# GAMES-UChile/mogptk

Hardware: AMD Instinct MI355X
Metric: log-marginal-likelihood+grad evals/sec, MOSM C=4 N=8192; 1/2/4/8 GPU (higher is better)
Workload: dtype f64

## Files before the change

mogptk_amd/csrc/exact.hip:

```cpp
#include "mogp_model.h"
#include <cstdlib>
#include <limits>

using namespace mogp;

static int wait_stream(hipStream_t st) {
    static const bool spin = !(std::getenv("MOGP_SPIN_WAIT") && std::atoi(std::getenv("MOGP_SPIN_WAIT")) == 0);
    if (!spin) { HIP_TRY(hipStreamSynchronize(st)); return 0; }
    for (;;) {
        const hipError_t e = hipStreamQuery(st);
        if (e == hipSuccess) return 0;
        if (e != hipErrorNotReady) return hip_fail(e, "hipStreamQuery", __FILE__, __LINE__);
    }
}

static hipEvent_t prof_event(mogp_model* m, int idx) {
    if (!m->profiling) return nullptr;
    while ((int)m->ev.size() <= idx) { hipEvent_t e; if (hipEventCreate(&e) != hipSuccess) return nullptr; m->ev.push_back(e); }
    return m->ev[idx];
}

static void kinv_block_ranges(mogp_model* m) {
    std::vector<int> blk;
    tile_blocks(m->sx.off, m->C, blk);
    const int nblk = (int)blk.size() / 2, D = m->D;
    m->blk_cen.assign((size_t)D * nblk, 0.0); m->blk_half.assign((size_t)D * nblk, 0.0);
    for (int b = 0; b < nblk; ++b)
        for (int d = 0; d < D; ++d) {
            const double* x = m->sx.xs.data() + (size_t)d * m->sx.Mpad + blk[2 * b];
            double lo = x[0], hi = x[0];
            for (int i = 1; i < blk[2 * b + 1]; ++i) { lo = std::fmin(lo, x[i]); hi = std::fmax(hi, x[i]); }
            m->blk_cen[(size_t)d * nblk + b] = 0.5 * (lo + hi); m->blk_half[(size_t)d * nblk + b] = 0.5 * (hi - lo);
        }
}

static int kinv_plan(mogp_model* m, bool want) {
    static const bool full = std::getenv("MOGP_FULL_INVERSE") && std::atoi(std::getenv("MOGP_FULL_INVERSE")) != 0;
    m->kinv_sparse = false; m->kinv_fraction = 1.0;
    if (!want || full || m->sh_n > 1 || m->tiles.empty() || m->radial) return 0;
    const int nb = m->nb, D = m->D, T = m->T, W = m->Wt;
    const int64_t ld = m->Npad;
    if (m->blk_cen.empty()) kinv_block_ranges(m);
    const int nblk = (int)(m->blk_cen.size() / std::max(D, 1));
    std::vector<char> need((size_t)nb * nb, 0);
    for (const GTile& t : m->tiles) {
        const double* tab = m->table.data() + (size_t)t.pair * T * W;
        bool read = false;
        for (int k = 0; k < T && !read; ++k) {
            const double* row = tab + (size_t)k * W;
            double emin = 0.0;
            for (int d = 0; d < D; ++d) {
                const double sd = (m->blk_cen[(size_t)d * nblk + t.rb] - m->blk_cen[(size_t)d * nblk + t.cb]) + row[2 + 2 * D + d];
                const double mu = std::fmax(0.0, std::fabs(sd) - m->blk_half[(size_t)d * nblk + t.rb] - m->blk_half[(size_t)d * nblk + t.cb]);
                emin += row[2 + d] * mu * mu;
            }
            read = !(0.5 * emin > 52.0);
        }
        if (!read) continue;
        const int i0 = t.r0 / MOGP_TILE, i1 = (t.r0 + t.nr - 1) / MOGP_TILE, j0 = t.c0 / MOGP_TILE, j1 = (t.c0 + t.nc - 1) / MOGP_TILE;
        for (int i = i0; i <= i1; ++i) for (int j = j0; j <= j1; ++j) if (j <= i) need[(size_t)i * nb + j] = 1;
    }
    for (int i = 0; i < nb; ++i) need[(size_t)i * nb + i] = 1;
    std::vector<GemmTask> acc, lau;
    std::vector<int> prefix(nb + 1, 0);
    for (int i = 0; i < nb; ++i) {
        for (int j = 0; j <= i; ++j) {
            if (!need[(size_t)i * nb + j]) continue;
            GemmTask a;
            a.a_off = (int64_t)i * MOGP_TILE; a.b_off = (int64_t)j * MOGP_TILE; a.c_off = (int64_t)i * MOGP_TILE * ld + (int64_t)j * MOGP_TILE;
            a.kt = 4 * MOGP_TILE / 16; a.pad = i + 1;
            acc.push_back(a);
            GemmTask l;
            l.a_off = (int64_t)i * MOGP_TILE * ld + (int64_t)i * MOGP_TILE; l.b_off = (int64_t)i * MOGP_TILE * ld + (int64_t)j * MOGP_TILE;
            l.c_off = a.c_off; l.kt = (int)((ld - (int64_t)i * MOGP_TILE) / 16); l.pad = 0;
            lau.push_back(l);
        }
        prefix[i + 1] = (int)acc.size();
    }
    const double frac = (double)acc.size() / ((double)nb * (nb + 1) / 2);
    m->kinv_fraction = frac;
    if (frac > 0.85) return 0;
    const bool same = acc.size() == m->kinv_acc_tasks.size() && (acc.empty() || std::memcmp(acc.data(), m->kinv_acc_tasks.data(), acc.size() * sizeof(GemmTask)) == 0);
    if (!same || m->d_kinv_acc.n < acc.size()) {
        int rc;
        if ((rc = m->d_kinv_acc.ensure(std::max<size_t>(acc.size(), 1)))) return rc;
        if ((rc = m->d_kinv_lauum.ensure(std::max<size_t>(lau.size(), 1)))) return rc;
        HIP_TRY(hipMemcpyAsync(m->d_kinv_acc.p, acc.data(), acc.size() * sizeof(GemmTask), hipMemcpyHostToDevice, m->st));
        HIP_TRY(hipMemcpyAsync(m->d_kinv_lauum.p, lau.data(), lau.size() * sizeof(GemmTask), hipMemcpyHostToDevice, m->st));
        HIP_TRY(hipStreamSynchronize(m->st));
        m->kinv_acc_tasks.swap(acc); m->kinv_lauum_tasks.swap(lau);
    }
    m->kinv_prefix.swap(prefix);
    m->kinv_sparse = true;
    return 0;
}

static int pin_ensure(mogp_model* m, size_t n) {
    if (n <= m->h_pin_n) return 0;
    if (m->h_pin) { hipError_t e = hipHostFree(m->h_pin); (void)e; m->h_pin = nullptr; m->h_pin_n = 0; }
    HIP_TRY(hipHostMalloc(reinterpret_cast<void**>(&m->h_pin), n * sizeof(double), hipHostMallocDefault));
    m->h_pin_n = n;
    return 0;
}
struct PinLayout {
    size_t nzz, logdet = 0, zz, info, moments, diagG, pivots, total;
    PinLayout(int nb, int64_t Npad, int C, int T, int Wt) : nzz((size_t)((Npad + 3) / 4)) {
        zz = (size_t)nb; info = zz + nzz; moments = info + 1; diagG = moments + (size_t)(C * (C + 1) / 2) * T * Wt; pivots = diagG + C; total = pivots + 2;
    }
    explicit PinLayout(const mogp_model* m) : PinLayout(m->nb, m->Npad, m->C, m->T, m->Wt) {}
};

namespace mogp {
int begin_call(mogp_model* m, int64_t* info, bool one_gpu) {
    m->mean_w = nullptr;
    if (int rc = use_device(m->ctx)) return rc;
    if (info) *info = 0;
    if (one_gpu) one_gpu_call(m);
    return 0;
}

int exact_begin(mogp_model* m, const double* noise_var, const double* data_var, double jitter, GramArgs& ga, double& jabs) {
    const int C = m->C;
    const int64_t N = m->N, Npad = m->Npad;
    if (m->T <= 0) return fail(MOGP_EINVAL, "mogp_model_set_terms must be called before an evaluation");
    if (!noise_var) return fail(MOGP_EINVAL, "noise_var is null");
    { int r__ = ensure_system(m); if (r__) return r__; }
    m->have_W = m->have_Kinv = false;
    m->gemm_ev_used = 0; m->gemm_launches = 0; m->gemm_flops = 0.0;

    double dsum = 0.0;
    if (!m->point_diag.empty()) {
        for (int c = 0; c < C; ++c)
            for (int k = m->sx.off[c]; k < m->sx.off[c + 1]; ++k) dsum += m->point_diag[k] + noise_var[c];
    } else if (m->radial && m->point_kinds) {
        dsum = table_diag_points(m, m->sx);
        for (int c = 0; c < C; ++c) dsum += (double)(m->sx.off[c + 1] - m->sx.off[c]) * noise_var[c];
    } else
    for (int c = 0; c < C; ++c) dsum += (double)(m->sx.off[c + 1] - m->sx.off[c]) * (table_diag(m, c) + noise_var[c]);
    if (data_var) {
        std::vector<double> dv(Npad, 0.0);
        for (int64_t pos = 0; pos < N; ++pos) { dv[pos] = data_var[m->sx.perm[pos]]; dsum += dv[pos]; }
        { int r__ = m->d_dvar.ensure(Npad); if (r__) return r__; }
        HIP_TRY(hipMemcpyAsync(m->d_dvar.p, dv.data(), Npad * sizeof(double), hipMemcpyHostToDevice, m->st));
    }
    jabs = jitter * dsum / (double)N;
    HIP_TRY(hipMemcpyAsync(m->d_noise.p, noise_var, C * sizeof(double), hipMemcpyHostToDevice, m->st));
    static const unsigned long long big = std::numeric_limits<unsigned long long>::max();
    HIP_TRY(hipMemcpyAsync(m->d_info.p, &big, sizeof(big), hipMemcpyHostToDevice, m->st));
    int rc;
    if ((rc = mark(m, 0))) return rc;
    ga = GramArgs{};
    ga.tiles = m->d_tiles.p; ga.xr = m->d_x.p; ga.xc = m->d_x.p; ga.ldxr = ga.ldxc = Npad; ga.nrows = ga.ncols = N;
    if ((rc = m->ph_xx.prepare(m->sx.off, m->sx.off, C, m->T, Npad, Npad, m->st, ga.ph))) return rc;
    ga.table = m->d_table.p; ga.T = m->T; ga.D = m->D; ga.C = C; ga.W = m->Wt;
    ga.out = m->k.A.p; ga.ldo = Npad; ga.noise = m->d_noise.p; ga.dvar = data_var ? m->d_dvar.p : nullptr;
    ga.jitter_abs = jabs; ga.mirror = 0;
    if (m->radial) { ga.kind = m->d_kind.p; ga.shape = m->d_shape.p; }
    return 0;
}
}

namespace mogp { int chain_fallback(mogp_model* m) {
    if (m->flow_ran) {
        m->no_flow = true; m->flow_ran = false;
        m->flow_timeouts++;
        m->flow_retry_at = m->n_fact + m->flow_backoff;
        m->flow_backoff = std::min(m->flow_backoff * 4, 16384);
        for (hipStream_t q : {m->st, m->st2, m->st3, m->st4, m->ctx->st5, m->st_priv}) if (q) HIP_TRY(hipStreamSynchronize(q));
        static bool said_flow = false;
        if (!said_flow) {
            said_flow = true;
            unsigned code = 0;
            if (m->k.flow_flags.p && m->k.flow_cur && m->k.flow_cur->base_err > 0) { hipError_t e = hipMemcpy(&code, m->k.flow_flags.p + m->k.flow_cur->base_err, sizeof(code), hipMemcpyDeviceToHost); (void)e; }
            fprintf(stderr, "mogp: the dataflow kernel timed out (wait 0x%x; GPU shared with another process?); using the stream schedule for the next %d evaluations (said once)\n", code, (int)(m->flow_retry_at - m->n_fact));
            fprintf(stderr, "mogp: the host enqueued that evaluation in %.0f us (longest so far %.0f us)\n", m->flow_enqueue_us, m->flow_enqueue_us_max);
        }
        if (std::getenv("MOGP_FLOW_DEBUG")) { fprintf(stderr, "mogp: dataflow time-out %d of this model\n", m->flow_timeouts); flow_debug_dump(m); }
        return 0;
    }
    if (m->no_chain) return fail(MOGP_EHIP, "chain kernel: a hand-off timed out although the model is on the launch-per-step chain");
    m->no_chain = true;
    for (hipStream_t q : {m->st, m->st2, m->st3, m->st4, m->ctx->st5, m->st_priv}) if (q) HIP_TRY(hipStreamSynchronize(q));
    static bool said = false;
    if (!said) { said = true; fprintf(stderr, "mogp: the persistent chain kernel timed out (GPU shared with another process?); using the launch-per-step chain\n"); }
    return 0;
} }

template <typename F> static int retry_on_streams(mogp_model* m, int rc, F again) {
    if (rc != MOGP_RETRY_NO_CHAIN) return rc;
    if ((rc = chain_fallback(m))) return rc;
    return again();
}

namespace mogp { int report_not_pd(unsigned long long hinfo, int64_t* info) {
    if (info) *info = (int64_t)hinfo;
    return fail(MOGP_ENOTPD, "linalg.cholesky: The factorization could not be completed because the input is not "
                             "positive-definite (the leading minor of order " + std::to_string(hinfo) + " is not positive-definite).");
} }

static int factorize_finish(mogp_model* m, const GramArgs& ga, double* lml, int64_t* info) {
    const int64_t N = m->N, Npad = m->Npad;
    const PinLayout pl(m);
    const unsigned long long big = std::numeric_limits<unsigned long long>::max();
    unsigned long long hinfo = 0;
    std::memcpy(&hinfo, m->h_pin + pl.info, sizeof(hinfo));
    int rc;
    if (hinfo == MOGP_INFO_CHAIN_TIMEOUT) return MOGP_RETRY_NO_CHAIN;
    static const bool fake = std::getenv("MOGP_FAKE_K") && std::atoi(std::getenv("MOGP_FAKE_K")) > 1;
    if (hinfo != big && !fake) {
        if (info) *info = (int64_t)hinfo;
        int flag = 0;
        HIP_TRY(hipMemsetAsync(m->d_flag.p, 0, sizeof(int), m->st));
        if ((rc = launch_gram(ga, (int)m->tiles.size(), m->st, m->radial ? m->gate_kinds : 0))) return rc;
        if ((rc = launch_nonfinite_scan(m->k.A.p, Npad, N, m->d_flag.p, m->st))) return rc;
        HIP_TRY(hipMemcpyAsync(&flag, m->d_flag.p, sizeof(int), hipMemcpyDeviceToHost, m->st));
        HIP_TRY(hipStreamSynchronize(m->st));
        if (flag & 1) return fail(MOGP_ENONFINITE, "linalg.cholesky: kernel matrix has NaNs!");
        if (flag & 2) return fail(MOGP_ENONFINITE, "linalg.cholesky: kernel matrix has infinities!");
        return report_not_pd(hinfo, info);
    }
    m->pivot_min = m->h_pin[pl.pivots]; m->pivot_max = m->h_pin[pl.pivots + 1];
    double logdet = 0.0, zz = 0.0;
    for (int i = 0; i < m->nb; ++i) logdet += m->h_pin[pl.logdet + i];
    for (size_t i = 0; i < pl.nzz; ++i) zz += m->h_pin[pl.zz + i];
    if (lml) *lml = -0.5 * (double)N * std::log(2.0 * M_PI) - logdet - 0.5 * zz;
    m->have_W = !m->factor_only && !m->accurate_ran;
    return 0;
}

struct FactorPlan {
    enum Schedule { Fused, Phases, FactorOnly } schedule = Phases;
    bool defer = false;
    bool want_inverse = true;
    bool refine = false;
};

static int factorize(mogp_model* m, const double* noise_var, const double* data_var, double jitter, const FactorPlan& plan,
                     double* lml, double* jitter_abs, int64_t* info, GramArgs* ga_out = nullptr) {
    const bool fuse_inverse = plan.schedule == FactorPlan::Fused, factor_only = plan.schedule == FactorPlan::FactorOnly;
    const int64_t N = m->N, Npad = m->Npad;
    GramArgs ga{};
    double jabs = 0.0;
    int rc = exact_begin(m, noise_var, data_var, jitter, ga, jabs);
    if (rc) return rc;
    if (jitter_abs) *jitter_abs = jabs;
    m->n_fact++;
    if (m->no_flow && m->n_fact >= m->flow_retry_at) m->no_flow = false;
    m->factor_only = factor_only;
    ga.ev0 = prof_event(m, 7); ga.ev1 = prof_event(m, 8);
    m->strip.attach(ga);
    static const bool split_on = !(std::getenv("MOGP_GRAM_SPLIT") && std::atoi(std::getenv("MOGP_GRAM_SPLIT")) == 0);
    const bool split = split_on && fuse_inverse && flow_enabled(m, m->k) && !m->tiles_head.empty() && !m->tiles_tail.empty() && m->st2;
    if (split) {
        GramArgs gh = ga, gt = ga;
        gh.tiles = m->d_tiles_head.p; m->strip_head.attach(gh); gh.ev1 = nullptr;
        gt.tiles = m->d_tiles_tail.p; m->strip_tail.attach(gt); gt.ev0 = nullptr; gt.phases_ready = 1;
        if ((rc = launch_gram(gh, (int)m->tiles_head.size(), m->st, m->radial ? m->gate_kinds : 0))) return rc;
        if ((rc = launch_pad_identity(m->k.A.p, Npad, N, Npad, m->st))) return rc;
        if (!m->gram_ev) HIP_TRY(hipEventCreateWithFlags(&m->gram_ev, hipEventDisableTiming));
        HIP_TRY(hipEventRecord(m->gram_ev, m->st));
        HIP_TRY(hipStreamWaitEvent(m->st2, m->gram_ev, 0));
        if ((rc = launch_gram(gt, (int)m->tiles_tail.size(), m->st2, m->radial ? m->gate_kinds : 0))) return rc;
        if (!m->gram_tail_ev) HIP_TRY(hipEventCreateWithFlags(&m->gram_tail_ev, hipEventDisableTiming));
        HIP_TRY(hipEventRecord(m->gram_tail_ev, m->st2));
        m->k.tail_ready = m->gram_tail_ev;
    } else {
        if ((rc = launch_gram(ga, (int)m->tiles.size(), m->st, m->radial ? m->gate_kinds : 0))) return rc;
        if ((rc = launch_pad_identity(m->k.A.p, Npad, N, Npad, m->st))) return rc;
    }
    ga.ev0 = ga.ev1 = nullptr;
    if ((rc = mark(m, 1))) return rc;

    const PinLayout pl(m);
    if ((rc = pin_ensure(m, pl.total))) return rc;
    if ((rc = m->d_pivots.ensure(2))) return rc;
    if (m->accurate && (rc = m->acc_rhs.ensure((size_t)Npad * MOGP_TILE))) return rc;
    m->k.flow_used = false;
    m->flow_ran = false;
    m->k.want_vec = fuse_inverse;
    m->k.vec_y = m->d_y.p; m->k.vec_z = m->d_z.p; m->k.vec_zz = m->d_zz.p; m->k.vec_part = m->d_alpha.p + Npad;
    const bool accurate = m->accurate && plan.schedule == FactorPlan::Phases;
    m->accurate_ran = accurate;
    m->k.keep_L = m->k.refine_panels = plan.refine || accurate;
    if (factor_only && m->rhs_job && flow_enabled(m, m->k)) rc = spd_potri_flow(m, m->k, m->rhs_job);
    else rc = fuse_inverse ? spd_potri_fused(m, m->k) : spd_potrf(m, m->k);
    m->k.keep_L = m->k.refine_panels = false;
    m->k.want_vec = false; m->k.tail_ready = nullptr;
    if (rc) return rc;
    if ((rc = mark(m, 2))) return rc;
    if (accurate) {
        static const bool acc_aside = !(std::getenv("MOGP_ACC_ASIDE") && std::atoi(std::getenv("MOGP_ACC_ASIDE")) == 0);
        hipStream_t ms = (plan.want_inverse && m->st2u && acc_aside) ? m->st2u : m->st;
        if (plan.want_inverse) {
            if (ms != m->st) {
                while ((int)m->k.inv_ev.size() < 4) { hipEvent_t e; HIP_TRY(hipEventCreateWithFlags(&e, hipEventDisableTiming)); m->k.inv_ev.push_back(e); }
                HIP_TRY(hipEventRecord(m->k.inv_ev[0], m->st));
                HIP_TRY(hipStreamWaitEvent(ms, m->k.inv_ev[0], 0));
            }
            if ((rc = m->k.Wm.ensure((size_t)Npad * Npad))) return rc;
            HIP_TRY(hipMemsetAsync(m->k.Wm.p, 0, (size_t)Npad * Npad * sizeof(double), ms));
            if ((rc = launch_add_diag(m->k.Wm.p, Npad, Npad, 1.0, ms))) return rc;
            if ((rc = trsm_lower(m, m->k.A.p, Npad, m->nb, m->k.Wm.p, Npad, Npad, false, ms, true))) return rc;
            GemmArgs g{};
            g.A = m->k.Wm.p; g.lda = Npad; g.a_kmajor = 1; g.B = m->k.Wm.p; g.ldb = Npad; g.b_kmajor = 1;
            g.C = m->k.B.p; g.ldc = Npad; g.alpha = 1.0; g.beta = 0.0; g.mode = GM_LAUUM; g.mt = g.nt = m->nb; g.K = (int)Npad;
            if ((rc = gemm_call(m, g, gemm_flops(g, nullptr), ms))) return rc;
            if (ms != m->st) HIP_TRY(hipEventRecord(m->k.inv_ev[1], ms));
        }
        HIP_TRY(hipMemsetAsync(m->acc_rhs.p, 0, (size_t)Npad * MOGP_TILE * sizeof(double), m->st));
        if ((rc = launch_copy2d(m->acc_rhs.p, MOGP_TILE, m->d_y.p, 1, Npad, 1, 1.0, m->st))) return rc;
        if ((rc = trsm_lower(m, m->k.A.p, Npad, m->nb, m->acc_rhs.p, MOGP_TILE, MOGP_TILE, false))) return rc;
        if ((rc = launch_copy2d(m->d_z.p, 1, m->acc_rhs.p, MOGP_TILE, Npad, 1, 1.0, m->st))) return rc;
        HIP_TRY(hipMemsetAsync(m->d_zz.p, 0, pl.nzz * sizeof(double), m->st));
        if ((rc = launch_gemv_rows(m->d_z.p, Npad, 1, Npad, m->d_z.p, m->d_zz.p, m->st))) return rc;
        if ((rc = trsm_lower(m, m->k.A.p, Npad, m->nb, m->acc_rhs.p, MOGP_TILE, MOGP_TILE, true))) return rc;
        if ((rc = launch_copy2d(m->d_alpha.p, 1, m->acc_rhs.p, MOGP_TILE, Npad, 1, 1.0, m->st))) return rc;
        if (plan.want_inverse && ms != m->st) HIP_TRY(hipStreamWaitEvent(m->st, m->k.inv_ev[1], 0));
    } else if (plan.schedule == FactorPlan::Phases && (rc = spd_trtri(m, m->k))) return rc;
    if ((rc = mark(m, 3))) return rc;

    if (factor_only) {
        HIP_TRY(hipMemsetAsync(m->d_zz.p, 0, pl.nzz * sizeof(double), m->st));
    } else if (!accurate) {
        const double* Wp = fuse_inverse ? m->k.Wm.p : m->k.A.p;
        m->w_in_Wm = fuse_inverse;
        if (fuse_inverse && m->k.flow_used && m->k.vec_done) {
            if ((rc = launch_flow_alpha_sum(m->k, m->d_alpha.p, m->st))) return rc;
        } else {
            if ((rc = launch_trmv_lower(Wp, Npad, Npad, m->d_y.p, m->d_z.p, m->d_zz.p, m->st))) return rc;
            if ((rc = launch_trmv_lower_t(Wp, Npad, Npad, m->d_z.p, m->d_alpha.p, m->st))) return rc;
        }
    }
    if (fuse_inverse && (rc = spd_potri_fused_finish(m, m->k))) return rc;
    if ((rc = mark(m, 4))) return rc;
    {
        static const bool fault = std::getenv("MOGP_FLOW_FAULT") && std::atoi(std::getenv("MOGP_FLOW_FAULT")) != 0;
        static const unsigned long long timed_out = MOGP_INFO_CHAIN_TIMEOUT;
        if (fault && m->k.flow_used) HIP_TRY(hipMemcpyAsync(m->d_info.p, &timed_out, sizeof(timed_out), hipMemcpyHostToDevice, m->st));
    }

    const int nzz = (int)pl.nzz;
    if ((rc = launch_pivot_range(m->k.invd.p, N, m->d_pivots.p, m->st))) return rc;
    HIP_TRY(hipMemcpyAsync(m->h_pin + pl.pivots, m->d_pivots.p, 2 * sizeof(double), hipMemcpyDeviceToHost, m->st));
    HIP_TRY(hipMemcpyAsync(m->h_pin + pl.logdet, m->k.logdet.p, m->nb * sizeof(double), hipMemcpyDeviceToHost, m->st));
    static const int zz_piece = []() { const char* e = std::getenv("MOGP_D2H_CHUNK"); const int v = e ? std::atoi(e) : 2048; return v > 0 ? v : (1 << 30); }();
    for (int o = 0; o < nzz; o += zz_piece)
        HIP_TRY(hipMemcpyAsync(m->h_pin + pl.zz + o, m->d_zz.p + o, std::min(zz_piece, nzz - o) * sizeof(double), hipMemcpyDeviceToHost, m->st));
    HIP_TRY(hipMemcpyAsync(m->h_pin + pl.info, m->d_info.p, sizeof(unsigned long long), hipMemcpyDeviceToHost, m->st));
    if (ga_out) *ga_out = ga;
    if (plan.defer) return 0;
    HIP_TRY(hipStreamSynchronize(m->st));
    return factorize_finish(m, ga, lml, info);
}

namespace mogp { void collect_timing(mogp_model* m, int last_mark) {
    if (!m->profiling) return;
    auto el = [&](int a, int b) { float t = 0.f; if (hipEventElapsedTime(&t, m->ev[a], m->ev[b]) != hipSuccess) t = 0.f; return (double)t; };
    std::fill(m->ms, m->ms + MOGP_ST_COUNT, 0.0);
    m->ms[MOGP_ST_GRAM] = el(0, 1);
    m->ms[MOGP_ST_POTRF] = el(1, 2);
    m->ms[MOGP_ST_TRTRI] = el(2, 3);
    m->ms[MOGP_ST_SOLVE] = el(3, 4);
    if (last_mark >= 6) { m->ms[MOGP_ST_LAUUM] = el(4, 5); m->ms[MOGP_ST_MOMENTS] = el(5, 6); }
    m->ms[MOGP_ST_TOTAL] = el(0, last_mark);
    if ((int)m->ev.size() > 8) m->ms[MOGP_ST_GRAM_KERNEL] = el(7, 8);
    if (last_mark >= 6 && (int)m->ev.size() > 10) m->ms[MOGP_ST_MOMENT_KERNEL] = el(9, 10);
    double gsum = 0.0;
    for (size_t i = 0; i + 1 < m->gemm_ev_used; i += 2) {
        float t = 0.f;
        if (hipEventElapsedTime(&t, m->gemm_ev[i], m->gemm_ev[i + 1]) == hipSuccess) gsum += t;
    }
    m->ms[MOGP_ST_GEMM_KERNEL] = gsum;
}

int moment_pass_device(mogp_model* m, const double* kinv, double ksign) {
    const int C = m->C, D = m->D, W = m->Wt, T = m->T, P = C * (C + 1) / 2;
    const int64_t Npad = m->Npad;
    const int rm = m->sh_n > 1 ? m->sh_n : 0;
    const bool own = m->sh_n > 1 && m->own_n == m->sh_n && m->own_rank == m->sh_rank;
    int rc;
    MomentArgs ma{};
    ma.tiles = own ? m->d_tiles_own.p : m->d_tiles.p; ma.ntiles = (int)(own ? m->tiles_own.size() : m->tiles.size());
    ma.x = m->d_x.p; ma.ldx = Npad; ma.nrows = ma.ncols = m->N;
    if ((rc = m->ph_xx.prepare(m->sx.off, m->sx.off, C, T, Npad, Npad, m->st, ma.ph))) return rc;
    ma.table = m->d_table.p; ma.T = T; ma.D = D; ma.C = C; ma.W = W; ma.kinv = kinv; ma.kinv_sign = ksign; ma.ld = Npad; ma.alpha = m->d_alpha.p;
    ma.row_mod = rm; ma.row_rem = m->sh_rank;
    if (m->radial) { ma.kind = m->d_kind.p; ma.shape = m->d_shape.p; }
    ma.partial = m->d_partial.p;
    ma.phases_ready = 1;
    ma.ev0 = prof_event(m, 9); ma.ev1 = prof_event(m, 10);
    if ((rc = launch_moments(ma, m->st, m->radial ? m->gate_kinds : 0))) return rc;
    if ((rc = launch_moment_reduce(m->d_partial.p, own ? m->d_pair_start_own.p : m->d_pair_start.p, P, T, W, D, m->d_moments.p, m->st))) return rc;
    if ((rc = launch_diagG(kinv, Npad, m->d_alpha.p, m->d_chan_off.p, C, m->d_diagG.p, m->st, ksign, rm, m->sh_rank))) return rc;
    if ((rc = mean_grad_enqueue(m, m->d_alpha.p, -1.0))) return rc;
    return mark(m, 6);
}

int moment_pass(mogp_model* m, const double* kinv, double ksign, double* moments, double* diagG) {
    const int C = m->C, W = m->Wt, T = m->T, P = C * (C + 1) / 2;
    int rc;
    if ((rc = moment_pass_device(m, kinv, ksign))) return rc;
    HIP_TRY(hipMemcpyAsync(moments, m->d_moments.p, (size_t)P * T * W * sizeof(double), hipMemcpyDeviceToHost, m->st));
    HIP_TRY(hipMemcpyAsync(diagG, m->d_diagG.p, C * sizeof(double), hipMemcpyDeviceToHost, m->st));
    HIP_TRY(hipStreamSynchronize(m->st));
    return 0;
}

int test_side(mogp_model* m, int64_t S, const double* Xs, const double* kss_diag, int64_t extra_rows, hipStream_t st, TestSide& ts, GramArgs& ga) {
    const int C = m->C, D = m->D;
    const int64_t Npad = m->Npad;
    SortedX& ss = ts.ss;
    int rc;
    if ((rc = sort_inputs(Xs, S, D, C, MOGP_TILE, ss))) return rc;
    const int64_t Spad = ts.Spad = ss.Mpad, Srow = Spad + extra_rows;
    std::vector<GTile> pt;
    build_rect_tiles(ss.off, m->sx.off, C, pt);
    ts.ntiles = (int)pt.size();
    if ((rc = m->d_xs.ensure((size_t)D * Spad))) return rc;
    if ((rc = m->d_Ksf.ensure((size_t)Srow * Npad))) return rc;
    if ((rc = m->d_mu.ensure(Spad))) return rc;
    if ((rc = m->d_kdiag.ensure(Spad))) return rc;
    if ((rc = m->d_ptiles.ensure(std::max<size_t>(pt.size(), 1)))) return rc;
    std::vector<double> kd(Spad, 0.0);
    const bool per_point = m->Wt > 2 + 3 * D || (m->radial && m->point_kinds);
    for (int c = 0; c < C; ++c)
        for (int pos = ss.off[c]; pos < ss.off[c + 1]; ++pos) kd[pos] = per_point ? kss_diag[ss.perm[pos]] : kss_diag[c];
    HIP_TRY(hipMemcpyAsync(m->d_xs.p, ss.xs.data(), (size_t)D * Spad * sizeof(double), hipMemcpyHostToDevice, st));
    HIP_TRY(hipMemcpyAsync(m->d_kdiag.p, kd.data(), Spad * sizeof(double), hipMemcpyHostToDevice, st));
    HIP_TRY(hipMemcpyAsync(m->d_ptiles.p, pt.data(), pt.size() * sizeof(GTile), hipMemcpyHostToDevice, st));
    HIP_TRY(hipMemsetAsync(m->d_Ksf.p, 0, (size_t)Srow * Npad * sizeof(double), st));
    ga = GramArgs{};
    ga.tiles = m->d_ptiles.p; ga.xr = m->d_xs.p; ga.ldxr = Spad; ga.xc = m->d_x.p; ga.ldxc = Npad; ga.nrows = S; ga.ncols = m->N;
    if ((rc = m->ph_sx.prepare(ss.off, m->sx.off, C, m->T, Spad, Npad, st, ga.ph))) return rc;
    ga.table = m->d_table.p; ga.T = m->T; ga.D = D; ga.C = C; ga.W = m->Wt; ga.out = m->d_Ksf.p; ga.ldo = Npad;
    ga.noise = nullptr; ga.dvar = nullptr; ga.jitter_abs = 0.0; ga.mirror = 0;
    if (m->radial) { ga.kind = m->d_kind.p; ga.shape = m->d_shape.p; }
    return 0;
}
}

static const std::string& grad_path_env() {
    static const std::string grad_path = []() { const char* e = std::getenv("MOGP_GRAD_PATH"); return std::string(e ? e : ""); }();
    return grad_path;
}

static int enqueue_inverse(mogp_model* m, const double* noise_var, const double* data_var, double jitter, bool inverse, bool banded,
                           double* lml, double* jitter_abs, int64_t* info, GramArgs& ga) {
    const std::string& grad_path = grad_path_env();
    int rc;
    if ((rc = ensure_system(m))) return rc;
    if ((rc = kinv_plan(m, inverse && banded && !m->accurate))) return rc;
    const int fused_max = flow_enabled(m, m->k) ? 112 : 80;
    const bool fused = inverse && !m->accurate && (grad_path == "fused" || (grad_path != "phases" && m->nb <= fused_max));
    FactorPlan plan;
    plan.schedule = fused ? FactorPlan::Fused : FactorPlan::Phases; plan.defer = inverse; plan.want_inverse = inverse;
    if ((rc = factorize(m, noise_var, data_var, jitter, plan, lml, jitter_abs, info, &ga))) return rc;
    if (!inverse) return 0;
    if (!fused && !m->accurate_ran && (rc = spd_lauum(m, m->k))) return rc;
    return mark(m, 5);
}

extern "C" {

int mogp_exact_eval(mogp_model* m, const double* noise_var, const double* data_var, double jitter, int flags,
                    double* lml, double* moments, double* diagG, double* trG, double* jitter_abs, int64_t* info) {
    if (!m) return fail(MOGP_EINVAL, "mogp_exact_eval: model is null");
    int rc;
    if ((rc = begin_call(m, info, true))) return rc;
    const std::string& grad_path = grad_path_env();
    const bool sweep = grad_path == "sweep" && (flags & MOGP_EVAL_GRAD);
    const bool grad = (flags & MOGP_EVAL_GRAD) != 0;
    GramArgs ga{};
    auto again = [&]() { return mogp_exact_eval(m, noise_var, data_var, jitter, flags, lml, moments, diagG, trG, jitter_abs, info); };
    if (grad && (!moments || !diagG || !trG)) return fail(MOGP_EINVAL, "mogp_exact_eval: gradient outputs are null");
    if (sweep) {
        if ((rc = ensure_system(m))) return rc;
        if ((rc = kinv_plan(m, false))) return rc;
        m->pivot_min = m->pivot_max = 0.0;
        if ((rc = eval_sweep(m, noise_var, data_var, jitter, lml, jitter_abs, info))) return retry_on_streams(m, rc, again);
    }
    else if ((rc = enqueue_inverse(m, noise_var, data_var, jitter, grad, true, lml, jitter_abs, info, ga))) return retry_on_streams(m, rc, again);
    if (!grad) { collect_timing(m, 4); return MOGP_OK; }

    const int C = m->C, W = m->Wt, T = m->T, P = C * (C + 1) / 2;

    const double* kinv = sweep ? m->k.A.p : m->k.B.p;
    const double ksign = sweep ? -1.0 : 1.0;
    if (sweep && (rc = mark(m, 5))) return rc;
    if (sweep) {
        if ((rc = moment_pass(m, kinv, ksign, moments, diagG))) return rc;
    } else {
        if ((rc = moment_pass_device(m, kinv, ksign))) return rc;
        const PinLayout pl(m);
        HIP_TRY(hipMemcpyAsync(m->h_pin + pl.moments, m->d_moments.p, (size_t)P * T * W * sizeof(double), hipMemcpyDeviceToHost, m->st));
        HIP_TRY(hipMemcpyAsync(m->h_pin + pl.diagG, m->d_diagG.p, C * sizeof(double), hipMemcpyDeviceToHost, m->st));
        if ((rc = wait_stream(m->st))) return rc;
        if ((rc = factorize_finish(m, ga, lml, info))) return retry_on_streams(m, rc, again);
        std::memcpy(moments, m->h_pin + pl.moments, (size_t)P * T * W * sizeof(double));
        std::memcpy(diagG, m->h_pin + pl.diagG, C * sizeof(double));
    }
    double tr = 0.0;
    for (int c = 0; c < C; ++c) tr += diagG[c];
    *trG = tr;
    m->have_Kinv = true;
    m->kinv_in_A = sweep;
    mean_grad_collect(m);
    collect_timing(m, 6);
    return MOGP_OK;
}

int mogp_exact_loo(mogp_model* m, const double* noise_var, const double* data_var, double jitter, int flags,
                   double* loo, double* mu, double* var, double* moments, double* diagG, double* trG, double* jitter_abs, int64_t* info) {
    if (!m) return fail(MOGP_EINVAL, "mogp_exact_loo: model is null");
    if (!loo || !mu || !var) return fail(MOGP_EINVAL, "mogp_exact_loo: loo, mu or var is null");
    const bool grad = (flags & MOGP_EVAL_GRAD) != 0;
    if (grad && (!moments || !diagG || !trG)) return fail(MOGP_EINVAL, "mogp_exact_loo: gradient outputs are null");
    int rc;
    if ((rc = begin_call(m, info, true))) return rc;
    auto again = [&]() { return mogp_exact_loo(m, noise_var, data_var, jitter, flags, loo, mu, var, moments, diagG, trG, jitter_abs, info); };
    const int C = m->C, W = m->Wt, T = m->T, P = C * (C + 1) / 2;
    const int64_t N = m->N, Npad = m->Npad;
    if ((rc = ensure_system(m))) return rc;
    if ((rc = loo_workspace(m, grad))) return rc;
    const PinLayout pl(m);
    const size_t pin_loo = pl.total, pin_mu = pin_loo + 1, pin_var = pin_mu + (size_t)Npad;
    if ((rc = pin_ensure(m, pin_var + (size_t)Npad))) return rc;
    GramArgs ga{};
    if ((rc = enqueue_inverse(m, noise_var, data_var, jitter, true, false, nullptr, jitter_abs, info, ga))) return retry_on_streams(m, rc, again);
    double* v = m->loo.vec.p;
    if ((rc = loo_points(m, m->k.B.p))) return rc;
    if (grad) {
        m->have_W = false;
        if ((rc = loo_adjoint(m, m->k.B.p, m->k.A.p))) return rc;
        if ((rc = loo_moment_pass(m))) return rc;
        HIP_TRY(hipMemcpyAsync(m->h_pin + pl.moments, m->d_moments.p, (size_t)P * T * W * sizeof(double), hipMemcpyDeviceToHost, m->st));
        HIP_TRY(hipMemcpyAsync(m->h_pin + pl.diagG, m->d_diagG.p, C * sizeof(double), hipMemcpyDeviceToHost, m->st));
    }
    HIP_TRY(hipMemcpyAsync(m->h_pin + pin_loo, v + LOO_SUM * Npad, sizeof(double), hipMemcpyDeviceToHost, m->st));
    HIP_TRY(hipMemcpyAsync(m->h_pin + pin_mu, v + LOO_MU * Npad, N * sizeof(double), hipMemcpyDeviceToHost, m->st));
    HIP_TRY(hipMemcpyAsync(m->h_pin + pin_var, v + LOO_VAR * Npad, N * sizeof(double), hipMemcpyDeviceToHost, m->st));
    if ((rc = wait_stream(m->st))) return rc;
    if ((rc = factorize_finish(m, ga, nullptr, info))) return retry_on_streams(m, rc, again);
    if (grad) m->have_W = false;
    *loo = m->h_pin[pin_loo];
    scatter_by_perm(m->sx, m->h_pin + pin_mu, mu);
    scatter_by_perm(m->sx, m->h_pin + pin_var, var);
    m->have_Kinv = true;
    m->kinv_in_A = false;
    if (!grad) { collect_timing(m, 5); return MOGP_OK; }
    std::memcpy(moments, m->h_pin + pl.moments, (size_t)P * T * W * sizeof(double));
    std::memcpy(diagG, m->h_pin + pl.diagG, C * sizeof(double));
    double tr = 0.0;
    for (int c = 0; c < C; ++c) tr += diagG[c];
    *trG = tr;
    mean_grad_collect(m);
    collect_timing(m, 6);
    return MOGP_OK;
}

int mogp_exact_cv(mogp_model* m, const double* noise_var, const double* data_var, double jitter, int flags, const int32_t* fold, int64_t nfolds,
                  double* cv, double* mu, double* var, double* moments, double* diagG, double* trG, double* jitter_abs, int64_t* info) {
    if (!m) return fail(MOGP_EINVAL, "mogp_exact_cv: model is null");
    if (!fold || !cv || !mu || !var) return fail(MOGP_EINVAL, "mogp_exact_cv: fold, cv, mu or var is null");
    const bool grad = (flags & MOGP_EVAL_GRAD) != 0;
    if (grad && (!moments || !diagG || !trG)) return fail(MOGP_EINVAL, "mogp_exact_cv: gradient outputs are null");
    int rc;
    if ((rc = begin_call(m, info, true))) return rc;
    auto again = [&]() { return mogp_exact_cv(m, noise_var, data_var, jitter, flags, fold, nfolds, cv, mu, var, moments, diagG, trG, jitter_abs, info); };
    const int C = m->C, W = m->Wt, T = m->T, P = C * (C + 1) / 2;
    const int64_t N = m->N, Npad = m->Npad;
    if ((rc = ensure_system(m))) return rc;
    if ((rc = cv_workspace(m, fold, nfolds, grad))) return rc;
    const PinLayout pl(m);
    const size_t pin_cv = pl.total, pin_mu = pin_cv + 1, pin_var = pin_mu + (size_t)Npad, pin_info = pin_var + (size_t)Npad;
    if ((rc = pin_ensure(m, pin_info + 1))) return rc;
    GramArgs ga{};
    if ((rc = enqueue_inverse(m, noise_var, data_var, jitter, true, false, nullptr, jitter_abs, info, ga))) return retry_on_streams(m, rc, again);
    double* v = m->loo.vec.p;
    if ((rc = cv_points(m, m->k.B.p, grad))) return rc;
    if (grad) {
        m->have_W = false;
        if ((rc = cv_adjoint(m, m->k.B.p, m->k.A.p))) return rc;
        if ((rc = loo_moment_pass(m))) return rc;
        HIP_TRY(hipMemcpyAsync(m->h_pin + pl.moments, m->d_moments.p, (size_t)P * T * W * sizeof(double), hipMemcpyDeviceToHost, m->st));
        HIP_TRY(hipMemcpyAsync(m->h_pin + pl.diagG, m->d_diagG.p, C * sizeof(double), hipMemcpyDeviceToHost, m->st));
    }
    HIP_TRY(hipMemcpyAsync(m->h_pin + pin_cv, v + LOO_SUM * Npad, sizeof(double), hipMemcpyDeviceToHost, m->st));
    HIP_TRY(hipMemcpyAsync(m->h_pin + pin_mu, v + LOO_MU * Npad, N * sizeof(double), hipMemcpyDeviceToHost, m->st));
    HIP_TRY(hipMemcpyAsync(m->h_pin + pin_var, v + LOO_VAR * Npad, N * sizeof(double), hipMemcpyDeviceToHost, m->st));
    HIP_TRY(hipMemcpyAsync(m->h_pin + pin_info, m->d_info.p, sizeof(unsigned long long), hipMemcpyDeviceToHost, m->st));
    if ((rc = wait_stream(m->st))) return rc;
    if ((rc = factorize_finish(m, ga, nullptr, info))) return retry_on_streams(m, rc, again);
    if (grad) m->have_W = false;
    unsigned long long finfo = 0;
    std::memcpy(&finfo, m->h_pin + pin_info, sizeof(finfo));
    if (finfo != std::numeric_limits<unsigned long long>::max()) {
        if (info) *info = (int64_t)(finfo - 1) / 256;
        return fail(MOGP_ENOTPD, "mogp_exact_cv: the block of Kj^-1 over fold " + std::to_string((finfo - 1) / 256) + " is not positive definite (pivot " +
                                 std::to_string((finfo - 1) % 256 + 1) + " of its factorisation): Kj is too ill-conditioned for this fold");
    }
    *cv = m->h_pin[pin_cv];
    for (int64_t pos = 0; pos < N; ++pos)
        if (m->cv.label[pos] < 0) m->h_pin[pin_mu + pos] = m->h_pin[pin_var + pos] = std::numeric_limits<double>::quiet_NaN();
    scatter_by_perm(m->sx, m->h_pin + pin_mu, mu);
    scatter_by_perm(m->sx, m->h_pin + pin_var, var);
    m->have_Kinv = true;
    m->kinv_in_A = false;
    if (!grad) { collect_timing(m, 5); return MOGP_OK; }
    std::memcpy(moments, m->h_pin + pl.moments, (size_t)P * T * W * sizeof(double));
    std::memcpy(diagG, m->h_pin + pl.diagG, C * sizeof(double));
    double tr = 0.0;
    for (int c = 0; c < C; ++c) tr += diagG[c];
    *trG = tr;
    mean_grad_collect(m);
    collect_timing(m, 6);
    return MOGP_OK;
}

int mogp_model_loo_bytes(mogp_model* m, int64_t* bytes) {
    if (!m || !bytes) return fail(MOGP_EINVAL, "mogp_model_loo_bytes: bad argument");
    *bytes = (int64_t)((m->loo.G.n + m->loo.vec.n) * sizeof(double) + cv_bytes(m));
    return MOGP_OK;
}

static int predict_core(mogp_model* m, const double* noise_var, const double* data_var, double jitter,
                        const double* kss_diag, int64_t S, const double* Xs, int full,
                        double* mu, double* var, int64_t* info, const double* mean_w) {
    int rc;
    if ((rc = begin_call(m, info, true))) return rc;
    const int C = m->C, nb = m->nb;
    const int64_t Npad = m->Npad;
    hipStream_t sv = m->st3 ? m->st3 : m->st;
    for (auto& e : m->pred_ev) if (!e) HIP_TRY(hipEventCreateWithFlags(&e, hipEventDisableTiming));
    HIP_TRY(hipEventRecord(m->pred_ev[0], m->st));
    HIP_TRY(hipStreamWaitEvent(sv, m->pred_ev[0], 0));
    TestSide ts; GramArgs ga{};
    if ((rc = test_side(m, S, Xs, kss_diag, MOGP_TILE, sv, ts, ga))) return rc;
    const SortedX& ss = ts.ss;
// ... 137 lines not shown
```

mogptk_amd/csrc/flow.hip:

```cpp
#include "mogp_model.h"
#include <unistd.h>
#include <chrono>
#include <set>

#include <cstdio>
#include <cstdlib>

namespace mogp {

typedef double d4_t __attribute__((ext_vector_type(4)));
typedef double d2_t __attribute__((ext_vector_type(2)));

#define FL_BK 16
#define FL_ROWK 18
#define FL_WTM 4
#define FL_WTN 2
#define FL_NWJ 4
#define FL_NWI 2
#define FL_NT 512
#define FL_COLK (MOGP_TILE + 16)
#define FL_OPER (MOGP_TILE * FL_ROWK)
#define FL_LDS_DOUBLES (2 * 2 * FL_OPER)
#define FL_LDS_BYTES (FL_LDS_DOUBLES * 8 + 16 + 3 * 64 * 4 + 16)
static_assert(MOGP_TILE * FL_ROWK == 16 * FL_COLK, "one LDS operand slot serves both layouts");
// ... 659 lines not shown
}
int launch_flow_alpha_sum(const Spd& w, double* alpha, hipStream_t st) {
    const FlowPlan& p = w.flow_cur ? *w.flow_cur : w.flow;
    hipLaunchKernelGGL(k_alpha_sum, dim3((unsigned)((w.Npad + 255) / 256)), dim3(256), 0, st, w.vec_part, w.Npad, p.nouter, p.ob, alpha);
    HIP_TRY(hipGetLastError());
    return 0;
}

bool flow_enabled(const mogp_model* m, const Spd& w) {
    const char* eo = std::getenv("MOGP_FLOW");
    const char* en = std::getenv("MOGP_FLOW_MIN");
    const int on = eo ? std::atoi(eo) : 1, nmin = en ? std::atoi(en) : 8;
    if (!on || (m->no_flow && m->n_fact < m->flow_retry_at) || !chain_enabled(m) || !m->ctx->st_priv) return false;
    if (m->kinv_sparse && &w == &m->k) return false;
    return w.nb >= nmin && w.nb <= 0xfff0;
}

int spd_potri_flow(mogp_model* m, Spd& w, const FlowRhs* rhs) {
    const int nb = w.nb, ob = 4;
    const int64_t ld = w.Npad;
    int rc;
    const auto host_t0 = std::chrono::steady_clock::now();
    hipStream_t crit = m->st, priv = m->st_priv, bulk = m->st2;
    if (w.Wm.n < (size_t)ld * ld) {
        if ((rc = w.Wm.ensure((size_t)ld * ld))) return rc;
        HIP_TRY(hipMemsetAsync(w.Wm.p, 0, (size_t)ld * ld * sizeof(double), crit));
    }
    if ((rc = w.Lm.ensure((size_t)ld * ld))) return rc;
    if (!rhs && (rc = w.Wt.ensure((size_t)ld * ld))) return rc;
    const bool replay = m->replay_flow && !rhs && &w == &m->k;
    FlowPlan& plan = rhs ? w.flow_rhs : replay ? w.flow_replay : w.flow;
    DevBuf<FlowTask>& d_tasks = rhs ? w.flow_tasks_rhs : replay ? w.flow_tasks_replay : w.flow_tasks;
    DevBuf<int>& d_qmeta = rhs ? w.flow_qmeta_rhs : replay ? w.flow_qmeta_replay : w.flow_qmeta;
    const int rhs_nt = rhs ? rhs->nt : 0;
    if (plan.nb != nb || plan.ob != ob || plan.rhs_nt != rhs_nt) {
        flow_build(nb, ob, plan, rhs_nt, replay);
        if ((rc = d_tasks.ensure(plan.tasks.size()))) return rc;
        if ((rc = d_qmeta.ensure(2 * FLOW_MAXQ))) return rc;
        int qm[2 * FLOW_MAXQ] = {0};
        for (int q = 0; q < plan.nq; ++q) { qm[2 * q] = plan.qbase[q]; qm[2 * q + 1] = plan.qsize[q]; }
        HIP_TRY(hipStreamSynchronize(crit));
        HIP_TRY(dev_upload(d_tasks.p, plan.tasks.data(), plan.tasks.size() * sizeof(FlowTask)));
        HIP_TRY(dev_upload(d_qmeta.p, qm, sizeof(qm)));
    }
    if ((rc = w.flow_flags.ensure((size_t)plan.nflags))) return rc;
    if (!w.flow_diag.p) {
        if ((rc = w.flow_diag.ensure(FLOW_DIAG_WORDS))) return rc;
        HIP_TRY(hipMemsetAsync(w.flow_diag.p, 0, FLOW_DIAG_WORDS * sizeof(unsigned), crit));
    }
    w.flow_cur = &plan;
    const FlowPlan& p = plan;
    const int nouter = p.nouter;
    if ((rc = w.chain_flags.ensure((size_t)(nouter + 1) * MOGP_CHAIN_FLAGS))) return rc;
    HIP_TRY(hipMemsetAsync(w.chain_flags.p, 0, (size_t)(nouter + 1) * MOGP_CHAIN_FLAGS * sizeof(unsigned), crit));
    HIP_TRY(hipMemsetAsync(w.flow_flags.p, 0, (size_t)p.nflags * sizeof(unsigned), crit));
    if (replay) {
        std::vector<unsigned> preset((size_t)p.nflags, 0u);
        for (const FlowPlan::Chain& c : p.chain) preset[c.done_idx] = c.expect;
        HIP_TRY(hipMemcpyAsync(w.flow_flags.p, preset.data(), preset.size() * sizeof(unsigned), hipMemcpyHostToDevice, crit));
        HIP_TRY(hipStreamSynchronize(crit));
    }
    if (!rhs && w.want_vec && w.vec_zz) HIP_TRY(hipMemsetAsync(w.vec_zz, 0, (size_t)((ld + 3) / 4) * sizeof(double), crit));
    static const bool want_trace = std::getenv("MOGP_FLOW_TRACE") && std::atoi(std::getenv("MOGP_FLOW_TRACE")) != 0;
    if (want_trace) {
        if ((rc = w.flow_trace.ensure(FLOW_TRACE_W * p.tasks.size() + 4 * (size_t)nouter))) return rc;
        HIP_TRY(hipMemsetAsync(w.flow_trace.p, 0, w.flow_trace.n * sizeof(unsigned long long), crit));
    }
    while ((int)w.inv_ev.size() < 4) {
        hipEvent_t e;
        HIP_TRY(hipEventCreateWithFlags(&e, hipEventDisableTiming));
        w.inv_ev.push_back(e);
    }
    hipEvent_t start = w.inv_ev[0], e_flow = w.inv_ev[1], e_chain = w.inv_ev[2];
    HIP_TRY(hipEventRecord(start, crit));
    HIP_TRY(hipStreamWaitEvent(bulk, start, 0));
    HIP_TRY(hipStreamWaitEvent(priv, start, 0));

    static std::atomic<unsigned long long> attr_done{0ull};
    static std::atomic<unsigned long long> attr_done_dbg{0ull};
    { int r__ = set_max_dynamic_lds(reinterpret_cast<const void*>(k_flow<false>), FL_LDS_BYTES, attr_done); if (r__) return r__; }
    { int r__ = set_max_dynamic_lds(reinterpret_cast<const void*>(k_flow<true>), FL_LDS_BYTES, attr_done_dbg); if (r__) return r__; }
    static const int wg_per_cu = std::getenv("MOGP_FLOW_WGS") ? std::max(1, std::atoi(std::getenv("MOGP_FLOW_WGS"))) : 2;
    int cus = (m->ctx->ncu > 0 ? m->ctx->ncu : 256) - m->ctx->ncu_reserved;
    { static const int drop = std::getenv("MOGP_FLOW_DROP_CUS") ? std::atoi(std::getenv("MOGP_FLOW_DROP_CUS")) : 16;
      if (drop > 0 && drop < cus) cus -= drop; }
    FlowArgs g{};
    g.bA = w.A.p; g.bL = w.Lm.p; g.bWt = rhs ? rhs->T : w.Wt.p; g.bWm = w.Wm.p; g.bB = rhs ? rhs->X : w.B.p; g.ld = ld;
    g.tasks = d_tasks.p; g.qmeta = d_qmeta.p; g.flags = w.flow_flags.p;
    g.nq = p.nq; g.ncas = FLOW_NCAS; g.base_heads = p.base_heads; g.base_err = p.base_err; g.info = m->d_info.p;
    g.trace = want_trace ? w.flow_trace.p : nullptr;
    g.diag = w.flow_diag.p;
    static const bool want_post = std::getenv("MOGP_FLOW_DEBUG") && std::atoi(std::getenv("MOGP_FLOW_DEBUG")) != 0;
    if (want_post) {
        const size_t nwg = (size_t)wg_per_cu * ((size_t)cus + (size_t)m->ctx->ncu_reserved);
        if ((rc = w.flow_post.ensure(nwg * FLOW_POST_W))) return rc;
        HIP_TRY(hipMemsetAsync(w.flow_post.p, 0, w.flow_post.n * sizeof(unsigned), bulk));
        g.post = w.flow_post.p;
        if ((rc = w.flow_done.ensure(p.tasks.size()))) return rc;
        HIP_TRY(hipMemsetAsync(w.flow_done.p, 0, p.tasks.size(), bulk));
        g.done = w.flow_done.p;
    }
    g.npad = ld;
    { const char* e = std::getenv("MOGP_FLOW_REFILL"); g.refill = e ? std::atoi(e) : 0; }
    { const char* e = std::getenv("MOGP_FLOW_CLAIM1"); g.claim_one = e ? std::atoi(e) : 0; }
    { const char* e = std::getenv("MOGP_FLOW_NHI"); g.nhi = e ? std::atoi(e) : 0; }
    { const char* e = std::getenv("MOGP_FLOW_NAP"); g.nap_max = e ? (unsigned)std::max(0, std::atoi(e)) : 4u; }
    { const char* e = std::getenv("MOGP_FLOW_NAP_CALM"); g.nap_calm = e ? (unsigned)std::max(0, std::atoi(e)) : 0u; if (g.nap_calm < g.nap_max) g.nap_calm = g.nap_max; }
    w.vec_done = false;
    if (!rhs && w.want_vec && w.vec_y && w.vec_z && w.vec_zz && w.vec_part) {
        g.vy = w.vec_y; g.vz = w.vec_z; g.vzz = w.vec_zz; g.vpart = w.vec_part;
        w.vec_done = true;
    }
    hipEvent_t pe0 = nullptr, pe1 = nullptr;
    if (m->profiling) {
        if (m->gemm_ev_used + 2 > m->gemm_ev.size())
            for (int i = 0; i < 64; ++i) { hipEvent_t e; HIP_TRY(hipEventCreate(&e)); m->gemm_ev.push_back(e); }
        pe0 = m->gemm_ev[m->gemm_ev_used++]; pe1 = m->gemm_ev[m->gemm_ev_used++];
        HIP_TRY(hipEventRecord(pe0, bulk));
    }
    if (rhs && rhs->ready) HIP_TRY(hipStreamWaitEvent(bulk, rhs->ready, 0));
    const bool dbg_kernel = g.post != nullptr || g.trace != nullptr;
    static_assert(sizeof(FlowArgs) <= 512, "Spd::flow_args slots");
    if ((rc = w.flow_args.ensure(1024))) return rc;
    if (w.flow_args_h.size() != 2048) w.flow_args_h.assign(2048, (char)0xff);
    auto upload = [&](size_t slot, const FlowArgs& a, hipStream_t st) -> int {
        char* held = w.flow_args_h.data() + slot;
        char* fresh_ = w.flow_args_h.data() + 1024 + slot;
        std::memset(fresh_, 0, 512);
        std::memcpy(fresh_, &a, sizeof(a));
        if (std::memcmp(held, fresh_, 512) == 0) return 0;
        HIP_TRY(hipStreamSynchronize(st));
        HIP_TRY(dev_upload(w.flow_args.p + slot, fresh_, 512));
        std::memcpy(held, fresh_, 512);
        return 0;
    };
    if ((rc = upload(0, g, bulk))) return rc;
    const FlowArgs* d_g = reinterpret_cast<const FlowArgs*>(w.flow_args.p);
    FlowHot hot{};
    hot.bA = g.bA; hot.bL = g.bL; hot.bWt = g.bWt; hot.bWm = g.bWm; hot.bB = g.bB; hot.ld = g.ld; hot.tasks = g.tasks; hot.qmeta = g.qmeta; hot.flags = g.flags;
    hot.nq = g.nq; hot.ncas = g.ncas; hot.base_heads = g.base_heads; hot.base_err = g.base_err; hot.nap_max = g.nap_max; hot.nap_calm = g.nap_calm;
    if (dbg_kernel) hipLaunchKernelGGL(k_flow<true>, dim3(wg_per_cu * cus), dim3(FL_NT), FL_LDS_BYTES, bulk, d_g, hot);
    else hipLaunchKernelGGL(k_flow<false>, dim3(wg_per_cu * cus), dim3(FL_NT), FL_LDS_BYTES, bulk, d_g, hot);
    HIP_TRY(hipGetLastError());
    if (pe1) HIP_TRY(hipEventRecord(pe1, bulk));
    HIP_TRY(hipEventRecord(e_flow, bulk));
    m->gemm_launches += 1;
    m->gemm_flops += p.flops;

    unsigned* ferr = w.flow_flags.p + p.base_err;
    for (int kb = 0; kb < nouter && !replay; ++kb) {
        const int k0 = kb * ob, k1 = std::min(k0 + ob, nb), nk = k1 - k0, na = std::min(ob, nb - k1);
        const FlowPlan::Chain& pc = p.chain[kb];
        ChainFlow cf{};
        cf.done_flag = w.flow_flags.p + pc.done_idx; cf.write_through = 1;
        cf.trace = want_trace ? w.flow_trace.p + FLOW_TRACE_W * p.tasks.size() + 4 * (size_t)kb : nullptr;
        cf.diag = w.flow_diag.p;
        if ((rc = launch_chain(w.A.p, ld, k0, nk, w.invd.p, w.logdet.p, m->d_info.p, 0, w.Wm.p + (int64_t)k0 * MOGP_TILE * (ld + 1), ld,
                               w.chain_flags.p + (size_t)kb * MOGP_CHAIN_FLAGS, ferr, priv, &cf))) return rc;
        if (na <= 0) continue;
        GemmArgs t1{};
        t1.A = w.A.p + (int64_t)k1 * MOGP_TILE * ld + (int64_t)k0 * MOGP_TILE; t1.lda = ld; t1.a_kmajor = 0;
        t1.B = w.Wm.p + (int64_t)k0 * MOGP_TILE * (ld + 1); t1.ldb = ld; t1.b_kmajor = 0;
        t1.C = w.Lm.p + (int64_t)k1 * MOGP_TILE * ld + (int64_t)k0 * MOGP_TILE; t1.ldc = ld; t1.alpha = 1.0; t1.beta = 0.0;
        t1.mode = GM_KHI_J; t1.small = 1; t1.mt = 2 * na; t1.nt = nk; t1.K = nk * MOGP_TILE;
        t1.fl_flags = w.flow_flags.p; t1.fl_nwait = pc.t1_nwait;
        for (int k = 0; k < pc.t1_nwait; ++k) { t1.fl_widx[k] = pc.t1_widx[k]; t1.fl_wval[k] = pc.t1_wval[k]; }
        static const unsigned hook_spins = std::getenv("MOGP_FLOW_HOOK_SPINS") ? (unsigned)std::atoll(std::getenv("MOGP_FLOW_HOOK_SPINS")) : 0u;
        t1.fl_spins = hook_spins; t1.fl_diag = w.flow_diag.p;
        t1.fl_wt = 1; t1.fl_sig = 1; t1.fl_sig_base = pc.t1_sig_base; t1.fl_sig_shift = 1; t1.fl_err = ferr; t1.sk_info = m->d_info.p;
        if ((rc = launch_gemm(t1, priv))) return rc;
        if (kb == 0 && w.tail_ready) HIP_TRY(hipStreamWaitEvent(priv, w.tail_ready, 0));
        GemmArgs t2{};
        t2.A = t1.C; t2.lda = ld; t2.a_kmajor = 0; t2.B = t1.C; t2.ldb = ld; t2.b_kmajor = 0;
        t2.C = w.A.p + (int64_t)k1 * MOGP_TILE * (ld + 1); t2.ldc = ld; t2.alpha = -1.0; t2.beta = 1.0;
        t2.mode = GM_RECT_LOWER; t2.small = 2; t2.mt = 2 * na; t2.nt = 2 * na; t2.K = nk * MOGP_TILE;
        t2.fl_flags = w.flow_flags.p; t2.fl_nwait = pc.t2_wval ? 1 : 0; t2.fl_widx[0] = pc.t2_widx; t2.fl_wval[0] = pc.t2_wval;
        t2.fl_err = ferr; t2.sk_info = m->d_info.p; t2.fl_spins = hook_spins; t2.fl_diag = w.flow_diag.p;
        if ((rc = launch_gemm(t2, priv))) return rc;
        m->gemm_flops += gemm_flops(t1, nullptr) + gemm_flops(t2, nullptr);
    }
    static const bool tail_on = !(std::getenv("MOGP_FLOW_TAIL") && std::atoi(std::getenv("MOGP_FLOW_TAIL")) == 0);
    if (tail_on && m->ctx->ncu_reserved > 0 && !replay) {
        if (rhs && rhs->ready) HIP_TRY(hipStreamWaitEvent(priv, rhs->ready, 0));
        g.post_base = wg_per_cu * cus;
        if ((rc = upload(512, g, priv))) return rc;
        const FlowArgs* d_g2 = reinterpret_cast<const FlowArgs*>(w.flow_args.p + 512);
        if (dbg_kernel) hipLaunchKernelGGL(k_flow<true>, dim3(wg_per_cu * m->ctx->ncu_reserved), dim3(FL_NT), FL_LDS_BYTES, priv, d_g2, hot);
        else hipLaunchKernelGGL(k_flow<false>, dim3(wg_per_cu * m->ctx->ncu_reserved), dim3(FL_NT), FL_LDS_BYTES, priv, d_g2, hot);
        HIP_TRY(hipGetLastError());
    }
    HIP_TRY(hipEventRecord(e_chain, priv));
    HIP_TRY(hipStreamWaitEvent(crit, e_flow, 0));
    HIP_TRY(hipStreamWaitEvent(crit, e_chain, 0));
    w.fused_last_inv = nullptr; w.fused_last_wt = nullptr;
    w.flow_used = true;
    m->flow_ran = true;
    m->flow_enqueue_us = std::chrono::duration<double, std::micro>(std::chrono::steady_clock::now() - host_t0).count();
    m->flow_enqueue_us_max = std::max(m->flow_enqueue_us_max, m->flow_enqueue_us);
    { const char* e = std::getenv("MOGP_FLOW_DEBUG");
      if (e && std::atoi(e) == 2 && &w == &m->k) { usleep(60000); fprintf(stderr, "mogp: dataflow state 60 ms after the evaluation was enqueued\n"); flow_debug_dump(m); } }
    return 0;
}

}

namespace mogp { void flow_debug_dump(mogp_model* m) {
    if (!m->k.flow_flags.p || !m->k.flow_cur) return;
    const FlowPlan& p = *m->k.flow_cur;
    std::vector<unsigned> fl((size_t)p.nflags);
    hipError_t e = hipMemcpy(fl.data(), m->k.flow_flags.p, fl.size() * sizeof(unsigned), hipMemcpyDeviceToHost); (void)e;
    std::vector<unsigned long long> tr;
// ... 212 lines not shown
```

mogptk_amd/csrc/gram.hip:

```cpp
#include "mogp_internal.h"

#include <algorithm>
#include <vector>
#include <cstdlib>

#ifdef MOGP_GRAM_DEBUG
#define GRAM_DBG(a, bit) ((a).dbg & (bit))
#else
#define GRAM_DBG(a, bit) 0
#endif

namespace mogp {

typedef double d2_t __attribute__((ext_vector_type(2)));

__device__ __forceinline__ double frac_turn(double p) { return p - rint(p); }

#define GT_SKIP (-1)
#define GT_GENERAL 0
#define GT_SKIP_EXPONENT 50.0
#define GT_DEGREE(zmax) ((zmax) <= 1.19e-3 ? 4 : (zmax) <= 4.93e-3 ? 5 : (zmax) <= 0.0139 ? 6 : (zmax) <= 0.0308 ? 7 : (zmax) <= 0.0578 ? 8 : (zmax) <= 0.0968 ? 9 : \
                         (zmax) <= 0.149 ? 10 : (zmax) <= 0.2147 ? 11 : (zmax) <= 0.294 ? 12 : 14)
#define GT_DEGREE_CASES(X) X(4) X(5) X(6) X(7) X(8) X(9) X(10) X(11) X(12) X(14)

__device__ __forceinline__ double fast_exp(double x) {
    const double n = rint(x * 1.44269504088896338700e+00);
    double r = fma(-n, 6.93147180369123816490e-01, x);
    r = fma(-n, 1.90821492927058770002e-10, r);
    double p = 1.6059043836821613e-10;
    p = fma(p, r, 2.08767569878681e-09);
    p = fma(p, r, 2.505210838544172e-08);
    p = fma(p, r, 2.755731922398589e-07);
    p = fma(p, r, 2.7557319223985893e-06);
    p = fma(p, r, 2.48015873015873e-05);
    p = fma(p, r, 1.984126984126984e-04);
    p = fma(p, r, 1.388888888888889e-03);
    p = fma(p, r, 8.333333333333333e-03);
    p = fma(p, r, 4.1666666666666664e-02);
    p = fma(p, r, 1.6666666666666666e-01);
    p = fma(p, r, 0.5);
    p = fma(p, r, 1.0);
    p = fma(p, r, 1.0);
    return ldexp(p, (int)n);
}

template <int N>
__device__ __forceinline__ double exp_taylor(double z) {
    constexpr double c[15] = {1.0, 1.0, 0.5, 1.6666666666666666e-01, 4.1666666666666664e-02, 8.333333333333333e-03,
                              1.388888888888889e-03, 1.984126984126984e-04, 2.48015873015873e-05, 2.7557319223985893e-06,
                              2.755731922398589e-07, 2.505210838544172e-08, 2.08767569878681e-09, 1.6059043836821613e-10,
                              1.1470745597729725e-11};
    double p = c[N];
#pragma unroll
    for (int k = N - 1; k >= 0; --k) p = fma(p, z, c[k]);
    return p;
}

struct PhaseArgs {
    const double* x; int64_t ld; const int* off; const double* table; int T, D, C, W, role; double* cs; double* sn;
};
__global__ __launch_bounds__(256) void k_phase_table(PhaseArgs a) {
    const int64_t pt = (int64_t)blockIdx.x * 256 + threadIdx.x;
    if (pt >= a.off[a.C]) return;
    const int o = blockIdx.y, t = blockIdx.z, D = a.D, W = a.W;
    int c = 0;
    while (pt >= a.off[c + 1]) ++c;
    const int pair = a.role == 0 ? c * a.C + o : o * a.C + c;
    const double* row = a.table + ((size_t)pair * a.T + t) * W;
    double ph = a.role == 0 ? row[1] : 0.0;
    for (int d = 0; d < D; ++d) {
        const double m = row[2 + D + d], xv = a.x[(size_t)d * a.ld + pt];
        ph = a.role == 0 ? fma(m, xv + row[2 + 2 * D + d], ph) : fma(m, xv, ph);
    }
    double sn, cs;
    sincospi(2.0 * frac_turn(ph), &sn, &cs);
    const size_t idx = ((size_t)o * a.T + t) * a.ld + pt;
    a.cs[idx] = cs;
    a.sn[idx] = sn;
}

struct CentreArgs { const double* x; int64_t ld; const int* off; int C, D; double* cen; double* half; };
__global__ __launch_bounds__(64) void k_block_centres(CentreArgs a) {
    int b = blockIdx.x, c = 0;
    for (; c < a.C; ++c) {
        const int nb = (a.off[c + 1] - a.off[c] + MOGP_GT - 1) / MOGP_GT;
        if (b < nb) break;
        b -= nb;
    }
    if (c >= a.C) return;
    const int start = a.off[c] + b * MOGP_GT, n = min(MOGP_GT, a.off[c + 1] - start), lane = threadIdx.x;
    for (int d = 0; d < a.D; ++d) {
        const double v = a.x[(size_t)d * a.ld + start + (lane < n ? lane : 0)];
        double lo = v, hi = v;
#pragma unroll
        for (int off = 32; off > 0; off >>= 1) { lo = fmin(lo, __shfl_xor(lo, off, 64)); hi = fmax(hi, __shfl_xor(hi, off, 64)); }
        if (lane == 0) { a.cen[(size_t)d * a.ld + start] = 0.5 * (lo + hi); a.half[(size_t)d * a.ld + start] = 0.5 * (hi - lo); }
    }
}

size_t phase_ws_doubles(int C, int T, int64_t ldr, int64_t ldc) { return (size_t)2 * (C * T + MOGP_MAXD) * (size_t)(ldr + ldc); }

struct PhaseView {
    const double *rcs, *rsn, *ccs, *csn, *rcen, *rhalf, *ccen, *chalf;
};
__host__ __device__ static inline PhaseView phase_view(double* ws, int C, int T, int D, int64_t ldr, int64_t ldc) {
    PhaseView v;
    double* p = ws;
    v.rcs = p; p += (size_t)C * T * ldr; v.rsn = p; p += (size_t)C * T * ldr;
    v.ccs = p; p += (size_t)C * T * ldc; v.csn = p; p += (size_t)C * T * ldc;
    v.rcen = p; p += (size_t)D * ldr; v.rhalf = p; p += (size_t)D * ldr;
    v.ccen = p; p += (size_t)D * ldc; v.chalf = p;
    return v;
}

static int launch_phase_tables(const PhaseRef& ph, const double* xr, int64_t ldxr, int64_t nr, const double* xc, int64_t ldxc, int64_t nc,
                               const double* table, int T, int D, int C, int W, hipStream_t s) {
    if (!ph.ws || !ph.offr || !ph.offc) { set_error("Gram / moment launch without a phase workspace"); return -1; }
    const PhaseView v = phase_view(ph.ws, C, T, D, ldxr, ldxc);
    PhaseArgs a;
    a.table = table; a.T = T; a.D = D; a.C = C; a.W = W;
    a.x = xr; a.ld = ldxr; a.off = ph.offr; a.role = 0; a.cs = const_cast<double*>(v.rcs); a.sn = const_cast<double*>(v.rsn);
    if (nr > 0) hipLaunchKernelGGL(k_phase_table, dim3((unsigned)((nr + 255) / 256), C, T), dim3(256), 0, s, a);
    a.x = xc; a.ld = ldxc; a.off = ph.offc; a.role = 1; a.cs = const_cast<double*>(v.ccs); a.sn = const_cast<double*>(v.csn);
    if (nc > 0) hipLaunchKernelGGL(k_phase_table, dim3((unsigned)((nc + 255) / 256), C, T), dim3(256), 0, s, a);
    CentreArgs c;
    c.C = C; c.D = D;
    c.x = xr; c.ld = ldxr; c.off = ph.offr; c.cen = const_cast<double*>(v.rcen); c.half = const_cast<double*>(v.rhalf);
    if (nr > 0) hipLaunchKernelGGL(k_block_centres, dim3((unsigned)((nr + MOGP_GT - 1) / MOGP_GT + C)), dim3(64), 0, s, c);
    c.x = xc; c.ld = ldxc; c.off = ph.offc; c.cen = const_cast<double*>(v.ccen); c.half = const_cast<double*>(v.chalf);
    if (nc > 0) hipLaunchKernelGGL(k_block_centres, dim3((unsigned)((nc + MOGP_GT - 1) / MOGP_GT + C)), dim3(64), 0, s, c);
    HIP_TRY(hipGetLastError());
    return 0;
}

template <int DM>
struct TileLds {
    double cu[MOGP_TC][MOGP_GT], su[MOGP_TC][MOGP_GT], cw[MOGP_TC][MOGP_GT], sw[MOGP_TC][MOGP_GT];
    double V[MOGP_TC][DM], s[MOGP_TC][DM], M[MOGP_TC][DM], A[MOGP_TC];
    double Kp[MOGP_TC][DM];
    double L[MOGP_TC][DM], e[MOGP_TC][DM];
    int deg[MOGP_TC];
};
template <int DM>
struct TileCtx { double cr[DM], cc[DM], hr[DM], hc[DM]; };

template <int DM>
__device__ __forceinline__ void tile_centres(TileCtx<DM>& X, const GTile& tl, int D, const PhaseView& v, int64_t ldxr, int64_t ldxc) {
    for (int d = 0; d < D; ++d) {
        X.cr[d] = v.rcen[(size_t)d * ldxr + tl.r0]; X.hr[d] = v.rhalf[(size_t)d * ldxr + tl.r0];
        X.cc[d] = v.ccen[(size_t)d * ldxc + tl.c0]; X.hc[d] = v.chalf[(size_t)d * ldxc + tl.c0];
    }
}

template <int DM>
__device__ __forceinline__ void tile_context(TileCtx<DM>& X, double (&p)[4][DM], double (&q)[4][DM], const GTile& tl, int D,
                                             const PhaseView& v, const double* __restrict__ xr, int64_t ldxr,
                                             const double* __restrict__ xc, int64_t ldxc, int rg, int cg) {
    tile_centres<DM>(X, tl, D, v, ldxr, ldxc);
#pragma unroll
    for (int m = 0; m < 4; ++m)
        for (int d = 0; d < D; ++d) {
            p[m][d] = xr[(size_t)d * ldxr + tl.r0 + min(rg * 4 + m, tl.nr - 1)] - X.cr[d];
            q[m][d] = xc[(size_t)d * ldxc + tl.c0 + min(cg * 4 + m, tl.nc - 1)] - X.cc[d];
        }
}

constexpr int STAGE_ITEMS = MOGP_TC * MOGP_GT * 2 / 256;
template <int DM>
struct StageItem { double x[DM], cs, sn; };

template <int DM>
__device__ __forceinline__ void stage_item_load(StageItem<DM>& I, int which, int t, int pnt, const GTile& tl, int D, int C, int T, int t0,
                                                const PhaseView& v, const double* __restrict__ xr, int64_t ldxr,
                                                const double* __restrict__ xc, int64_t ldxc) {
    const int i = tl.pair / C, j = tl.pair - i * C;
    if (which == 0) {
        const int64_t g = tl.r0 + min(pnt, tl.nr - 1);
        const size_t k = ((size_t)j * T + t0 + t) * ldxr + g;
        I.cs = v.rcs[k]; I.sn = v.rsn[k];
        for (int d = 0; d < D; ++d) I.x[d] = xr[(size_t)d * ldxr + g];
    } else {
        const int64_t g = tl.c0 + min(pnt, tl.nc - 1);
        const size_t k = ((size_t)i * T + t0 + t) * ldxc + g;
// ... 1682 lines not shown
```

mogptk_amd/csrc/loo.hip:

```cpp
#include "mogp_model.h"

using namespace mogp;

#define RC(x) do { int r__ = (x); if (r__) return r__; } while (0)

namespace {

__global__ __launch_bounds__(256) void k_loo_points(const double* __restrict__ kinv, int64_t ld, const double* __restrict__ alpha,
                                                    const double* __restrict__ y, int64_t N, int64_t Npad, double* __restrict__ vec) {
    const int64_t i = (int64_t)blockIdx.x * 256 + threadIdx.x;
    if (i >= Npad) return;
    double mu = 0.0, var = 0.0, a = 0.0, b = 0.0, sa = 0.0, term = 0.0;
    if (i < N) {
        const double kap = kinv[i * ld + i], al = alpha[i];
        var = 1.0 / kap;
        b = al * var;
        mu = y[i] - b;
        a = 0.5 * var + 0.5 * b * b;
        sa = sqrt(a);
        term = 0.5 * log(kap) - 0.5 * al * b - 0.91893853320467274178;
    }
    vec[LOO_MU * Npad + i] = mu; vec[LOO_VAR * Npad + i] = var; vec[LOO_A * Npad + i] = a; vec[LOO_B * Npad + i] = b;
    vec[LOO_SA * Npad + i] = sa; vec[LOO_TERM * Npad + i] = term;
}
// ... 43 lines not shown
    return 0;
}

int loo_points(mogp_model* m, double* kinv) {
    const int64_t N = m->N, Npad = m->Npad;
    double* v = m->loo.vec.p;
    RC(launch_symmetrize(kinv, Npad, Npad, m->st));
    const double* y = m->mean_on ? m->d_y0.p : m->d_y.p;
    hipLaunchKernelGGL(k_loo_points, dim3((unsigned)((Npad + 255) / 256)), dim3(256), 0, m->st, kinv, Npad, m->d_alpha.p, y, N, Npad, v);
    hipLaunchKernelGGL(k_loo_sum, dim3(1), dim3(256), 0, m->st, v + LOO_TERM * Npad, N, v + LOO_SUM * Npad);
    HIP_TRY(hipGetLastError());
    return 0;
}

int loo_adjoint(mogp_model* m, const double* kinv, double* scratch) {
    const int64_t N = m->N, Npad = m->Npad;
    double* v = m->loo.vec.p;
    double* rho = v + LOO_RHO * Npad;
    RC(launch_gemv_rows(kinv, Npad, Npad, Npad, v + LOO_B * Npad, rho, m->st));
    RC(launch_scale_cols(kinv, scratch, Npad, Npad, Npad, v + LOO_SA * Npad, m->st));
    GemmArgs g = make_gemm(scratch, Npad, 0, scratch, Npad, 0, m->loo.G.p, Npad, -1.0, GM_LOWER, m->nb, m->nb, Npad);
    RC(gemm_call(m, g, gemm_flops(g, nullptr)));
    hipLaunchKernelGGL(k_loo_rank2, dim3((unsigned)((N + 255) / 256), (unsigned)N), dim3(256), 0, m->st, m->loo.G.p, Npad, N, m->d_alpha.p, rho);
    HIP_TRY(hipGetLastError());
    return 0;
}

int launch_loo_sum(const double* term, int64_t n, double* out, hipStream_t st) {
    hipLaunchKernelGGL(k_loo_sum, dim3(1), dim3(256), 0, st, term, n, out);
    HIP_TRY(hipGetLastError());
    return 0;
}

int launch_loo_rank2(double* G, int64_t ld, int64_t n, const double* alpha, const double* rho, hipStream_t st) {
    hipLaunchKernelGGL(k_loo_rank2, dim3((unsigned)((n + 255) / 256), (unsigned)n), dim3(256), 0, st, G, ld, n, alpha, rho);
    HIP_TRY(hipGetLastError());
    return 0;
}

int loo_moment_pass(mogp_model* m) {
    const int C = m->C, D = m->D, W = m->Wt, T = m->T, P = C * (C + 1) / 2;
    const int64_t Npad = m->Npad;
    MomentArgs ma{};
    ma.tiles = m->d_tiles.p; ma.ntiles = (int)m->tiles.size();
    ma.x = m->d_x.p; ma.ldx = Npad; ma.nrows = ma.ncols = m->N;
    RC(m->ph_xx.prepare(m->sx.off, m->sx.off, C, T, Npad, Npad, m->st, ma.ph));
    ma.table = m->d_table.p; ma.T = T; ma.D = D; ma.C = C; ma.W = W;
    ma.G = m->loo.G.p; ma.ldg = Npad; ma.sym = 1; ma.ldgz = Npad;
    if (m->radial) { ma.kind = m->d_kind.p; ma.shape = m->d_shape.p; }
    ma.partial = m->d_partial.p;
    ma.phases_ready = 1;
    RC(launch_moments(ma, m->st, m->radial ? m->gate_kinds : 0));
    RC(launch_moment_reduce(m->d_partial.p, m->d_pair_start.p, P, T, W, D, m->d_moments.p, m->st, 1));
    hipLaunchKernelGGL(k_loo_diag, dim3(C), dim3(256), 0, m->st, m->loo.G.p, Npad, m->d_chan_off.p, m->d_diagG.p);
    HIP_TRY(hipGetLastError());
    RC(mean_grad_enqueue(m, m->loo.vec.p + LOO_RHO * Npad, -1.0));
    return mark(m, 6);
}

}
```

mogptk_amd/csrc/mogp_api.hip:

```cpp
#include "mogp_model.h"

#include <algorithm>
#include <cmath>
#include <cstring>
#include <cstdlib>

namespace mogp {

static thread_local std::string g_err;
void set_error(const std::string& msg) { g_err = msg; }
int hip_fail(hipError_t e, const char* what, const char* file, int line) {
    g_err = std::string("HIP error '") + hipGetErrorString(e) + "' in " + what + " (" + file + ":" + std::to_string(line) + ")";
    return MOGP_EHIP;
}
int launch_potrf_trtri_tile(double* A, int64_t ld, int t, double* invd, double* logdet, unsigned long long* info, hipStream_t s,
                            long long info_base = 0, int store_L = 0);

int fail(int code, const std::string& msg) { g_err = msg; return code; }

int sort_inputs(const double* X, int64_t M, int D, int C, int64_t pad_to, SortedX& o) {
    o.M = M;
    o.Mpad = round_up(std::max<int64_t>(M, 1), pad_to);
    o.perm.resize(M);
    o.off.assign(C + 1, 0);
// ... 529 lines not shown
                        v = r[0] * h * h;
                    }
                    prod *= v;
                    if (t == m->T - 1 || !(kd[t] & MOGP_KIND_TIMES)) { s += prod; prod = 1.0; }
                }
            }
        }
        return s;
    }
    if (W == 2 + 3 * D) {
        for (int c = 0; c < C; ++c) s += (double)(pts.off[c + 1] - pts.off[c]) * table_diag(m, c);
        return s;
    }
    for (int c = 0; c < C; ++c) {
        const double* tab = m->table.data() + (size_t)(c * C + c) * m->T * W;
        for (int pos = pts.off[c]; pos < pts.off[c + 1]; ++pos)
            for (int t = 0; t < m->T; ++t) {
                const double* r = tab + (size_t)t * W;
                double arg = 0.0, ph = r[1], env = 0.0;
                for (int d = 0; d < D; ++d) {
                    arg += r[2 + d] * r[2 + 2 * D + d] * r[2 + 2 * D + d];
                    ph += r[2 + D + d] * r[2 + 2 * D + d];
                    const double a = pts.xs[(size_t)d * pts.Mpad + pos] - r[2 + 4 * D + d];
                    env += r[2 + 3 * D + d] * a * a;
                }
                s += r[0] * std::exp(-0.5 * (arg + env)) * std::cos(2.0 * M_PI * ph);
            }
    }
    return s;
}
}

namespace mogp { void one_gpu_call(mogp_model* m) { m->sh_n = 1; m->sh_rank = 0; m->sh_owned = false; } }

namespace mogp { int ensure_system(mogp_model* m) {
    int rc;
    if (m->tiles.empty()) {
        build_sym_tiles(m->sx.off, m->C, m->tiles, m->pair_start);
        if ((rc = m->d_tiles.ensure(m->tiles.size()))) return rc;
        if ((rc = m->d_pair_start.ensure(m->pair_start.size()))) return rc;
        HIP_TRY(dev_upload(m->d_tiles.p, m->tiles.data(), m->tiles.size() * sizeof(GTile)));
        if ((rc = m->strip.build(m->tiles))) return rc;
        for (const GTile& t : m->tiles) (t.c0 < 4 * MOGP_TILE ? m->tiles_head : m->tiles_tail).push_back(t);
        if (!m->tiles_head.empty() && !m->tiles_tail.empty()) {
            if ((rc = m->d_tiles_head.ensure(m->tiles_head.size()))) return rc;
            if ((rc = m->d_tiles_tail.ensure(m->tiles_tail.size()))) return rc;
            HIP_TRY(dev_upload(m->d_tiles_head.p, m->tiles_head.data(), m->tiles_head.size() * sizeof(GTile)));
            HIP_TRY(dev_upload(m->d_tiles_tail.p, m->tiles_tail.data(), m->tiles_tail.size() * sizeof(GTile)));
            if ((rc = m->strip_head.build(m->tiles_head))) return rc;
            if ((rc = m->strip_tail.build(m->tiles_tail))) return rc;
        }
        HIP_TRY(dev_upload(m->d_pair_start.p, m->pair_start.data(), m->pair_start.size() * sizeof(int)));
    }
    if ((rc = m->d_partial.ensure(m->tiles.size() * (size_t)std::max(m->T, 1) * (size_t)std::max(m->Wt, 1)))) return rc;
    if (m->k.Npad == m->Npad) return (m->k.owned_rows && !m->sh_owned) ? spd_make_whole(m->k) : 0;
    return spd_alloc(m->k, m->Npad, m->sh_owned ? m->ctx->device : -1);
} }

extern "C" {

static int ctx_streams(mogp_ctx* ctx) {
    if (ctx->streams_ready) return 0;
    int lo_prio = 0;
    {
        int lo = 0, hi = 0;
        HIP_TRY(hipDeviceGetStreamPriorityRange(&lo, &hi));
        lo_prio = lo;
        HIP_TRY(hipStreamCreateWithPriority(&ctx->st, hipStreamNonBlocking, hi));
        const char* er = std::getenv("MOGP_RESERVE_CUS");
        const int reserve = er ? std::atoi(er) : 2;
        hipDeviceProp_t prop;
        HIP_TRY(hipGetDeviceProperties(&prop, ctx->device));
        const int ncu = prop.multiProcessorCount;
        const bool masked = reserve > 0 && 16 * reserve < ncu;
        ctx->ncu = ncu; ctx->ncu_reserved = masked ? 8 * reserve : 0;
        ctx->chain_ok = !masked || 8 * reserve >= 13;
        if (masked) {
            std::vector<uint32_t> bulk((ncu + 31) / 32, 0u), priv((ncu + 31) / 32, 0u);
            for (int i = 0; i < ncu; ++i) (i < 8 * reserve ? priv : bulk)[i / 32] |= 1u << (i % 32);
            HIP_TRY(hipExtStreamCreateWithCUMask(&ctx->st_priv, (uint32_t)priv.size(), priv.data()));
            HIP_TRY(hipExtStreamCreateWithCUMask(&ctx->st2, (uint32_t)bulk.size(), bulk.data()));
            HIP_TRY(hipExtStreamCreateWithCUMask(&ctx->st3, (uint32_t)bulk.size(), bulk.data()));
            HIP_TRY(hipExtStreamCreateWithCUMask(&ctx->st4, (uint32_t)bulk.size(), bulk.data()));
        } else {
            HIP_TRY(hipStreamCreateWithPriority(&ctx->st2, hipStreamNonBlocking, (lo + hi) / 2));
            HIP_TRY(hipStreamCreateWithPriority(&ctx->st3, hipStreamNonBlocking, lo));
            HIP_TRY(hipStreamCreateWithPriority(&ctx->st4, hipStreamNonBlocking, lo));
        }
    }
    {
        hipDeviceProp_t prop;
        HIP_TRY(hipGetDeviceProperties(&prop, ctx->device));
        std::vector<uint32_t> all((prop.multiProcessorCount + 31) / 32, 0u);
        for (int i = 0; i < prop.multiProcessorCount; ++i) all[i / 32] |= 1u << (i % 32);
        if (ctx->st_priv) HIP_TRY(hipExtStreamCreateWithCUMask(&ctx->st2u, (uint32_t)all.size(), all.data()));
        else HIP_TRY(hipStreamCreateWithPriority(&ctx->st2u, hipStreamNonBlocking, lo_prio));
    }
    ctx->streams_ready = true;
    return 0;
}

int mogp_model_create(mogp_ctx* ctx, int64_t N, int D, int C, const double* X, const double* y, mogp_model** out) {
    if (!ctx || !X || !y || !out) return fail(MOGP_EINVAL, "mogp_model_create: null argument");
    *out = nullptr;
    if (N <= 0 || D <= 0 || D > MOGP_MAXD || C <= 0) return fail(MOGP_EINVAL, "mogp_model_create: need N > 0, 0 < D <= 8, C > 0");
    int rc;
    if ((rc = use_device(ctx))) return rc;
    mogp_model* m = new mogp_model();
    m->ctx = ctx; m->N = N; m->D = D; m->C = C;
    if ((rc = sort_inputs(X, N, D, C, MOGP_TILE, m->sx))) { delete m; return rc; }
    m->Npad = m->sx.Mpad;
    m->nb = (int)(m->Npad / MOGP_TILE);
    const int64_t Npad = m->Npad;
    const int nchunks = (int)((Npad + 511) / 512);
#define TRY_RC(x) do { int r__ = (x); if (r__) { mogp_model_destroy(m); return r__; } } while (0)
#define TRY_HIP(x) do { hipError_t e__ = (x); if (e__ != hipSuccess) { int r__ = hip_fail(e__, #x, __FILE__, __LINE__); mogp_model_destroy(m); return r__; } } while (0)
    TRY_RC(ctx_streams(ctx));
    m->st = ctx->st; m->st2 = ctx->st2; m->st2u = ctx->st2u; m->st3 = ctx->st3; m->st4 = ctx->st4; m->st_priv = ctx->st_priv;
    TRY_RC(m->d_x.ensure((size_t)D * Npad));
    TRY_RC(m->d_y.ensure(Npad));
    TRY_RC(m->d_noise.ensure(C));
    TRY_RC(m->d_z.ensure(Npad));
    TRY_RC(m->d_alpha.ensure((size_t)(1 + nchunks) * Npad));
    TRY_RC(m->d_zz.ensure((Npad + 3) / 4));
    TRY_RC(m->d_diagG.ensure(C));
    TRY_RC(m->d_info.ensure(2));
    TRY_RC(m->d_flag.ensure(1));
    TRY_RC(m->d_chan_off.ensure(C + 1));
    TRY_HIP(dev_upload(m->d_x.p, m->sx.xs.data(), (size_t)D * Npad * sizeof(double)));
    TRY_HIP(dev_upload(m->d_chan_off.p, m->sx.off.data(), (C + 1) * sizeof(int)));
    TRY_RC(mogp_model_set_y(m, y));
#undef TRY_RC
#undef TRY_HIP
    *out = m;
    return MOGP_OK;
}

int mogp_model_destroy(mogp_model* m) {
    if (!m) return MOGP_OK;
    if (m->ctx) { hipError_t e = hipSetDevice(m->ctx->device); (void)e; }
    if (m->st) { hipError_t e = hipStreamSynchronize(m->st); (void)e; }
    for (auto e : m->ev) { hipError_t r = hipEventDestroy(e); (void)r; }
    for (auto e : m->gemm_ev) { hipError_t r = hipEventDestroy(e); (void)r; }
    for (auto& e : m->pred_ev) if (e) { hipError_t r = hipEventDestroy(e); (void)r; e = nullptr; }
    for (hipStream_t q : {m->st2, m->st2u, m->st3, m->st4, m->ctx->st5, m->st_priv}) if (q) { hipError_t e = hipStreamSynchronize(q); (void)e; }
    m->k.release(); m->ws.release(); m->ws_tail.release();
    for (int b = 0; b < 2; ++b) { m->swU[b].release(); m->swUr[b].release(); m->swXr[b].release(); }
    for (auto e : m->sw_ev) { hipError_t r = hipEventDestroy(e); (void)r; }
    for (auto e : m->sh_prof) { hipError_t r = hipEventDestroy(e); (void)r; }
    m->d_symv.release(); m->sh_send.release(); m->sh_recv.release(); m->sh_send1.release(); m->sh_recv1.release(); m->sh_fact.release();
    for (auto e : m->sh_ev) { hipError_t r = hipEventDestroy(e); (void)r; }
    if (m->tw) { m->tw->release(); delete m->tw; m->tw = nullptr; }
    m->oa.release();
    m->loo.release();
    m->cv.release();
    m->d_x.release(); m->d_y.release(); m->d_table.release(); m->d_kind.release(); m->d_shape.release();
    m->d_noise.release(); m->d_dvar.release(); m->d_z.release(); m->d_alpha.release(); m->d_zz.release();
    m->d_partial.release(); m->d_moments.release(); m->d_diagG.release(); m->d_tiles.release(); m->d_pair_start.release(); m->strip.release(); m->strip_own.release();
    m->d_tiles_head.release(); m->d_tiles_tail.release(); m->strip_head.release(); m->strip_tail.release();
    if (m->gram_ev) { hipError_t r = hipEventDestroy(m->gram_ev); (void)r; m->gram_ev = nullptr; }
    if (m->gram_tail_ev) { hipError_t r = hipEventDestroy(m->gram_tail_ev); (void)r; m->gram_tail_ev = nullptr; }
    m->d_chan_off.release(); m->d_flag.release(); m->d_info.release(); m->d_pivots.release(); m->acc_rhs.release();
    m->d_xs.release(); m->d_Ksf.release(); m->d_Vt.release(); m->d_mu.release(); m->d_var.release(); m->d_kdiag.release();
    m->d_Kss.release(); m->d_ptiles.release(); m->d_pred_tasks.release();
    m->ph_xx.release(); m->ph_sx.release(); m->ph_ss.release();
    if (m->h_pin) { hipError_t e = hipHostFree(m->h_pin); (void)e; m->h_pin = nullptr; }
    mean_release(m);

    delete m;
    return MOGP_OK;
}

int mogp_model_set_y(mogp_model* m, const double* y) {
    if (!m || !y) return fail(MOGP_EINVAL, "mogp_model_set_y: null argument");
    int rc;
    if ((rc = use_device(m->ctx))) return rc;
    std::vector<double> ys(m->Npad, 0.0);
    for (int64_t pos = 0; pos < m->N; ++pos) ys[pos] = y[m->sx.perm[pos]];
    if (m->mean_on) {
        HIP_TRY(dev_upload(m->d_y0.p, ys.data(), m->Npad * sizeof(double)));
        m->hy0 = ys;
        m->mean_g_valid = m->mean_g_pending = false;
        return mean_apply(m);
    }
    HIP_TRY(dev_upload(m->d_y.p, ys.data(), m->Npad * sizeof(double)));
    m->hy = ys;
    return MOGP_OK;
}

int mogp_model_set_terms_ex(mogp_model* m, int T, int width, const double* table) {
    if (!m || !table || T <= 0) return fail(MOGP_EINVAL, "mogp_model_set_terms: bad argument");
    if (width != 2 + 3 * m->D && width != 2 + 5 * m->D) return fail(MOGP_EINVAL, "mogp_model_set_terms: the row width must be 2 + 3 D or 2 + 5 D");
    int rc;
    if ((rc = use_device(m->ctx))) return rc;
    const int W = width;
    const size_t n = (size_t)m->C * m->C * T * W;
    for (size_t i = 0; i < n; ++i)
        if (!std::isfinite(table[i])) return fail(MOGP_ENONFINITE, "spectral term table has non-finite entries (kernel parameters diverged)");
    if (T != m->T) { m->radial = m->point_kinds = false; m->gate_kinds = 0; }
    m->T = T;
    m->Wt = W;
    if (m->tw) m->tw->pred_valid = false;
    m->table.assign(table, table + n);
    if ((rc = m->d_table.ensure(n))) return rc;
    if ((rc = m->d_moments.ensure((size_t)(m->C * (m->C + 1) / 2) * T * W))) return rc;
    HIP_TRY(hipMemcpyAsync(m->d_table.p, m->table.data(), n * sizeof(double), hipMemcpyHostToDevice, m->st));
    return MOGP_OK;
}

int mogp_model_set_terms(mogp_model* m, int T, const double* table) {
    if (!m) return fail(MOGP_EINVAL, "mogp_model_set_terms: bad argument");
    return mogp_model_set_terms_ex(m, T, 2 + 3 * m->D, table);
}

int mogp_model_set_kinds(mogp_model* m, int T, const int* kind, const double* shape) {
    if (!m) return fail(MOGP_EINVAL, "mogp_model_set_kinds: model is null");
    if (T != m->T || T <= 0) return fail(MOGP_EINVAL, "mogp_model_set_kinds: T must be that of the last mogp_model_set_terms");
    const size_t n = (size_t)m->C * m->C * T;
    bool any = false;
    if (const char* bad = check_kinds(kind, shape, m->C, m->D, T, &any)) return fail(MOGP_EINVAL, std::string("mogp_model_set_kinds: ") + bad);
    m->radial = false; m->point_kinds = false; m->gate_kinds = 0;
    if (!any) return MOGP_OK;
    if (m->Wt != 2 + 3 * m->D) return fail(MOGP_EINVAL, "mogp_model_set_kinds: radial profiles do not combine with enveloped term rows");
    m->hkind.assign(kind, kind + n);
    m->hshape.assign(shape, shape + n);
    for (size_t i = 0; i < n; ++i) {
        const int k = kind[i] & MOGP_KIND_MASK;
        m->point_kinds |= k == MOGP_KIND_DOT || k == MOGP_KIND_GATE || k == MOGP_KIND_WDOT;
    }
    m->gate_kinds = extra_rows(kind, n);
    int rc;
    if ((rc = use_device(m->ctx))) return rc;
    if ((rc = m->d_kind.ensure(n))) return rc;
    if ((rc = m->d_shape.ensure(n))) return rc;
    HIP_TRY(hipMemcpyAsync(m->d_kind.p, kind, n * sizeof(int), hipMemcpyHostToDevice, m->st));
    HIP_TRY(hipMemcpyAsync(m->d_shape.p, shape, n * sizeof(double), hipMemcpyHostToDevice, m->st));
    m->radial = true;
    return MOGP_OK;
}

int mogp_model_set_point_diag(mogp_model* m, const double* kdiag) {
    if (!m) return fail(MOGP_EINVAL, "mogp_model_set_point_diag: model is null");
    m->point_diag.clear();
    if (kdiag) {
        m->point_diag.resize(m->N);
        for (int64_t pos = 0; pos < m->N; ++pos) m->point_diag[pos] = kdiag[m->sx.perm[pos]];
    }
    return MOGP_OK;
}

int mogp_gram(mogp_ctx* ctx, int C, int D, int T, const double* table, int64_t M1, const double* X1,
              int64_t M2, const double* X2, double* K_out) {
    return mogp_gram_ex(ctx, C, D, T, 2 + 3 * D, table, M1, X1, M2, X2, K_out);
}

int mogp_gram_ex(mogp_ctx* ctx, int C, int D, int T, int width, const double* table, int64_t M1, const double* X1,
                 int64_t M2, const double* X2, double* K_out) {
    return mogp_gram_kinds(ctx, C, D, T, width, table, nullptr, nullptr, M1, X1, M2, X2, K_out);
// ... 222 lines not shown
```

mogptk_amd/csrc/mogp_internal.h:

```cpp
#pragma once
#include <hip/hip_runtime.h>
#include <stdint.h>
#include <atomic>
#include <string>
#include <vector>

#define MOGP_TILE 128
#define MOGP_GT 64
#define MOGP_TC 8
#define MOGP_MAXD 8

#define MOGP_KIND_GAUSS 0
#define MOGP_KIND_RQ 1
#define MOGP_KIND_MATERN12 2
#define MOGP_KIND_MATERN32 3
#define MOGP_KIND_MATERN52 4
#ifndef MOGP_KIND_PERIODIC
#define MOGP_KIND_PERIODIC 5
#endif
#ifndef MOGP_KIND_SINC
#define MOGP_KIND_SINC 6
#define MOGP_KIND_DOT 7
#define MOGP_DOT_DEGREE_MAX 8
#endif
#ifndef MOGP_KIND_GATE
#define MOGP_KIND_GATE 8
#endif
#ifndef MOGP_KIND_WDOT
#define MOGP_KIND_WDOT 9
#define MOGP_KIND_WHITE 10
#endif
#ifndef MOGP_KIND_TIMES
#define MOGP_KIND_TIMES (1 << 8)
#endif
#define MOGP_KIND_MASK 0xff
#define MOGP_GROUP_MAX 4

namespace mogp {
const char* check_kinds(const int* kind, const double* shape, int C, int D, int T, bool* any);
}

namespace mogp {

void set_error(const std::string& msg);
int hip_fail(hipError_t e, const char* what, const char* file, int line);
#define HIP_TRY(x)                                                        \
    do {                                                                  \
        hipError_t e__ = (x);                                             \
        if (e__ != hipSuccess) return mogp::hip_fail(e__, #x, __FILE__, __LINE__); \
    } while (0)

inline int set_max_dynamic_lds(const void* fn, int bytes, std::atomic<unsigned long long>& done) {
    int dev = 0;
    HIP_TRY(hipGetDevice(&dev));
    const unsigned long long bit = 1ull << (dev & 63);
    if (done.load(std::memory_order_acquire) & bit) return 0;
    HIP_TRY(hipFuncSetAttribute(fn, hipFuncAttributeMaxDynamicSharedMemorySize, bytes));
    done.fetch_or(bit, std::memory_order_release);
    return 0;
}

struct GTile {
    int r0, c0;
    int nr, nc;
    int pair;
    int flags;
    int rb, cb;
};
struct GSeg { int r0, c0, n, pair; int diag, pad[3]; };
enum { GT_MIRROR = 1,
       GT_DIAG = 2 };

struct PhaseRef {
    const int* offr = nullptr;
    const int* offc = nullptr;
    double* ws = nullptr;
};
size_t phase_ws_doubles(int C, int T, int64_t ldr, int64_t ldc);

struct GramArgs {
    const GTile* tiles;
    const double* xr;
    const double* xc;
    int64_t ldxr, ldxc;
    int64_t nrows, ncols;
    PhaseRef ph;
    const double* table;
    int T, D, C;
    int W;
    double* out;
    int64_t ldo;
    double* out2;
    const double* noise;
    const double* dvar;
    double jitter_abs;
    int mirror;
    hipEvent_t ev0, ev1;
    const GSeg* segs; int nsegs;
    const GTile* rest; int nrest;
    int dbg;
    int tab_lds;
    int phases_ready;
    const int* kind;
    const double* shape;
};

struct MomentArgs {
    const GTile* tiles;
    int ntiles;
    const double* x;
    int64_t ldx;
    const double* xc;
    int64_t ldxc;
    int64_t nrows, ncols;
    PhaseRef ph;
    const double* table;
    int T, D, C;
    int W;
    const double* kinv;
    int64_t ld;
    const double* alpha;
    double kinv_sign;
    int row_mod, row_rem;
    const double* G;
    int64_t ldg;
    const double* ru;
    const double* rw;
    double rcoef;
    int sym;
// ... 145 lines not shown
```

mogptk_amd/csrc/mogp_model.h:

```cpp
#pragma once
#include "../../include/mogp_hip.h"
#include "mogp_internal.h"

#include <algorithm>
#include <cmath>
#include <cstring>
#include <string>
#include <map>
#include <vector>

namespace mogp {

inline int dev_fill_zero(void* p, size_t bytes) {
    HIP_TRY(hipMemset(p, 0, bytes));
    HIP_TRY(hipStreamSynchronize(nullptr));
    return 0;
}

inline hipError_t dev_upload(void* dst, const void* src, size_t bytes) {
    hipError_t e = hipMemcpy(dst, src, bytes, hipMemcpyHostToDevice);
    return e != hipSuccess ? e : hipStreamSynchronize(nullptr);
}

template <typename T>
struct DevBuf {
    T* p = nullptr;
    size_t n = 0;
    bool borrowed = false;
    int ensure(size_t count) {
        if (count <= n) return 0;
        if (borrowed) { set_error("DevBuf: a borrowed range cannot grow"); return -1; }
        if (p) { hipError_t e = hipFree(p); (void)e; p = nullptr; n = 0; }
        HIP_TRY(hipMalloc(reinterpret_cast<void**>(&p), count * sizeof(T)));
        n = count;
        return 0;
    }
    void release() { if (p && !borrowed) { hipError_t e = hipFree(p); (void)e; } p = nullptr; n = 0; borrowed = false; }
};

struct RowBacked {
    static constexpr size_t GRAN = (size_t)2 << 20;
    char* base = nullptr;
    size_t bytes = 0, gran = GRAN;
    int device = 0;
    std::vector<hipMemGenericAllocationHandle_t> handle;
    std::vector<char> have;
    size_t nbacked = 0;
    int reserve(size_t nbytes, int dev) {
        release();
        bytes = (nbytes + gran - 1) / gran * gran;
        void* q = nullptr;
        HIP_TRY(hipMemAddressReserve(&q, bytes, gran, nullptr, 0));
        base = static_cast<char*>(q); device = dev;
        have.assign(bytes / gran, 0);
        handle.resize(bytes / gran);
        return 0;
    }
    int back(size_t off, size_t len) {
        if (len == 0) return 0;
        if (!base || off + len > bytes) { set_error("RowBacked::back: outside the reserved range"); return -1; }
        const size_t g_lo = off / gran, g_hi = (off + len - 1) / gran;
        hipMemAllocationProp prop{};
        prop.type = hipMemAllocationTypePinned; prop.location.type = hipMemLocationTypeDevice; prop.location.id = device;
        hipMemAccessDesc acc{};
        acc.location.type = hipMemLocationTypeDevice; acc.location.id = device; acc.flags = hipMemAccessFlagsProtReadWrite;
        for (size_t g = g_lo; g <= g_hi;) {
            if (have[g]) { ++g; continue; }
            size_t e = g;
            for (; e <= g_hi && !have[e]; ++e) {
                HIP_TRY(hipMemCreate(&handle[e], gran, &prop, 0));
                hipError_t me = hipMemMap(base + e * gran, gran, 0, handle[e], 0);
                if (me == hipSuccess) me = hipMemSetAccess(base + e * gran, gran, &acc, 1);
                if (me != hipSuccess) { hipError_t x = hipMemUnmap(base + e * gran, gran); x = hipMemRelease(handle[e]); (void)x; HIP_TRY(me); }
                have[e] = 1; ++nbacked;
            }
            { int z__ = dev_fill_zero(base + g * gran, (e - g) * gran); if (z__) return z__; }
            g = e;
        }
        return 0;
    }
    size_t backed_bytes() const { return nbacked * gran; }
    void release() {
        for (size_t g = 0; g < have.size(); ++g)
            if (have[g]) {
                hipError_t e = hipMemUnmap(base + g * gran, gran); (void)e;
                e = hipMemRelease(handle[g]); (void)e;
            }
        have.clear(); handle.clear(); nbacked = 0;
        if (base) { hipError_t e = hipMemAddressFree(base, bytes); (void)e; }
        base = nullptr; bytes = 0;
    }
};

struct PhaseWs {
    DevBuf<double> ws;
    DevBuf<int> offr, offc;
    std::vector<int> hr, hc;
    int prepare(const std::vector<int>& r, const std::vector<int>& c, int C, int T, int64_t ldr, int64_t ldc, hipStream_t s, PhaseRef& out) {
        int rc;
        if ((rc = ws.ensure(phase_ws_doubles(C, T, ldr, ldc)))) return rc;
        if (hr != r) {
            if ((rc = offr.ensure(r.size()))) return rc;
            hr = r;
            HIP_TRY(hipMemcpyAsync(offr.p, hr.data(), hr.size() * sizeof(int), hipMemcpyHostToDevice, s));
        }
        if (hc != c) {
            if ((rc = offc.ensure(c.size()))) return rc;
            hc = c;
            HIP_TRY(hipMemcpyAsync(offc.p, hc.data(), hc.size() * sizeof(int), hipMemcpyHostToDevice, s));
        }
        out.offr = offr.p; out.offc = offc.p; out.ws = ws.p;
        return 0;
    }
    void release() { ws.release(); offr.release(); offc.release(); hr.clear(); hc.clear(); }
};

struct SortedX {
    int64_t M = 0, Mpad = 0;
    std::vector<int64_t> perm;
    std::vector<int> off;
    std::vector<double> xs;
    bool identity = true;
};


int fail(int code, const std::string& msg);
static inline int64_t round_up(int64_t v, int64_t m) { return (v + m - 1) / m * m; }
int sort_inputs(const double* X, int64_t M, int D, int C, int64_t pad_to, SortedX& o);
void build_sym_tiles(const std::vector<int>& off, int C, std::vector<GTile>& tiles, std::vector<int>& pair_start);
void build_rect_tiles(const std::vector<int>& offr, const std::vector<int>& offc, int C, std::vector<GTile>& tiles,
                      std::vector<int>* pair_start = nullptr);

}

using namespace mogp;

enum { MOGP_COMM_NONE = 0, MOGP_COMM_RCCL = 1, MOGP_COMM_EXTERNAL = 2 };
struct mogp_comm {
    int kind = MOGP_COMM_NONE, rank = 0, n = 1;
    void* nccl = nullptr;
    mogp_allgather_cb allgather = nullptr;
    mogp_allreduce_cb allreduce = nullptr;
    void* user = nullptr;
};

struct mogp_ctx {
    int device = 0;
    mogp_comm comm;
    std::string name;
    hipStream_t st = nullptr, st2 = nullptr, st3 = nullptr, st4 = nullptr, st5 = nullptr, st_priv = nullptr, st2u = nullptr;
    bool streams_ready = false;
    bool chain_ok = true;
    struct SkWs { DevBuf<double> ws; DevBuf<unsigned> flags; unsigned epoch = 0; };
    std::map<hipStream_t, SkWs> sk;
    int ncu = 0, ncu_reserved = 0;
};

struct TrtriLevel {
    std::vector<GemmTask> h1, h2;
    DevBuf<GemmTask> d1, d2;
    double flops1 = 0, flops2 = 0;
};

#define MOGP_CHAIN_BOUND_TILES 160
#define MOGP_NPANEL 4
struct Spd {
    int64_t Npad = 0;
    int nb = 0;
    bool keep_L = false;
    bool refine_panels = false;
    DevBuf<double> pscr;
    DevBuf<double> A, B, invd, logdet;
    RowBacked Arows;
    bool owned_rows = false;
    DevBuf<double> Wm;
    std::vector<TrtriLevel> levels;
    std::vector<hipEvent_t> sync_ev;
    std::vector<hipEvent_t> row_ev;
    bool want_row_ev = false;
    std::vector<hipEvent_t> inv_ev;
    hipEvent_t fused_last_inv = nullptr, fused_last_wt = nullptr;
    DevBuf<double> Wd;
    DevBuf<double> Pb[MOGP_NPANEL];
    DevBuf<unsigned> chain_flags;
    DevBuf<double> Lm, Wt;
    FlowPlan flow;
    DevBuf<FlowTask> flow_tasks;
    DevBuf<int> flow_qmeta;
    FlowPlan flow_replay;
    DevBuf<FlowTask> flow_tasks_replay;
    DevBuf<int> flow_qmeta_replay;
    FlowPlan flow_rhs;
    DevBuf<FlowTask> flow_tasks_rhs;
    DevBuf<int> flow_qmeta_rhs;
    const FlowPlan* flow_cur = nullptr;
    DevBuf<unsigned> flow_flags;
    DevBuf<char> flow_args;
    std::vector<char> flow_args_h;
    DevBuf<unsigned char> flow_done;
    DevBuf<unsigned> flow_post;
    DevBuf<unsigned> flow_diag;
    DevBuf<unsigned long long> flow_trace;
    hipEvent_t tail_ready = nullptr;
    bool flow_used = false;
    bool want_vec = false, vec_done = false;
    const double* vec_y = nullptr; double* vec_z = nullptr; double* vec_zz = nullptr; double* vec_part = nullptr;
    void release() {
        for (auto& lv : levels) { lv.d1.release(); lv.d2.release(); }
        for (auto e : sync_ev) { hipError_t r = hipEventDestroy(e); (void)r; }
        for (auto e : row_ev) { hipError_t r = hipEventDestroy(e); (void)r; }
        row_ev.clear();
        for (auto e : inv_ev) { hipError_t r = hipEventDestroy(e); (void)r; }
        inv_ev.clear(); Wm.release(); Wd.release(); chain_flags.release(); for (auto& b : Pb) b.release();
        Lm.release(); Wt.release(); flow_tasks.release(); flow_qmeta.release(); flow_flags.release(); flow_args.release(); flow_args_h.clear(); flow_diag.release(); flow_post.release(); flow_done.release(); flow_trace.release(); flow = FlowPlan();
        flow_tasks_rhs.release(); flow_qmeta_rhs.release(); flow_rhs = FlowPlan(); flow_cur = nullptr;
        flow_tasks_replay.release(); flow_qmeta_replay.release(); flow_replay = FlowPlan();
        levels.clear(); sync_ev.clear();
        A.release(); B.release(); invd.release(); logdet.release(); pscr.release();
        Arows.release(); owned_rows = false;
    }
};

struct StripTiles {
    std::vector<mogp::GSeg> segs;
    std::vector<mogp::GTile> rest;
    mogp::DevBuf<mogp::GSeg> d_segs;
    mogp::DevBuf<mogp::GTile> d_rest;
    int build(const std::vector<mogp::GTile>& tiles);
    void attach(mogp::GramArgs& ga) const { ga.segs = d_segs.p; ga.nsegs = (int)segs.size(); ga.rest = d_rest.p; ga.nrest = (int)rest.size(); }
    void release() { d_segs.release(); d_rest.release(); }
};

struct TitsiasWork {
    int64_t Mpad = 0;
    Spd a, q;
    DevBuf<double> zx, B, v, GB, Qs, E, R, T1, GA, Hm;
    DevBuf<double> vec, scratch, gz, partial_uu, partial_uf, mom_uu, mom_uf, zero_noise;
    DevBuf<GTile> tiles_uu, tiles_uf;
    DevBuf<int> ps_uu, ps_uf;
    StripTiles strip_uf;
    std::vector<int> tile_key;
    size_t n_tuu = 0, n_tuf = 0;
    DevBuf<double> Kus, Aus, Bus;
    DevBuf<double> zero_col;
    DevBuf<double> kslices;
    DevBuf<double> red;
    const double* Wq = nullptr;
    SortedX pred_ss;
    bool pred_valid = false;
    hipEvent_t side_ev[2] = {nullptr, nullptr};
    hipEvent_t prod_ev[2] = {nullptr, nullptr};
    DevBuf<int> blk_z, blk_x;
    std::vector<int> hblk_z, hblk_x;
    DevBuf<double> gzp;
    SortedX sv_sz; bool sv_dense = false, sv_valid = false;
    DevBuf<double> kd_point;
    DevBuf<double> nvec;
    PhaseWs ph_zz, ph_zx, ph_zs;
    void release() {
        ph_zz.release(); ph_zx.release(); ph_zs.release();
        a.release(); q.release();
        zx.release(); B.release(); v.release(); GB.release(); Qs.release(); E.release(); R.release(); T1.release(); GA.release(); Hm.release();
        vec.release(); scratch.release(); gz.release(); partial_uu.release(); partial_uf.release(); mom_uu.release(); mom_uf.release();
        zero_noise.release(); tiles_uu.release(); tiles_uf.release(); ps_uu.release(); ps_uf.release(); strip_uf.release(); tile_key.clear();
        Kus.release(); Aus.release(); Bus.release(); zero_col.release(); kslices.release(); nvec.release(); kd_point.release(); red.release();
        blk_z.release(); blk_x.release(); gzp.release(); hblk_z.clear(); hblk_x.clear();
        for (auto& e : side_ev) if (e) { hipError_t r = hipEventDestroy(e); (void)r; e = nullptr; }
        for (auto& e : prod_ev) if (e) { hipError_t r = hipEventDestroy(e); (void)r; e = nullptr; }
    }
};

struct OaWork {
    mogp::DevBuf<double> K, Sc, Y, vec;
    bool valid = false;
    void release() { K.release(); Sc.release(); Y.release(); vec.release(); valid = false; }
};

struct LooWork {
    mogp::DevBuf<double> G, vec;
    void release() { G.release(); vec.release(); }
};

struct CvWork {
    mogp::DevBuf<int> off, idx;
    mogp::DevBuf<long long> foff;
    mogp::DevBuf<double> fac;
    std::vector<int> label;
    int64_t nfolds = 0;
    int mmax = 0;
    size_t fac_doubles = 0;
    hipEvent_t ev[4] = {nullptr, nullptr, nullptr, nullptr};
    bool timed = false;
    void release() {
        off.release(); idx.release(); foff.release(); fac.release(); label.clear(); nfolds = 0; mmax = 0; fac_doubles = 0;
        for (auto& e : ev) if (e) { hipError_t r = hipEventDestroy(e); (void)r; e = nullptr; }
        timed = false;
    }
};

struct FlowRhs { double* T; double* X; int nt; hipEvent_t ready; };
struct mogp_model {
    mogp_ctx* ctx = nullptr;
    int64_t N = 0, Npad = 0;
    int nb = 0, D = 0, C = 0, T = 0;
    int Wt = 0;
    std::vector<double> point_diag;
    SortedX sx;
    std::vector<GTile> tiles;
    std::vector<int> pair_start;
    std::vector<double> table;
    int gate_kinds = 0;
    bool radial = false;
    mogp::DevBuf<int> d_kind;
    std::vector<int> hkind;
    mogp::DevBuf<double> d_shape;
    std::vector<double> hshape;
    bool point_kinds = false;
    hipStream_t st = nullptr;
    hipStream_t st2 = nullptr;
    hipStream_t st2u = nullptr;
    hipStream_t st3 = nullptr;
    hipStream_t st4 = nullptr;
    hipStream_t st_priv = nullptr;
    Spd k;
    Spd ws, ws_tail;
    DevBuf<double> swU[2], swUr[2];
    DevBuf<double> swXr[2];
    std::vector<hipEvent_t> sw_ev;
    int sh_rank = 0, sh_n = 1;
    bool sh_owned = false;
    int backed_rank = -1, backed_n = 0;
    std::vector<GTile> tiles_own;
    std::vector<int> pair_start_own;
    DevBuf<GTile> d_tiles_own;
    bool factor_only = false;
    hipEvent_t pred_ev[2] = {nullptr, nullptr};
    StripTiles strip, strip_own;
    std::vector<GTile> tiles_head, tiles_tail;
    DevBuf<GTile> d_tiles_head, d_tiles_tail;
    StripTiles strip_head, strip_tail;
    hipEvent_t gram_ev = nullptr, gram_tail_ev = nullptr;
    DevBuf<int> d_pair_start_own;
    int own_rank = -1, own_n = 0;
    DevBuf<double> sh_send, sh_recv;
    DevBuf<double> sh_send1, sh_recv1;
    DevBuf<double> sh_fact;
    bool sh_factor_once = false;
    bool sh_split = false;
    std::vector<hipEvent_t> sh_ev;
    std::vector<hipEvent_t> sh_prof;
    double sh_ms[6] = {0, 0, 0, 0, 0, 0};
    int sh_prof_blocks = 0;
    double sh_jabs = 0.0;
    bool sh_dvar = false;

    std::vector<double> hy;
    DevBuf<double> d_symv;
    DevBuf<double> d_x, d_y, d_table, d_noise, d_dvar, d_z, d_alpha, d_zz, d_partial, d_moments, d_diagG;
    DevBuf<GTile> d_tiles;
    std::vector<GemmTask> kinv_acc_tasks, kinv_lauum_tasks;
    std::vector<int> kinv_prefix;
    DevBuf<GemmTask> d_kinv_acc, d_kinv_lauum;
    std::vector<double> blk_cen, blk_half;
    bool kinv_sparse = false;
    double kinv_fraction = 1.0;
    DevBuf<int> d_pair_start, d_chan_off, d_flag;
    DevBuf<double> d_pivots;
    bool accurate = false, accurate_ran = false;
    DevBuf<double> acc_rhs;
    double pivot_min = 0.0, pivot_max = 0.0;
    DevBuf<unsigned long long> d_info;

    DevBuf<double> d_xs, d_Ksf, d_Vt, d_mu, d_var, d_kdiag, d_Kss;
    DevBuf<GTile> d_ptiles;
    DevBuf<GemmTask> d_pred_tasks;
    PhaseWs ph_xx, ph_sx, ph_ss;

    double* h_pin = nullptr;
    size_t h_pin_n = 0;

    bool profiling = false;
    std::vector<hipEvent_t> ev;
    std::vector<hipEvent_t> gemm_ev;
    size_t gemm_ev_used = 0;
    double ms[MOGP_ST_COUNT] = {0};
    int64_t gemm_launches = 0;
    double gemm_flops = 0.0;
    bool have_W = false, have_Kinv = false, kinv_in_A = false, w_in_Wm = false;
    bool flow_ran = false;
    const FlowRhs* rhs_job = nullptr;
    bool replay_flow = false;
    bool no_flow = false;
    long long n_fact = 0, flow_retry_at = 0;
    int flow_backoff = 64, flow_timeouts = 0;
    double flow_enqueue_us = 0.0, flow_enqueue_us_max = 0.0;
    bool no_chain = false;
    TitsiasWork* tw = nullptr;
    OaWork oa;
    LooWork loo;
    CvWork cv;

    bool mean_on = false, mean_g_valid = false, mean_g_pending = false;
    std::vector<double> mean_coef, mean_g, hy0;
    DevBuf<double> d_y0, d_mean_coef, d_mean_part, d_mean_g;
    double* h_mean_pin = nullptr;
    hipEvent_t mean_ev = nullptr;
    const double* mean_w = nullptr;
    double mean_w_scale = 0.0;
};


namespace mogp {
int use_device(mogp_ctx* c);
int gemm_call(mogp_model* m, const GemmArgs& g, double flops, hipStream_t st = nullptr);
int mark(mogp_model* m, int idx);
double table_diag(const mogp_model* m, int c);
double table_diag_points(const mogp_model* m, const SortedX& pts);
int mean_apply(mogp_model* m);
int mean_grad_enqueue(mogp_model* m, const double* w, double scale);
void mean_grad_collect(mogp_model* m);
void mean_release(mogp_model* m);
int spd_alloc(Spd& w, int64_t Npad, int owned_rows_device = -1);
int spd_make_whole(Spd& w);
inline GemmArgs make_gemm(const double* A, int64_t lda, int akm, const double* B, int64_t ldb, int bkm, double* C, int64_t ldc,
                          double alpha, int mode, int mt, int nt, int64_t K) {
    GemmArgs g{};
    g.A = A; g.lda = lda; g.a_kmajor = akm; g.B = B; g.ldb = ldb; g.b_kmajor = bkm; g.C = C; g.ldc = ldc;
    g.alpha = alpha; g.beta = 0.0; g.mode = mode; g.mt = mt; g.nt = nt; g.K = (int)K;
    return g;
}
int side_fork(mogp_model* m, TitsiasWork& t, hipStream_t* side);
int side_join(mogp_model* m, TitsiasWork& t, hipStream_t side);
int gz_prepare(mogp_model* m, TitsiasWork& t, const std::vector<int>& offz, int D);
void gz_attach(const TitsiasWork& t, MomentArgs& ma, bool zx);
int spd_check_info(mogp_model* m, const char* which, int64_t* info);
int spd_info_verdict(mogp_model* m, const char* which, unsigned long long hinfo, int64_t* info);
int sparse_timeout_check(mogp_model* m);
bool chain_enabled(const mogp_model* m);
int chain_fallback(mogp_model* m);
int spd_invert(mogp_model* m, Spd& w, const char* which, int64_t* info, const double** W, bool defer_check = false);
int mm_lower_splitk(mogp_model* m, TitsiasWork& t, const double* A, const double* B, double* out, int mt, int64_t Mpad, int64_t ldk, int64_t K,
                    double alpha = 1.0);
int launch_scale_cols(const double* in, double* out, int64_t ld, int64_t rows, int64_t n, const double* s, hipStream_t st);
int sparse_workspace(mogp_model* m, TitsiasWork& t, int64_t Mpad);
int sparse_tiles(mogp_model* m, TitsiasWork& t, const SortedX& sz, bool want_uf);
int sparse_kuu(mogp_model* m, int64_t M, const double* Z, double jitter, bool want_uf, SortedX& sz, double* jit, const char* need_grouped = nullptr);
int sparse_kuf(mogp_model* m, TitsiasWork& t, const SortedX& sz, hipStream_t stream, bool use_strips, double* out2);
int refined_apply(mogp_model* m, TitsiasWork& t, const double* P, const double* Q, const double* rhs, double* out);
int allreduce_vec_scalars(mogp_model* m, TitsiasWork& t, double* vec, int64_t n, double* hs, int k);
int adjoint_GA(mogp_model* m, TitsiasWork& t, double scale, hipStream_t stream);
int solve_with_rider(mogp_model* m, TitsiasWork& t, double* panel, const double* r, double* beta);
struct MomentSpec { const double* G; int64_t ldg; const double* ru; const double* rw; double rcoef; bool dz; };
int sparse_moments(mogp_model* m, TitsiasWork& t, const SortedX& sz, const MomentSpec* uf, const MomentSpec& uu, bool sharded, hipStream_t side);
int sparse_predict_panels(mogp_model* m, TitsiasWork& t, const SortedX& sz, int64_t S, const double* Xs, SortedX& ss);
int sparse_point_stats(mogp_model* m, TitsiasWork& t, const SortedX& pts, const double* a, const double* b, const double* mu_panel,
                       const double* mu_vec, double mu_div, const double* kdiag, double* mu, double* var);
int sparse_predict_finish(mogp_model* m, TitsiasWork& t, const SortedX& ss, const double* mu_panel, const double* mu_vec, double mu_div,
                          const double* kss_diag, double* mu, double* var);
#define MOGP_RETRY_NO_CHAIN 0x7e7e
extern int g_outer;
int begin_call(mogp_model* m, int64_t* info, bool one_gpu);
int exact_begin(mogp_model* m, const double* noise_var, const double* data_var, double jitter, GramArgs& ga, double& jabs);
int report_not_pd(unsigned long long hinfo, int64_t* info);
struct TestSide { SortedX ss; int64_t Spad = 0; int ntiles = 0; };
int test_side(mogp_model* m, int64_t S, const double* Xs, const double* kss_diag, int64_t extra_rows, hipStream_t st, TestSide& ts, GramArgs& ga);
inline void scatter_by_perm(const SortedX& ss, const double* sorted, double* out) { for (int64_t pos = 0; pos < ss.M; ++pos) out[ss.perm[pos]] = sorted[pos]; }
int moment_pass_device(mogp_model* m, const double* kinv, double ksign);
int moment_pass(mogp_model* m, const double* kinv, double ksign, double* moments, double* diagG);
void collect_timing(mogp_model* m, int last_mark);
enum { LOO_MU = 0, LOO_VAR, LOO_A, LOO_B, LOO_SA, LOO_TERM, LOO_RHO, LOO_SUM, LOO_COUNT };
int loo_workspace(mogp_model* m, bool grad);
int loo_points(mogp_model* m, double* kinv);
int loo_adjoint(mogp_model* m, const double* kinv, double* scratch);
int loo_moment_pass(mogp_model* m);
int launch_loo_sum(const double* term, int64_t n, double* out, hipStream_t st);
int launch_loo_rank2(double* G, int64_t ld, int64_t n, const double* alpha, const double* rho, hipStream_t st);
int cv_workspace(mogp_model* m, const int32_t* fold, int64_t nfolds, bool grad);
int cv_points(mogp_model* m, double* kinv, bool grad);
int cv_adjoint(mogp_model* m, const double* kinv, double* scratch);
size_t cv_bytes(const mogp_model* m);
int eval_sweep(mogp_model* m, const double* noise_var, const double* data_var, double jitter, double* lml, double* jitter_abs, int64_t* info);
void one_gpu_call(mogp_model* m);
int ensure_system(mogp_model* m);
int spd_potrf(mogp_model* m, Spd& w, long long info_base = 0);
int spd_potri_fused(mogp_model* m, Spd& w);
bool flow_enabled(const mogp_model* m, const Spd& w);
int launch_flow_alpha_sum(const Spd& w, double* alpha, hipStream_t st);
int spd_potri_flow(mogp_model* m, Spd& w, const FlowRhs* rhs = nullptr);
void flow_debug_dump(mogp_model* m);
int spd_potri_fused_finish(mogp_model* m, Spd& w);
int spd_trtri(mogp_model* m, Spd& w);
int spd_lauum(mogp_model* m, Spd& w);
int spd_sweep(mogp_model* m, Spd& w);
int sweep_prepare(mogp_model* m, Spd& w);
int sweep_nblocks(const Spd& w);
int sweep_block(mogp_model* m, Spd& w, int kb, hipEvent_t* prof = nullptr, hipEvent_t panel_ready = nullptr, hipEvent_t* stall = nullptr);
int sweep_finish(mogp_model* m, Spd& w);
int trsm_lower(mogp_model* m, const double* L, int64_t ldl, int nb, double* B, int64_t ldb, int64_t ncols, bool trans, hipStream_t st = nullptr, bool tri = false,
               const hipEvent_t* row_ready = nullptr);
int launch_transpose(double* dst, const double* src, int64_t ld, int64_t n, hipStream_t s);
int launch_sym_lower_avg(double* A, int64_t ld, int64_t n, double scale, hipStream_t s);
int comm_allgather(mogp_ctx* ctx, const double* send, double* recv, int64_t count, hipStream_t st);
int comm_allreduce(mogp_ctx* ctx, double* buf, int64_t count, hipStream_t st);
int shard_pack(mogp_model* m, Spd& w, int kb, double** send, double** recv, int64_t* count);
int shard_unpack(mogp_model* m, Spd& w, int kb);
int shard_pack_part(mogp_model* m, Spd& w, int kb, int part, DevBuf<double>& sendb, DevBuf<double>& recvb, int64_t* count, hipStream_t st);
int shard_unpack_part(mogp_model* m, Spd& w, int kb, int part, DevBuf<double>& recvb, hipStream_t st);
int shard_factor_bcast(mogp_model* m, Spd& w, Spd& s, int k0, int nk, bool mine, hipStream_t st);
}
```

mogptk_amd/csrc/oa.hip:

```cpp
#include "mogp_model.h"

#include <cmath>
#include <cstring>
#include <limits>

using namespace mogp;

#define RC(x) do { int r__ = (x); if (r__) return r__; } while (0)

namespace {

__global__ void k_oa_scale(const double* __restrict__ K, double* __restrict__ A, int64_t ld, const double* __restrict__ lam) {
    const int64_t i = blockIdx.x;
    const int64_t jend = (i / MOGP_TILE + 1) * MOGP_TILE;
    const double li = lam[i];
    for (int64_t j = threadIdx.x; j < jend; j += blockDim.x) {
        const int64_t lo = j <= i ? i * ld + j : j * ld + i;
        A[i * ld + j] = li * lam[j] * K[lo] + (i == j ? 1.0 : 0.0);
    }
}

__global__ void k_oa_rowstats(const double* __restrict__ Binv, int64_t ld, int64_t n, const double* __restrict__ d,
                              double* __restrict__ s_out, double* __restrict__ r_out) {
    const int64_t i = blockIdx.x;
// ... 10 lines not shown
        __syncthreads();
    }
    if (threadIdx.x == 0) { s_out[i] = rs[0]; r_out[i] = rr[0]; }
}

__global__ void k_oa_adjoint(double* __restrict__ Y, const double* __restrict__ Binv, int64_t ld, int64_t n, const double* __restrict__ lam,
                             const double* __restrict__ nu, const double* __restrict__ e) {
    const int64_t j = (int64_t)blockIdx.x * blockDim.x + threadIdx.x;
    if (j >= n) return;
    const int64_t i = blockIdx.y;
    Y[i * ld + j] = lam[i] * lam[j] * (Y[i * ld + j] - 0.5 * Binv[i * ld + j]) + 0.5 * (e[i] * nu[j] + nu[i] * e[j] - nu[i] * nu[j]);
}


enum { V_NU = 0, V_LAM, V_MU, V_B, V_E, V_F, V_D, V_W, V_S, V_R, V_EN, V_GNU, V_COUNT };

int upload_sorted(mogp_model* m, const double* src, double* dst, double pad) {
    std::vector<double> h(m->Npad, pad);
    for (int64_t pos = 0; pos < m->N; ++pos) h[pos] = src[m->sx.perm[pos]];
    HIP_TRY(dev_upload(dst, h.data(), m->Npad * sizeof(double)));
    return 0;
}

}

extern "C" {

int mogp_oa_forward(mogp_model* m, const double* q_nu, const double* q_lambda, double* mu, double* var, double* kl, int64_t* info) {
    if (m) m->mean_w = nullptr;
    if (!m || !q_nu || !q_lambda || !mu || !var || !kl) return fail(MOGP_EINVAL, "mogp_oa_forward: bad argument");
    RC(use_device(m->ctx));
    if (info) *info = 0;
    const int C = m->C, D = m->D;
    const int64_t N = m->N, Npad = m->Npad;
    if (m->T <= 0) return fail(MOGP_EINVAL, "mogp_model_set_terms must be called before an evaluation");
    if (m->Wt != 2 + 3 * D) return fail(MOGP_EINVAL, "the Opper-Archambeau path does not take terms with an envelope (MOHSM): exact inference only");
    for (int64_t i = 0; i < N; ++i)
        if (!(q_lambda[i] > 0.0)) return fail(MOGP_EINVAL, "mogp_oa_forward: q_lambda must be positive");
    OaWork& o = m->oa;
    o.valid = false;
    one_gpu_call(m);
    RC(ensure_system(m));
    m->have_W = m->have_Kinv = false;
    m->kinv_sparse = false;
    m->gemm_ev_used = 0; m->gemm_launches = 0; m->gemm_flops = 0.0;
    RC(o.K.ensure((size_t)Npad * Npad));
    RC(o.vec.ensure((size_t)V_COUNT * Npad));
    const int nchunks = (int)((Npad + 511) / 512);
    RC(m->d_symv.ensure((size_t)(4 + nchunks) * Npad));
    double* nu = o.vec.p + V_NU * Npad;
    double* lam = o.vec.p + V_LAM * Npad;
    RC(upload_sorted(m, q_nu, nu, 0.0));
    RC(upload_sorted(m, q_lambda, lam, 0.0));
    const unsigned long long big = std::numeric_limits<unsigned long long>::max();
    HIP_TRY(hipMemcpyAsync(m->d_info.p, &big, sizeof(big), hipMemcpyHostToDevice, m->st));

    GramArgs ga{};
    ga.tiles = m->d_tiles.p; ga.xr = m->d_x.p; ga.xc = m->d_x.p; ga.ldxr = ga.ldxc = Npad; ga.nrows = ga.ncols = N;
    RC(m->ph_xx.prepare(m->sx.off, m->sx.off, C, m->T, Npad, Npad, m->st, ga.ph));
    ga.table = m->d_table.p; ga.T = m->T; ga.D = D; ga.C = C; ga.W = m->Wt;
    ga.out = o.K.p; ga.ldo = Npad; ga.noise = nullptr; ga.dvar = nullptr; ga.jitter_abs = 0.0; ga.mirror = 0;
    m->strip.attach(ga);
    RC(launch_gram(ga, (int)m->tiles.size(), m->st));
    RC(launch_pad_identity(o.K.p, Npad, N, Npad, m->st));
    double* dmu = o.vec.p + V_MU * Npad;
    RC(launch_symv_lower(o.K.p, Npad, Npad, nu, dmu, m->d_symv.p, 1.0, m->st, 0, 0));
    std::vector<double> hmu(Npad), hb(Npad), hl(m->nb);
    HIP_TRY(hipMemcpyAsync(hmu.data(), dmu, Npad * sizeof(double), hipMemcpyDeviceToHost, m->st));
    hipLaunchKernelGGL(k_oa_scale, dim3((unsigned)Npad), dim3(256), 0, m->st, o.K.p, m->k.A.p, Npad, lam);
    HIP_TRY(hipGetLastError());
    if (m->nb <= (flow_enabled(m, m->k) ? 112 : 80)) {
        RC(spd_potri_fused(m, m->k));
        RC(spd_potri_fused_finish(m, m->k));
    } else {
        RC(spd_potrf(m, m->k)); RC(spd_trtri(m, m->k)); RC(spd_lauum(m, m->k));
    }
    RC(launch_symmetrize(m->k.B.p, Npad, Npad, m->st));
    double* db = o.vec.p + V_B * Npad;
    RC(launch_get_diag(m->k.B.p, Npad, Npad, db, m->st));
    unsigned long long hinfo = 0;
    HIP_TRY(hipMemcpyAsync(hb.data(), db, Npad * sizeof(double), hipMemcpyDeviceToHost, m->st));
    HIP_TRY(hipMemcpyAsync(hl.data(), m->k.logdet.p, m->nb * sizeof(double), hipMemcpyDeviceToHost, m->st));
    HIP_TRY(hipMemcpyAsync(&hinfo, m->d_info.p, sizeof(hinfo), hipMemcpyDeviceToHost, m->st));
    HIP_TRY(hipStreamSynchronize(m->st));
    if (hinfo == MOGP_INFO_CHAIN_TIMEOUT) {
        RC(chain_fallback(m));
        return mogp_oa_forward(m, q_nu, q_lambda, mu, var, kl, info);
    }
    if (hinfo != big) {
        if (info) *info = (int64_t)hinfo;
        return fail(MOGP_ENOTPD, "linalg.cholesky: The factorization could not be completed because the input is not "
                                 "positive-definite (the leading minor of order " + std::to_string(hinfo) + " is not positive-definite).");
    }
    double logdet = 0.0, tr = 0.0, maha = 0.0;
    for (double v : hl) logdet += v;
    for (int64_t pos = 0; pos < N; ++pos) {
        const int64_t dst = m->sx.perm[pos];
        mu[dst] = hmu[pos];
        var[dst] = (1.0 - hb[pos]) / (q_lambda[dst] * q_lambda[dst]);
        tr += hb[pos];
        maha += q_nu[dst] * hmu[pos];
    }
    *kl = maha + 2.0 * logdet + tr - (double)N;
    o.valid = true;
    return MOGP_OK;
}
// ... 70 lines not shown
```

mogptk_amd/csrc/shard.hip:

```cpp
#include "mogp_model.h"
#include <cstdlib>
#include <limits>

using namespace mogp;

static int sweep_eval_begin(mogp_model* m, const double* noise_var, const double* data_var, double jitter) {
    const int64_t N = m->N, Npad = m->Npad;
    GramArgs ga{};
    int rc = exact_begin(m, noise_var, data_var, jitter, ga, m->sh_jabs);
    if (rc) return rc;
    m->sh_dvar = data_var != nullptr;
    if (m->radial) return fail(MOGP_EINVAL, "the sweep / sharded evaluation does not take radial kinds (mogp_model_set_kinds)");
    const bool own = m->sh_n > 1 && m->own_n == m->sh_n && m->own_rank == m->sh_rank;
    if (own) ga.tiles = m->d_tiles_own.p;
    (own ? m->strip_own : m->strip).attach(ga);
    if ((rc = launch_gram(ga, (int)(own ? m->tiles_own.size() : m->tiles.size()), m->st))) return rc;
    if (!(m->sh_owned && m->sh_n > 1 && (m->nb - 1) % m->sh_n != m->sh_rank))
        if ((rc = launch_pad_identity(m->k.A.p, Npad, N, Npad, m->st))) return rc;
    return mark(m, 1);
}

static int sweep_eval_alpha(mogp_model* m) {
    const int64_t Npad = m->Npad;
    int rc;
// ... 153 lines not shown
    { const char* e = std::getenv("MOGP_SHARD_FACTOR_ONCE"); m->sh_factor_once = c.n > 1 && e && std::atoi(e) != 0; }
    const int PEV = 10;
    if (m->profiling) {
        while ((int)m->sh_prof.size() < PEV * nblocks) { hipEvent_t e; HIP_TRY(hipEventCreate(&e)); m->sh_prof.push_back(e); }
        m->sh_prof_blocks = nblocks;
    }
    while ((int)m->sh_ev.size() < 2 * nblocks) { hipEvent_t e; HIP_TRY(hipEventCreateWithFlags(&e, hipEventDisableTiming)); m->sh_ev.push_back(e); }
    hipStream_t qc = m->st3;
    for (int kb = 0; kb < nblocks; ++kb) {
        int64_t count = 0;
        hipEvent_t* pe = m->profiling ? m->sh_prof.data() + PEV * kb : nullptr;
        if (pe) HIP_TRY(hipEventRecord(pe[0], m->st));
        if (!m->sh_split) {
            double *send = nullptr, *recv = nullptr;
            if ((rc = shard_pack(m, m->k, kb, &send, &recv, &count))) return rc;
            if ((rc = comm_allgather(m->ctx, send, recv, count, m->st))) return rc;
            if ((rc = shard_unpack(m, m->k, kb))) return rc;
            if (pe) HIP_TRY(hipEventRecord(pe[1], m->st));
            if ((rc = sweep_block(m, m->k, kb, pe ? pe + 2 : nullptr))) return rc;
            continue;
        }
        hipEvent_t packed = m->sh_ev[2 * kb], rest_in = m->sh_ev[2 * kb + 1];
        int64_t count2 = 0;
        if ((rc = shard_pack_part(m, m->k, kb, 1, m->sh_send1, m->sh_recv1, &count, m->st))) return rc;
        if ((rc = shard_pack_part(m, m->k, kb, 2, m->sh_send, m->sh_recv, &count2, m->st))) return rc;
        HIP_TRY(hipEventRecord(packed, m->st));
        if ((rc = comm_allgather(m->ctx, m->sh_send1.p, m->sh_recv1.p, count, m->st))) return rc;
        if ((rc = shard_unpack_part(m, m->k, kb, 1, m->sh_recv1, m->st))) return rc;
        if (pe) HIP_TRY(hipEventRecord(pe[1], m->st));
        HIP_TRY(hipStreamWaitEvent(qc, packed, 0));
        if (pe) HIP_TRY(hipEventRecord(pe[6], qc));
        if ((rc = comm_allgather(m->ctx, m->sh_send.p, m->sh_recv.p, count2, qc))) return rc;
        if ((rc = shard_unpack_part(m, m->k, kb, 2, m->sh_recv, qc))) return rc;
        if (pe) HIP_TRY(hipEventRecord(pe[7], qc));
        HIP_TRY(hipEventRecord(rest_in, qc));
        if ((rc = sweep_block(m, m->k, kb, pe ? pe + 2 : nullptr, rest_in, pe ? pe + 8 : nullptr))) return rc;
    }
    if ((rc = sweep_finish(m, m->k))) return rc;
    if ((rc = sweep_eval_alpha(m))) return rc;
    return comm_allreduce(m->ctx, m->d_alpha.p, m->Npad, m->st);
}

int mogp_exact_eval_sharded(mogp_model* m, const double* noise_var, const double* data_var, double jitter,
                            double* lml, double* moments, double* diagG, double* trG, double* jitter_abs, int64_t* info) {
    if (!m || !lml || !moments || !diagG || !trG) return fail(MOGP_EINVAL, "mogp_exact_eval_sharded: bad argument");
    int rc;
    if ((rc = begin_call(m, info, false))) return rc;
    const int C = m->C, W = m->Wt, T = m->T, P = C * (C + 1) / 2;
    m->pivot_min = m->pivot_max = 0.0;
    if ((rc = sharded_inverse(m, noise_var, data_var, jitter, jitter_abs))) return rc;
    if ((rc = mark(m, 5))) return rc;
    if ((rc = moment_pass_device(m, m->k.A.p, -1.0))) return rc;
    if ((rc = comm_allreduce(m->ctx, m->d_moments.p, (int64_t)P * T * W, m->st))) return rc;
    if ((rc = comm_allreduce(m->ctx, m->d_diagG.p, C, m->st))) return rc;
    HIP_TRY(hipMemcpyAsync(moments, m->d_moments.p, (size_t)P * T * W * sizeof(double), hipMemcpyDeviceToHost, m->st));
    HIP_TRY(hipMemcpyAsync(diagG, m->d_diagG.p, C * sizeof(double), hipMemcpyDeviceToHost, m->st));
    if ((rc = sweep_eval_scalars(m, lml, info))) return sharded_rc(m, rc);
    if (m->sh_prof_blocks > 0) {
        for (hipStream_t q : {m->st2, m->st2u}) if (q) HIP_TRY(hipStreamSynchronize(q));
        if (m->st3) HIP_TRY(hipStreamSynchronize(m->st3));
        double acc6[6] = {0, 0, 0, 0, 0, 0};
        for (int kb = 0; kb < m->sh_prof_blocks; ++kb) {
            hipEvent_t* pe = m->sh_prof.data() + 10 * kb;
            const int a_[6] = {0, 1, 2, 4, 6, 8}, b_[6] = {1, 2, 3, 5, 7, 9};
            for (int i = 0; i < 6; ++i) {
                if (i >= 4 && !m->sh_split) continue;
                float t = 0.f;
                if (hipEventElapsedTime(&t, pe[a_[i]], pe[b_[i]]) == hipSuccess) acc6[i] += t;
            }
        }
        for (int i = 0; i < 6; ++i) m->sh_ms[i] = acc6[i];
    }
    double tr = 0.0;
    for (int c = 0; c < C; ++c) tr += diagG[c];
    *trG = tr;
    m->have_Kinv = true; m->kinv_in_A = true;
    collect_timing(m, 6);
    return MOGP_OK;
}

__global__ __launch_bounds__(256) void k_owned_quadform(const double* __restrict__ Ksf, int64_t ldk, const double* __restrict__ T, int64_t ldt, int64_t S,
                                                        int nown, int P, int rank, double* __restrict__ part) {
    const int lane = threadIdx.x & 63, wave = threadIdx.x >> 6;
    const int64_t s = (int64_t)blockIdx.x * 4 + wave;
    if (s >= S) return;
    double acc = 0.0;
    for (int j = 0; j < nown; ++j) {
        const double* kr = Ksf + s * ldk + (int64_t)(rank + j * P) * MOGP_TILE;
        const double* tr = T + s * ldt + (int64_t)j * MOGP_TILE;
        acc = fma(kr[lane], tr[lane], acc);
        acc = fma(kr[lane + 64], tr[lane + 64], acc);
    }
#pragma unroll
    for (int off = 32; off > 0; off >>= 1) acc += __shfl_down(acc, off, 64);
    if (lane == 0) part[s] = acc;
}
__global__ void k_var_finish(const double* __restrict__ kdiag, const double* __restrict__ part, int64_t S, double* __restrict__ var) {
    const int64_t i = (int64_t)blockIdx.x * blockDim.x + threadIdx.x;
    if (i < S) var[i] = kdiag[i] + part[i];
}

int mogp_exact_predict_sharded(mogp_model* m, const double* noise_var, const double* data_var, double jitter,
                               const double* kss_diag, int64_t S, const double* Xs, double* mu, double* var, int64_t* info) {
    if (!m || !Xs || !mu || !var || !kss_diag || S <= 0) return fail(MOGP_EINVAL, "mogp_exact_predict_sharded: bad argument");
    int rc;
    if ((rc = begin_call(m, info, false))) return rc;
    mogp_comm& cm = m->ctx->comm;
    const int P = cm.n, rank = cm.rank, nb = m->nb;
    const int64_t Npad = m->Npad;
// ... 72 lines not shown
```

mogptk_amd/csrc/sparse.hip:

```cpp
#include "mogp_model.h"

#include <cmath>
#include <cstdlib>
#include <cstring>
#include <limits>

using namespace mogp;

#define RC(x) do { int r__ = (x); if (r__) return r__; } while (0)

namespace {

__global__ void k_scale_cols(const double* __restrict__ in, double* __restrict__ out, int64_t ld, int64_t n, const double* __restrict__ s) {
    const int64_t j = (int64_t)blockIdx.x * blockDim.x + threadIdx.x;
    if (j >= n) return;
    const int64_t r = blockIdx.y;
    out[r * ld + j] = in[r * ld + j] * s[j];
}

}

namespace mogp {

int launch_scale_cols(const double* in, double* out, int64_t ld, int64_t rows, int64_t n, const double* s, hipStream_t st) {
// ... 127 lines not shown
        t.Mpad = Mpad;
        RC(spd_alloc(t.a, Mpad)); RC(spd_alloc(t.q, Mpad));
        RC(t.zx.ensure((size_t)D * Mpad));
        RC(t.B.ensure((size_t)Mpad * Npad)); RC(t.v.ensure((size_t)Mpad * Npad));
        RC(t.Qs.ensure((size_t)Mpad * Mpad));
        RC(t.vec.ensure((size_t)8 * Mpad + 4 * Npad));
        RC(t.scratch.ensure((size_t)(Mpad / 256 + 2) * std::max(Npad, Mpad) + (size_t)(Mpad / 512 + 2) * Mpad));
        RC(t.zero_noise.ensure(C));
        RC(dev_fill_zero(t.zero_noise.p, C * sizeof(double)));
        RC(dev_fill_zero(t.B.p, (size_t)Mpad * Npad * sizeof(double)));
        RC(dev_fill_zero(t.v.p, (size_t)Mpad * Npad * sizeof(double)));
    }
    return 0;
}

int sparse_tiles(mogp_model* m, TitsiasWork& t, const SortedX& sz, bool want_uf) {
    std::vector<int> key(sz.off);
    key.insert(key.end(), m->sx.off.begin(), m->sx.off.end());
    key.push_back(1);
    if (key == t.tile_key) return 0;
    if (!want_uf) { key.back() = 0; if (key == t.tile_key) return 0; }
    t.tile_key.clear();
    std::vector<GTile> tuu, tuf;
    std::vector<int> psuu, psuf;
    build_sym_tiles(sz.off, m->C, tuu, psuu);
    if (want_uf) build_rect_tiles(sz.off, m->sx.off, m->C, tuf, &psuf);
    HIP_TRY(hipStreamSynchronize(m->st));
    RC(t.tiles_uu.ensure(tuu.size())); RC(t.ps_uu.ensure(psuu.size()));
    HIP_TRY(dev_upload(t.tiles_uu.p, tuu.data(), tuu.size() * sizeof(GTile)));
    HIP_TRY(dev_upload(t.ps_uu.p, psuu.data(), psuu.size() * sizeof(int)));
    if (want_uf) {
        RC(t.tiles_uf.ensure(tuf.size())); RC(t.ps_uf.ensure(psuf.size()));
        HIP_TRY(dev_upload(t.tiles_uf.p, tuf.data(), tuf.size() * sizeof(GTile)));
        HIP_TRY(dev_upload(t.ps_uf.p, psuf.data(), psuf.size() * sizeof(int)));
        RC(t.strip_uf.build(tuf));
    }
    t.n_tuu = tuu.size(); t.n_tuf = tuf.size();
    t.tile_key = key;
    return 0;
}

int sparse_kuu(mogp_model* m, int64_t M, const double* Z, double jitter, bool want_uf, SortedX& sz, double* jit, const char* need_grouped) {
    const int C = m->C, D = m->D, W = m->Wt;
    if (m->T <= 0) return fail(MOGP_EINVAL, "mogp_model_set_terms must be called before an evaluation");
    RC(sort_inputs(Z, M, D, C, MOGP_TILE, sz));
    if (need_grouped && !sz.identity) return fail(MOGP_EINVAL, need_grouped);
    const int64_t Mpad = sz.Mpad;
    if (!m->tw) m->tw = new TitsiasWork();
    TitsiasWork& t = *m->tw;
    RC(sparse_workspace(m, t, Mpad));
    m->gemm_ev_used = 0; m->gemm_launches = 0; m->gemm_flops = 0.0;
    HIP_TRY(hipMemcpyAsync(t.zx.p, sz.xs.data(), (size_t)D * Mpad * sizeof(double), hipMemcpyHostToDevice, m->st));
    RC(sparse_tiles(m, t, sz, want_uf));
    const unsigned long long big = std::numeric_limits<unsigned long long>::max();
    HIP_TRY(hipMemcpyAsync(m->d_info.p, &big, sizeof(big), hipMemcpyHostToDevice, m->st));

    *jit = jitter * table_diag_points(m, sz) / (double)M;

    GramArgs ga{};
    ga.tiles = t.tiles_uu.p; ga.xr = t.zx.p; ga.xc = t.zx.p; ga.ldxr = ga.ldxc = Mpad; ga.nrows = ga.ncols = M;
    RC(t.ph_zz.prepare(sz.off, sz.off, C, m->T, Mpad, Mpad, m->st, ga.ph));
    ga.table = m->d_table.p; ga.T = m->T; ga.D = D; ga.C = C; ga.W = W; ga.out = t.a.A.p; ga.ldo = Mpad;
    ga.noise = t.zero_noise.p; ga.dvar = nullptr; ga.jitter_abs = *jit; ga.mirror = 0;
    RC(launch_gram(ga, (int)t.n_tuu, m->st));
    RC(launch_pad_identity(t.a.A.p, Mpad, M, Mpad, m->st));
    t.a.keep_L = true;
    t.a.refine_panels = !(std::getenv("MOGP_REFINE_PANELS") && std::atoi(std::getenv("MOGP_REFINE_PANELS")) == 0);
    return 0;
}

int sparse_kuf(mogp_model* m, TitsiasWork& t, const SortedX& sz, hipStream_t stream, bool use_strips, double* out2) {
    const int64_t Mpad = t.Mpad, Npad = m->Npad;
    GramArgs ga{};
    ga.tiles = t.tiles_uf.p; ga.xr = t.zx.p; ga.ldxr = Mpad; ga.xc = m->d_x.p; ga.ldxc = Npad; ga.nrows = sz.M; ga.ncols = m->N;
    RC(t.ph_zx.prepare(sz.off, m->sx.off, m->C, m->T, Mpad, Npad, stream, ga.ph));
    ga.table = m->d_table.p; ga.T = m->T; ga.D = m->D; ga.C = m->C; ga.W = m->Wt; ga.out = t.B.p; ga.ldo = Npad; ga.mirror = 0;
    ga.out2 = out2;
    if (use_strips) t.strip_uf.attach(ga);
    return launch_gram(ga, (int)t.n_tuf, stream);
}

int refined_apply(mogp_model* m, TitsiasWork& t, const double* P, const double* Q, const double* rhs, double* out) {
    const int64_t Mpad = t.Mpad;
    double* tmp = t.vec.p + 5 * Mpad;
    double* res = t.vec.p + 6 * Mpad;
    RC(launch_gemv_rows(P, Mpad, Mpad, Mpad, rhs, out, m->st));
    RC(launch_gemv_rows(Q, Mpad, Mpad, Mpad, out, tmp, m->st));
    RC(launch_axpby(Mpad, 1.0, rhs, -1.0, tmp, res, m->st));
    RC(launch_gemv_rows(P, Mpad, Mpad, Mpad, res, tmp, m->st));
    RC(launch_axpby(Mpad, 1.0, out, 1.0, tmp, out, m->st));
    return 0;
}

int allreduce_vec_scalars(mogp_model* m, TitsiasWork& t, double* vec, int64_t n, double* hs, int k) {
    RC(t.red.ensure((size_t)n + k));
    if (n) HIP_TRY(hipMemcpyAsync(t.red.p, vec, n * sizeof(double), hipMemcpyDeviceToDevice, m->st));
    HIP_TRY(hipMemcpyAsync(t.red.p + n, hs, k * sizeof(double), hipMemcpyHostToDevice, m->st));
    HIP_TRY(hipStreamSynchronize(m->st));
    RC(comm_allreduce(m->ctx, t.red.p, n + k, m->st));
    if (n) HIP_TRY(hipMemcpyAsync(vec, t.red.p, n * sizeof(double), hipMemcpyDeviceToDevice, m->st));
    HIP_TRY(hipMemcpyAsync(hs, t.red.p + n, k * sizeof(double), hipMemcpyDeviceToHost, m->st));
    HIP_TRY(hipStreamSynchronize(m->st));
    return 0;
}

int adjoint_GA(mogp_model* m, TitsiasWork& t, double scale, hipStream_t stream) {
// ... 122 lines not shown
```

Measured before the change: 96.84.

## Pre-arm next evaluation's flag resets and move tail readbacks to side stream

Several latency-trimming changes land together. The flow/chain flag and zz memsets for the next gradient evaluation are enqueued on the bulk stream at the end of the current one ("arming"). Pivot, logdet, zz and info readbacks move to a side stream gated on inversion events. The tail Gram launch is deferred into a callback run by the factorization. Moments and diagG are merged into one buffer so a single D2H copy suffices, the phase-centre workspace is reused across calls, and the kinv sparsity plan skips tiles already marked. This cuts per-call launch and synchronization overhead, but adds cross-call state whose invalidation must be handled correctly in every path.

```diff
diff --git a/mogptk_amd/csrc/exact.hip b/mogptk_amd/csrc/exact.hip
--- a/mogptk_amd/csrc/exact.hip
+++ b/mogptk_amd/csrc/exact.hip
@@ -44,6 +44,10 @@
     const int nblk = (int)(m->blk_cen.size() / std::max(D, 1));
     std::vector<char> need((size_t)nb * nb, 0);
     for (const GTile& t : m->tiles) {
+        const int i0 = t.r0 / MOGP_TILE, i1 = (t.r0 + t.nr - 1) / MOGP_TILE, j0 = t.c0 / MOGP_TILE, j1 = (t.c0 + t.nc - 1) / MOGP_TILE;
+        bool marked = true;
+        for (int i = i0; i <= i1 && marked; ++i) for (int j = j0; j <= j1; ++j) if (j <= i && !need[(size_t)i * nb + j]) { marked = false; break; }
+        if (marked) continue;
         const double* tab = m->table.data() + (size_t)t.pair * T * W;
         bool read = false;
         for (int k = 0; k < T && !read; ++k) {
@@ -57,10 +61,13 @@
             read = !(0.5 * emin > 52.0);
         }
         if (!read) continue;
-        const int i0 = t.r0 / MOGP_TILE, i1 = (t.r0 + t.nr - 1) / MOGP_TILE, j0 = t.c0 / MOGP_TILE, j1 = (t.c0 + t.nc - 1) / MOGP_TILE;
         for (int i = i0; i <= i1; ++i) for (int j = j0; j <= j1; ++j) if (j <= i) need[(size_t)i * nb + j] = 1;
     }
     for (int i = 0; i < nb; ++i) need[(size_t)i * nb + i] = 1;
+    size_t nneed = 0;
+    for (int i = 0; i < nb; ++i) for (int j = 0; j <= i; ++j) nneed += need[(size_t)i * nb + j] ? 1 : 0;
+    m->kinv_fraction = (double)nneed / ((double)nb * (nb + 1) / 2);
+    if (m->kinv_fraction > 0.85) return 0;
     std::vector<GemmTask> acc, lau;
     std::vector<int> prefix(nb + 1, 0);
     for (int i = 0; i < nb; ++i) {
@@ -77,9 +84,6 @@
         }
         prefix[i + 1] = (int)acc.size();
     }
-    const double frac = (double)acc.size() / ((double)nb * (nb + 1) / 2);
-    m->kinv_fraction = frac;
-    if (frac > 0.85) return 0;
     const bool same = acc.size() == m->kinv_acc_tasks.size() && (acc.empty() || std::memcmp(acc.data(), m->kinv_acc_tasks.data(), acc.size() * sizeof(GemmTask)) == 0);
     if (!same || m->d_kinv_acc.n < acc.size()) {
         int rc;
@@ -111,12 +115,37 @@
 };
 
 namespace mogp {
+int arm_drop(mogp_model* m) {
+    Armed& a = m->arm;
+    if (a.enq) HIP_TRY(hipStreamWaitEvent(m->st, a.ev, 0));
+    a.enq = a.valid = a.want = a.live = false;
+    return 0;
+}
+
 int begin_call(mogp_model* m, int64_t* info, bool one_gpu) {
     m->mean_w = nullptr;
     if (int rc = use_device(m->ctx)) return rc;
+    if (int rc = arm_drop(m)) return rc;
+    m->tail_side = nullptr;
     if (info) *info = 0;
     if (one_gpu) one_gpu_call(m);
     return 0;
+}
+
+static int tail_join(mogp_model* m, bool& pending) {
+    pending = m->tail_side != nullptr;
+    if (pending) HIP_TRY(hipEventRecord(m->tail_ev[1], m->tail_side));
+    m->tail_side = nullptr;
+    return 0;
+}
+static int tail_wait(mogp_model* m) {
+    static const bool spin = !(std::getenv("MOGP_SPIN_WAIT") && std::atoi(std::getenv("MOGP_SPIN_WAIT")) == 0);
+    if (!spin) { HIP_TRY(hipEventSynchronize(m->tail_ev[1])); return 0; }
+    for (;;) {
+        const hipError_t e = hipEventQuery(m->tail_ev[1]);
+        if (e == hipSuccess) return 0;
+        if (e != hipErrorNotReady) return hip_fail(e, "hipEventQuery", __FILE__, __LINE__);
+    }
 }
 
 int exact_begin(mogp_model* m, const double* noise_var, const double* data_var, double jitter, GramArgs& ga, double& jabs) {
@@ -144,14 +173,14 @@
         HIP_TRY(hipMemcpyAsync(m->d_dvar.p, dv.data(), Npad * sizeof(double), hipMemcpyHostToDevice, m->st));
     }
     jabs = jitter * dsum / (double)N;
-    HIP_TRY(hipMemcpyAsync(m->d_noise.p, noise_var, C * sizeof(double), hipMemcpyHostToDevice, m->st));
-    static const unsigned long long big = std::numeric_limits<unsigned long long>::max();
-    HIP_TRY(hipMemcpyAsync(m->d_info.p, &big, sizeof(big), hipMemcpyHostToDevice, m->st));
+    std::memcpy(m->h_up, noise_var, C * sizeof(double));
+    HIP_TRY(hipMemcpyAsync(m->d_noise.p, m->h_up, C * sizeof(double), hipMemcpyHostToDevice, m->st));
+    if (!m->arm.live) HIP_TRY(hipMemsetAsync(m->d_info.p, 0xff, sizeof(unsigned long long), m->st));
     int rc;
     if ((rc = mark(m, 0))) return rc;
     ga = GramArgs{};
     ga.tiles = m->d_tiles.p; ga.xr = m->d_x.p; ga.xc = m->d_x.p; ga.ldxr = ga.ldxc = Npad; ga.nrows = ga.ncols = N;
-    if ((rc = m->ph_xx.prepare(m->sx.off, m->sx.off, C, m->T, Npad, Npad, m->st, ga.ph))) return rc;
+    if ((rc = m->ph_xx.prepare_fixed(m->sx.off, C, m->T, Npad, m->st, ga.ph))) return rc;
     ga.table = m->d_table.p; ga.T = m->T; ga.D = m->D; ga.C = C; ga.W = m->Wt;
     ga.out = m->k.A.p; ga.ldo = Npad; ga.noise = m->d_noise.p; ga.dvar = data_var ? m->d_dvar.p : nullptr;
     ga.jitter_abs = jabs; ga.mirror = 0;
@@ -161,6 +190,7 @@
 }
 
 namespace mogp { int chain_fallback(mogp_model* m) {
+    m->arm.valid = m->arm.live = false;
     if (m->flow_ran) {
         m->no_flow = true; m->flow_ran = false;
         m->flow_timeouts++;
@@ -257,13 +287,14 @@
         gt.tiles = m->d_tiles_tail.p; m->strip_tail.attach(gt); gt.ev0 = nullptr; gt.phases_ready = 1;
         if ((rc = launch_gram(gh, (int)m->tiles_head.size(), m->st, m->radial ? m->gate_kinds : 0))) return rc;
         if ((rc = launch_pad_identity(m->k.A.p, Npad, N, Npad, m->st))) return rc;
-        if (!m->gram_ev) HIP_TRY(hipEventCreateWithFlags(&m->gram_ev, hipEventDisableTiming));
-        HIP_TRY(hipEventRecord(m->gram_ev, m->st));
-        HIP_TRY(hipStreamWaitEvent(m->st2, m->gram_ev, 0));
-        if ((rc = launch_gram(gt, (int)m->tiles_tail.size(), m->st2, m->radial ? m->gate_kinds : 0))) return rc;
         if (!m->gram_tail_ev) HIP_TRY(hipEventCreateWithFlags(&m->gram_tail_ev, hipEventDisableTiming));
-        HIP_TRY(hipEventRecord(m->gram_tail_ev, m->st2));
-        m->k.tail_ready = m->gram_tail_ev;
+        const int ntail = (int)m->tiles_tail.size(), rows = m->radial ? m->gate_kinds : 0;
+        m->k.bulk_first = [m, gt, ntail, rows]() -> int {
+            if (int r = launch_gram(gt, ntail, m->st2, rows)) return r;
+            HIP_TRY(hipEventRecord(m->gram_tail_ev, m->st2));
+            m->k.tail_ready = m->gram_tail_ev;
+            return 0;
+        };
     } else {
         if ((rc = launch_gram(ga, (int)m->tiles.size(), m->st, m->radial ? m->gate_kinds : 0))) return rc;
         if ((rc = launch_pad_identity(m->k.A.p, Npad, N, Npad, m->st))) return rc;
@@ -275,6 +306,7 @@
     if ((rc = pin_ensure(m, pl.total))) return rc;
     if ((rc = m->d_pivots.ensure(2))) return rc;
     if (m->accurate && (rc = m->acc_rhs.ensure((size_t)Npad * MOGP_TILE))) return rc;
+    for (hipEvent_t* e : {&m->tail_ev[0], &m->tail_ev[1], &m->arm.ev, &m->arm.scal_ev}) if (!*e) HIP_TRY(hipEventCreateWithFlags(e, hipEventDisableTiming));
     m->k.flow_used = false;
     m->flow_ran = false;
     m->k.want_vec = fuse_inverse;
@@ -286,6 +318,10 @@
     else rc = fuse_inverse ? spd_potri_fused(m, m->k) : spd_potrf(m, m->k);
     m->k.keep_L = m->k.refine_panels = false;
     m->k.want_vec = false; m->k.tail_ready = nullptr;
+    if (m->k.bulk_first) {
+        m->k.bulk_first = nullptr;
+        if (!rc) rc = fail(MOGP_EHIP, "factorize: the second Gram launch was never enqueued");
+    }
     if (rc) return rc;
     if ((rc = mark(m, 2))) return rc;
     if (accurate) {
@@ -340,13 +376,47 @@
     }
 
     const int nzz = (int)pl.nzz;
-    if ((rc = launch_pivot_range(m->k.invd.p, N, m->d_pivots.p, m->st))) return rc;
-    HIP_TRY(hipMemcpyAsync(m->h_pin + pl.pivots, m->d_pivots.p, 2 * sizeof(double), hipMemcpyDeviceToHost, m->st));
-    HIP_TRY(hipMemcpyAsync(m->h_pin + pl.logdet, m->k.logdet.p, m->nb * sizeof(double), hipMemcpyDeviceToHost, m->st));
+    static const bool aside_on = !(std::getenv("MOGP_TAIL_ASIDE") && std::atoi(std::getenv("MOGP_TAIL_ASIDE")) == 0);
+    const bool dataflow_grad = m->arm.want && plan.defer && fuse_inverse && m->k.flow_used && m->k.vec_done;
+    hipStream_t ss = m->st;
+    if (dataflow_grad && aside_on && m->st3 && m->k.inv_ev.size() >= 3) {
+        ss = m->tail_side = m->st3;
+        static const bool fault_hook = std::getenv("MOGP_FLOW_FAULT") && std::atoi(std::getenv("MOGP_FLOW_FAULT")) != 0;
+        if (fault_hook) {
+            HIP_TRY(hipEventRecord(m->tail_ev[0], m->st));
+            HIP_TRY(hipStreamWaitEvent(ss, m->tail_ev[0], 0));
+        } else {
+            HIP_TRY(hipStreamWaitEvent(ss, m->k.inv_ev[1], 0));
+            HIP_TRY(hipStreamWaitEvent(ss, m->k.inv_ev[2], 0));
+        }
+    }
+    if ((rc = launch_pivot_range(m->k.invd.p, N, m->d_pivots.p, ss))) return rc;
+    HIP_TRY(hipMemcpyAsync(m->h_pin + pl.pivots, m->d_pivots.p, 2 * sizeof(double), hipMemcpyDeviceToHost, ss));
+    HIP_TRY(hipMemcpyAsync(m->h_pin + pl.logdet, m->k.logdet.p, m->nb * sizeof(double), hipMemcpyDeviceToHost, ss));
     static const int zz_piece = []() { const char* e = std::getenv("MOGP_D2H_CHUNK"); const int v = e ? std::atoi(e) : 2048; return v > 0 ? v : (1 << 30); }();
     for (int o = 0; o < nzz; o += zz_piece)
-        HIP_TRY(hipMemcpyAsync(m->h_pin + pl.zz + o, m->d_zz.p + o, std::min(zz_piece, nzz - o) * sizeof(double), hipMemcpyDeviceToHost, m->st));
-    HIP_TRY(hipMemcpyAsync(m->h_pin + pl.info, m->d_info.p, sizeof(unsigned long long), hipMemcpyDeviceToHost, m->st));
+        HIP_TRY(hipMemcpyAsync(m->h_pin + pl.zz + o, m->d_zz.p + o, std::min(zz_piece, nzz - o) * sizeof(double), hipMemcpyDeviceToHost, ss));
+    HIP_TRY(hipMemcpyAsync(m->h_pin + pl.info, m->d_info.p, sizeof(unsigned long long), hipMemcpyDeviceToHost, ss));
+
+    static const bool arm_on = !(std::getenv("MOGP_PREARM") && std::atoi(std::getenv("MOGP_PREARM")) == 0) && !std::getenv("MOGP_FLOW_DEBUG") && !std::getenv("MOGP_FLOW_TRACE");
+    if (dataflow_grad && arm_on && !m->replay_flow && m->k.flow_cur == &m->k.flow && m->st2 && m->k.inv_ev.size() >= 3) {
+        Armed& a = m->arm;
+        hipStream_t bulk = m->st2;
+        const FlowPlan& p = m->k.flow;
+        HIP_TRY(hipEventRecord(a.scal_ev, ss));
+        HIP_TRY(hipStreamWaitEvent(bulk, a.scal_ev, 0));
+        HIP_TRY(hipStreamWaitEvent(bulk, m->k.inv_ev[1], 0));
+        HIP_TRY(hipStreamWaitEvent(bulk, m->k.inv_ev[2], 0));
+        a.chain_p = m->k.chain_flags.p; a.chain_n = (size_t)(p.nouter + 1) * MOGP_CHAIN_FLAGS;
+        a.flow_p = m->k.flow_flags.p; a.nflags = (size_t)p.nflags;
+        a.zz_p = m->d_zz.p; a.nzz = pl.nzz;
+        HIP_TRY(hipMemsetAsync(m->k.chain_flags.p, 0, a.chain_n * sizeof(unsigned), bulk));
+        HIP_TRY(hipMemsetAsync(m->k.flow_flags.p, 0, (size_t)p.base_err * sizeof(unsigned), bulk));
+        HIP_TRY(hipMemsetAsync(m->d_zz.p, 0, a.nzz * sizeof(double), bulk));
+        HIP_TRY(hipMemsetAsync(m->d_info.p, 0xff, sizeof(unsigned long long), bulk));
+        HIP_TRY(hipEventRecord(a.ev, bulk));
+        a.enq = true;
+    }
     if (ga_out) *ga_out = ga;
     if (plan.defer) return 0;
     HIP_TRY(hipStreamSynchronize(m->st));
@@ -391,7 +461,7 @@
     ma.ev0 = prof_event(m, 9); ma.ev1 = prof_event(m, 10);
     if ((rc = launch_moments(ma, m->st, m->radial ? m->gate_kinds : 0))) return rc;
     if ((rc = launch_moment_reduce(m->d_partial.p, own ? m->d_pair_start_own.p : m->d_pair_start.p, P, T, W, D, m->d_moments.p, m->st))) return rc;
-    if ((rc = launch_diagG(kinv, Npad, m->d_alpha.p, m->d_chan_off.p, C, m->d_diagG.p, m->st, ksign, rm, m->sh_rank))) return rc;
+    if ((rc = launch_diagG(kinv, Npad, m->d_alpha.p, m->d_chan_off.p, C, m->diagG_dev(), m->st, ksign, rm, m->sh_rank))) return rc;
     if ((rc = mean_grad_enqueue(m, m->d_alpha.p, -1.0))) return rc;
     return mark(m, 6);
 }
@@ -401,7 +471,7 @@
     int rc;
     if ((rc = moment_pass_device(m, kinv, ksign))) return rc;
     HIP_TRY(hipMemcpyAsync(moments, m->d_moments.p, (size_t)P * T * W * sizeof(double), hipMemcpyDeviceToHost, m->st));
-    HIP_TRY(hipMemcpyAsync(diagG, m->d_diagG.p, C * sizeof(double), hipMemcpyDeviceToHost, m->st));
+    HIP_TRY(hipMemcpyAsync(diagG, m->diagG_dev(), C * sizeof(double), hipMemcpyDeviceToHost, m->st));
     HIP_TRY(hipStreamSynchronize(m->st));
     return 0;
 }
@@ -466,10 +536,12 @@
                     double* lml, double* moments, double* diagG, double* trG, double* jitter_abs, int64_t* info) {
     if (!m) return fail(MOGP_EINVAL, "mogp_exact_eval: model is null");
     int rc;
+    const bool was_armed = m->arm.enq && m->arm.valid;
     if ((rc = begin_call(m, info, true))) return rc;
     const std::string& grad_path = grad_path_env();
     const bool sweep = grad_path == "sweep" && (flags & MOGP_EVAL_GRAD);
     const bool grad = (flags & MOGP_EVAL_GRAD) != 0;
+    if (grad && !sweep) { m->arm.want = true; m->arm.live = was_armed; }
     GramArgs ga{};
     auto again = [&]() { return mogp_exact_eval(m, noise_var, data_var, jitter, flags, lml, moments, diagG, trG, jitter_abs, info); };
     if (grad && (!moments || !diagG || !trG)) return fail(MOGP_EINVAL, "mogp_exact_eval: gradient outputs are null");
@@ -491,11 +563,14 @@
         if ((rc = moment_pass(m, kinv, ksign, moments, diagG))) return rc;
     } else {
         if ((rc = moment_pass_device(m, kinv, ksign))) return rc;
+        bool side_pending = false;
+        if ((rc = tail_join(m, side_pending))) return rc;
         const PinLayout pl(m);
-        HIP_TRY(hipMemcpyAsync(m->h_pin + pl.moments, m->d_moments.p, (size_t)P * T * W * sizeof(double), hipMemcpyDeviceToHost, m->st));
-        HIP_TRY(hipMemcpyAsync(m->h_pin + pl.diagG, m->d_diagG.p, C * sizeof(double), hipMemcpyDeviceToHost, m->st));
+        HIP_TRY(hipMemcpyAsync(m->h_pin + pl.moments, m->d_moments.p, ((size_t)P * T * W + C) * sizeof(double), hipMemcpyDeviceToHost, m->st));
         if ((rc = wait_stream(m->st))) return rc;
+        if (side_pending && (rc = tail_wait(m))) return rc;
         if ((rc = factorize_finish(m, ga, lml, info))) return retry_on_streams(m, rc, again);
+        m->arm.valid = m->arm.enq;
         std::memcpy(moments, m->h_pin + pl.moments, (size_t)P * T * W * sizeof(double));
         std::memcpy(diagG, m->h_pin + pl.diagG, C * sizeof(double));
     }
@@ -533,8 +608,7 @@
         m->have_W = false;
         if ((rc = loo_adjoint(m, m->k.B.p, m->k.A.p))) return rc;
         if ((rc = loo_moment_pass(m))) return rc;
-        HIP_TRY(hipMemcpyAsync(m->h_pin + pl.moments, m->d_moments.p, (size_t)P * T * W * sizeof(double), hipMemcpyDeviceToHost, m->st));
-        HIP_TRY(hipMemcpyAsync(m->h_pin + pl.diagG, m->d_diagG.p, C * sizeof(double), hipMemcpyDeviceToHost, m->st));
+        HIP_TRY(hipMemcpyAsync(m->h_pin + pl.moments, m->d_moments.p, ((size_t)P * T * W + C) * sizeof(double), hipMemcpyDeviceToHost, m->st));
     }
     HIP_TRY(hipMemcpyAsync(m->h_pin + pin_loo, v + LOO_SUM * Npad, sizeof(double), hipMemcpyDeviceToHost, m->st));
     HIP_TRY(hipMemcpyAsync(m->h_pin + pin_mu, v + LOO_MU * Npad, N * sizeof(double), hipMemcpyDeviceToHost, m->st));
@@ -582,8 +656,7 @@
         m->have_W = false;
         if ((rc = cv_adjoint(m, m->k.B.p, m->k.A.p))) return rc;
         if ((rc = loo_moment_pass(m))) return rc;
-        HIP_TRY(hipMemcpyAsync(m->h_pin + pl.moments, m->d_moments.p, (size_t)P * T * W * sizeof(double), hipMemcpyDeviceToHost, m->st));
-        HIP_TRY(hipMemcpyAsync(m->h_pin + pl.diagG, m->d_diagG.p, C * sizeof(double), hipMemcpyDeviceToHost, m->st));
+        HIP_TRY(hipMemcpyAsync(m->h_pin + pl.moments, m->d_moments.p, ((size_t)P * T * W + C) * sizeof(double), hipMemcpyDeviceToHost, m->st));
     }
     HIP_TRY(hipMemcpyAsync(m->h_pin + pin_cv, v + LOO_SUM * Npad, sizeof(double), hipMemcpyDeviceToHost, m->st));
     HIP_TRY(hipMemcpyAsync(m->h_pin + pin_mu, v + LOO_MU * Npad, N * sizeof(double), hipMemcpyDeviceToHost, m->st));
diff --git a/mogptk_amd/csrc/flow.hip b/mogptk_amd/csrc/flow.hip
--- a/mogptk_amd/csrc/flow.hip
+++ b/mogptk_amd/csrc/flow.hip
@@ -735,30 +735,8 @@
     const FlowPlan& p = plan;
     const int nouter = p.nouter;
     if ((rc = w.chain_flags.ensure((size_t)(nouter + 1) * MOGP_CHAIN_FLAGS))) return rc;
-    HIP_TRY(hipMemsetAsync(w.chain_flags.p, 0, (size_t)(nouter + 1) * MOGP_CHAIN_FLAGS * sizeof(unsigned), crit));
-    HIP_TRY(hipMemsetAsync(w.flow_flags.p, 0, (size_t)p.nflags * sizeof(unsigned), crit));
-    if (replay) {
-        std::vector<unsigned> preset((size_t)p.nflags, 0u);
-        for (const FlowPlan::Chain& c : p.chain) preset[c.done_idx] = c.expect;
-        HIP_TRY(hipMemcpyAsync(w.flow_flags.p, preset.data(), preset.size() * sizeof(unsigned), hipMemcpyHostToDevice, crit));
-        HIP_TRY(hipStreamSynchronize(crit));
-    }
-    if (!rhs && w.want_vec && w.vec_zz) HIP_TRY(hipMemsetAsync(w.vec_zz, 0, (size_t)((ld + 3) / 4) * sizeof(double), crit));
     static const bool want_trace = std::getenv("MOGP_FLOW_TRACE") && std::atoi(std::getenv("MOGP_FLOW_TRACE")) != 0;
-    if (want_trace) {
-        if ((rc = w.flow_trace.ensure(FLOW_TRACE_W * p.tasks.size() + 4 * (size_t)nouter))) return rc;
-        HIP_TRY(hipMemsetAsync(w.flow_trace.p, 0, w.flow_trace.n * sizeof(unsigned long long), crit));
-    }
-    while ((int)w.inv_ev.size() < 4) {
-        hipEvent_t e;
-        HIP_TRY(hipEventCreateWithFlags(&e, hipEventDisableTiming));
-        w.inv_ev.push_back(e);
-    }
-    hipEvent_t start = w.inv_ev[0], e_flow = w.inv_ev[1], e_chain = w.inv_ev[2];
-    HIP_TRY(hipEventRecord(start, crit));
-    HIP_TRY(hipStreamWaitEvent(bulk, start, 0));
-    HIP_TRY(hipStreamWaitEvent(priv, start, 0));
-
+    if (want_trace && (rc = w.flow_trace.ensure(FLOW_TRACE_W * p.tasks.size() + 4 * (size_t)nouter))) return rc;
     static std::atomic<unsigned long long> attr_done{0ull};
     static std::atomic<unsigned long long> attr_done_dbg{0ull};
     { int r__ = set_max_dynamic_lds(reinterpret_cast<const void*>(k_flow<false>), FL_LDS_BYTES, attr_done); if (r__) return r__; }
@@ -799,9 +777,7 @@
         if (m->gemm_ev_used + 2 > m->gemm_ev.size())
             for (int i = 0; i < 64; ++i) { hipEvent_t e; HIP_TRY(hipEventCreate(&e)); m->gemm_ev.push_back(e); }
         pe0 = m->gemm_ev[m->gemm_ev_used++]; pe1 = m->gemm_ev[m->gemm_ev_used++];
-        HIP_TRY(hipEventRecord(pe0, bulk));
-    }
-    if (rhs && rhs->ready) HIP_TRY(hipStreamWaitEvent(bulk, rhs->ready, 0));
+    }
     const bool dbg_kernel = g.post != nullptr || g.trace != nullptr;
     static_assert(sizeof(FlowArgs) <= 512, "Spd::flow_args slots");
     if ((rc = w.flow_args.ensure(1024))) return rc;
@@ -818,6 +794,53 @@
         return 0;
     };
     if ((rc = upload(0, g, bulk))) return rc;
+
+    const size_t chain_words = (size_t)(nouter + 1) * MOGP_CHAIN_FLAGS, zz_n = (size_t)((ld + 3) / 4);
+    const bool zz_here = !rhs && w.want_vec && w.vec_zz;
+    const Armed& ar = m->arm;
+    const bool armed = ar.live && &w == &m->k && &plan == &w.flow && !want_trace && zz_here && ar.chain_p == w.chain_flags.p && ar.chain_n == chain_words &&
+                       ar.flow_p == w.flow_flags.p && ar.nflags == (size_t)p.nflags && ar.zz_p == w.vec_zz && ar.nzz == zz_n;
+    m->arm.live = false;
+    if (!armed) {
+        HIP_TRY(hipMemsetAsync(w.chain_flags.p, 0, chain_words * sizeof(unsigned), crit));
+        HIP_TRY(hipMemsetAsync(w.flow_flags.p, 0, (size_t)p.nflags * sizeof(unsigned), crit));
+    }
+    if (replay) {
+        std::vector<unsigned> preset((size_t)p.nflags, 0u);
+        for (const FlowPlan::Chain& c : p.chain) preset[c.done_idx] = c.expect;
+        HIP_TRY(hipMemcpyAsync(w.flow_flags.p, preset.data(), preset.size() * sizeof(unsigned), hipMemcpyHostToDevice, crit));
+        HIP_TRY(hipStreamSynchronize(crit));
+    }
+    if (zz_here && !armed) HIP_TRY(hipMemsetAsync(w.vec_zz, 0, zz_n * sizeof(double), crit));
+    if (want_trace) HIP_TRY(hipMemsetAsync(w.flow_trace.p, 0, w.flow_trace.n * sizeof(unsigned long long), crit));
+    while ((int)w.inv_ev.size() < 4) {
+        hipEvent_t e;
+        HIP_TRY(hipEventCreateWithFlags(&e, hipEventDisableTiming));
+        w.inv_ev.push_back(e);
+    }
+    hipEvent_t start = w.inv_ev[0], e_flow = w.inv_ev[1], e_chain = w.inv_ev[2];
+    HIP_TRY(hipEventRecord(start, crit));
+    HIP_TRY(hipStreamWaitEvent(priv, start, 0));
+    unsigned* ferr = w.flow_flags.p + p.base_err;
+    auto chain_launch = [&](int kb) -> int {
+        const int k0 = kb * ob, k1 = std::min(k0 + ob, nb), nk = k1 - k0;
+        const FlowPlan::Chain& pc = p.chain[kb];
+        ChainFlow cf{};
+        cf.done_flag = w.flow_flags.p + pc.done_idx; cf.write_through = 1;
+        cf.trace = want_trace ? w.flow_trace.p + FLOW_TRACE_W * p.tasks.size() + 4 * (size_t)kb : nullptr;
+        cf.diag = w.flow_diag.p;
+        return launch_chain(w.A.p, ld, k0, nk, w.invd.p, w.logdet.p, m->d_info.p, 0, w.Wm.p + (int64_t)k0 * MOGP_TILE * (ld + 1), ld,
+                            w.chain_flags.p + (size_t)kb * MOGP_CHAIN_FLAGS, ferr, priv, &cf);
+    };
+    if (!replay && nouter > 0 && (rc = chain_launch(0))) return rc;
+    HIP_TRY(hipStreamWaitEvent(bulk, start, 0));
+    if (w.bulk_first) {
+        rc = w.bulk_first(); w.bulk_first = nullptr;
+        if (rc) return rc;
+    }
+    if (pe0) HIP_TRY(hipEventRecord(pe0, bulk));
+    if (rhs && rhs->ready) HIP_TRY(hipStreamWaitEvent(bulk, rhs->ready, 0));
+
     const FlowArgs* d_g = reinterpret_cast<const FlowArgs*>(w.flow_args.p);
     FlowHot hot{};
     hot.bA = g.bA; hot.bL = g.bL; hot.bWt = g.bWt; hot.bWm = g.bWm; hot.bB = g.bB; hot.ld = g.ld; hot.tasks = g.tasks; hot.qmeta = g.qmeta; hot.flags = g.flags;
@@ -830,16 +853,10 @@
     m->gemm_launches += 1;
     m->gemm_flops += p.flops;
 
-    unsigned* ferr = w.flow_flags.p + p.base_err;
     for (int kb = 0; kb < nouter && !replay; ++kb) {
         const int k0 = kb * ob, k1 = std::min(k0 + ob, nb), nk = k1 - k0, na = std::min(ob, nb - k1);
         const FlowPlan::Chain& pc = p.chain[kb];
-        ChainFlow cf{};
-        cf.done_flag = w.flow_flags.p + pc.done_idx; cf.write_through = 1;
-        cf.trace = want_trace ? w.flow_trace.p + FLOW_TRACE_W * p.tasks.size() + 4 * (size_t)kb : nullptr;
-        cf.diag = w.flow_diag.p;
-        if ((rc = launch_chain(w.A.p, ld, k0, nk, w.invd.p, w.logdet.p, m->d_info.p, 0, w.Wm.p + (int64_t)k0 * MOGP_TILE * (ld + 1), ld,
-                               w.chain_flags.p + (size_t)kb * MOGP_CHAIN_FLAGS, ferr, priv, &cf))) return rc;
+        if (kb > 0 && (rc = chain_launch(kb))) return rc;
         if (na <= 0) continue;
         GemmArgs t1{};
         t1.A = w.A.p + (int64_t)k1 * MOGP_TILE * ld + (int64_t)k0 * MOGP_TILE; t1.lda = ld; t1.a_kmajor = 0;
diff --git a/mogptk_amd/csrc/gram.hip b/mogptk_amd/csrc/gram.hip
--- a/mogptk_amd/csrc/gram.hip
+++ b/mogptk_amd/csrc/gram.hip
@@ -59,10 +59,13 @@
 struct PhaseArgs {
     const double* x; int64_t ld; const int* off; const double* table; int T, D, C, W, role; double* cs; double* sn;
 };
-__global__ __launch_bounds__(256) void k_phase_table(PhaseArgs a) {
+struct PhaseArgs2 { PhaseArgs r[2]; };
+__global__ __launch_bounds__(256) void k_phase_table(PhaseArgs2 both) {
+    const int T = both.r[0].T, z = blockIdx.z;
+    const PhaseArgs& a = both.r[z < T ? 0 : 1];
     const int64_t pt = (int64_t)blockIdx.x * 256 + threadIdx.x;
-    if (pt >= a.off[a.C]) return;
-    const int o = blockIdx.y, t = blockIdx.z, D = a.D, W = a.W;
+    if (!a.x || pt >= a.off[a.C]) return;
+    const int o = blockIdx.y, t = z < T ? z : z - T, D = a.D, W = a.W;
     int c = 0;
     while (pt >= a.off[c + 1]) ++c;
     const int pair = a.role == 0 ? c * a.C + o : o * a.C + c;
@@ -79,7 +82,7 @@
     a.sn[idx] = sn;
 }
 
-struct CentreArgs { const double* x; int64_t ld; const int* off; int C, D; double* cen; double* half; };
+struct CentreArgs { const double* x; int64_t ld; const int* off; int C, D; double* cen; double* half; double* cen2; double* half2; };
 __global__ __launch_bounds__(64) void k_block_centres(CentreArgs a) {
     int b = blockIdx.x, c = 0;
     for (; c < a.C; ++c) {
@@ -94,7 +97,11 @@
         double lo = v, hi = v;
 #pragma unroll
         for (int off = 32; off > 0; off >>= 1) { lo = fmin(lo, __shfl_xor(lo, off, 64)); hi = fmax(hi, __shfl_xor(hi, off, 64)); }
-        if (lane == 0) { a.cen[(size_t)d * a.ld + start] = 0.5 * (lo + hi); a.half[(size_t)d * a.ld + start] = 0.5 * (hi - lo); }
+        if (lane == 0) {
+            const double cen = 0.5 * (lo + hi), half = 0.5 * (hi - lo);
+            a.cen[(size_t)d * a.ld + start] = cen; a.half[(size_t)d * a.ld + start] = half;
+            if (a.cen2) { a.cen2[(size_t)d * a.ld + start] = cen; a.half2[(size_t)d * a.ld + start] = half; }
+        }
     }
 }
 
@@ -117,18 +124,28 @@
                                const double* table, int T, int D, int C, int W, hipStream_t s) {
     if (!ph.ws || !ph.offr || !ph.offc) { set_error("Gram / moment launch without a phase workspace"); return -1; }
     const PhaseView v = phase_view(ph.ws, C, T, D, ldxr, ldxc);
-    PhaseArgs a;
-    a.table = table; a.T = T; a.D = D; a.C = C; a.W = W;
-    a.x = xr; a.ld = ldxr; a.off = ph.offr; a.role = 0; a.cs = const_cast<double*>(v.rcs); a.sn = const_cast<double*>(v.rsn);
-    if (nr > 0) hipLaunchKernelGGL(k_phase_table, dim3((unsigned)((nr + 255) / 256), C, T), dim3(256), 0, s, a);
-    a.x = xc; a.ld = ldxc; a.off = ph.offc; a.role = 1; a.cs = const_cast<double*>(v.ccs); a.sn = const_cast<double*>(v.csn);
-    if (nc > 0) hipLaunchKernelGGL(k_phase_table, dim3((unsigned)((nc + 255) / 256), C, T), dim3(256), 0, s, a);
+    PhaseArgs2 both;
+    for (int role = 0; role < 2; ++role) {
+        PhaseArgs& a = both.r[role];
+        a.table = table; a.T = T; a.D = D; a.C = C; a.W = W; a.role = role;
+        const bool have = (role == 0 ? nr : nc) > 0;
+        a.x = have ? (role == 0 ? xr : xc) : nullptr; a.ld = role == 0 ? ldxr : ldxc; a.off = role == 0 ? ph.offr : ph.offc;
+        a.cs = const_cast<double*>(role == 0 ? v.rcs : v.ccs); a.sn = const_cast<double*>(role == 0 ? v.rsn : v.csn);
+    }
+    const int64_t nmax = nr > nc ? nr : nc;
+    if (nmax > 0) hipLaunchKernelGGL(k_phase_table, dim3((unsigned)((nmax + 255) / 256), C, 2 * T), dim3(256), 0, s, both);
     CentreArgs c;
-    c.C = C; c.D = D;
-    c.x = xr; c.ld = ldxr; c.off = ph.offr; c.cen = const_cast<double*>(v.rcen); c.half = const_cast<double*>(v.rhalf);
-    if (nr > 0) hipLaunchKernelGGL(k_block_centres, dim3((unsigned)((nr + MOGP_GT - 1) / MOGP_GT + C)), dim3(64), 0, s, c);
-    c.x = xc; c.ld = ldxc; c.off = ph.offc; c.cen = const_cast<double*>(v.ccen); c.half = const_cast<double*>(v.chalf);
-    if (nc > 0) hipLaunchKernelGGL(k_block_centres, dim3((unsigned)((nc + MOGP_GT - 1) / MOGP_GT + C)), dim3(64), 0, s, c);
+    c.C = C; c.D = D; c.cen2 = c.half2 = nullptr;
+    if (ph.centres == PH_CENTRES_BOTH && xr == xc && ldxr == ldxc && nr == nc) {
+        c.x = xr; c.ld = ldxr; c.off = ph.offr; c.cen = const_cast<double*>(v.rcen); c.half = const_cast<double*>(v.rhalf);
+        c.cen2 = const_cast<double*>(v.ccen); c.half2 = const_cast<double*>(v.chalf);
+        if (nr > 0) hipLaunchKernelGGL(k_block_centres, dim3((unsigned)((nr + MOGP_GT - 1) / MOGP_GT + C)), dim3(64), 0, s, c);
+    } else if (ph.centres != PH_CENTRES_KEPT) {
+        c.x = xr; c.ld = ldxr; c.off = ph.offr; c.cen = const_cast<double*>(v.rcen); c.half = const_cast<double*>(v.rhalf);
+        if (nr > 0) hipLaunchKernelGGL(k_block_centres, dim3((unsigned)((nr + MOGP_GT - 1) / MOGP_GT + C)), dim3(64), 0, s, c);
+        c.x = xc; c.ld = ldxc; c.off = ph.offc; c.cen = const_cast<double*>(v.ccen); c.half = const_cast<double*>(v.chalf);
+        if (nc > 0) hipLaunchKernelGGL(k_block_centres, dim3((unsigned)((nc + MOGP_GT - 1) / MOGP_GT + C)), dim3(64), 0, s, c);
+    }
     HIP_TRY(hipGetLastError());
     return 0;
 }
diff --git a/mogptk_amd/csrc/loo.hip b/mogptk_amd/csrc/loo.hip
--- a/mogptk_amd/csrc/loo.hip
+++ b/mogptk_amd/csrc/loo.hip
@@ -119,7 +119,7 @@
     ma.phases_ready = 1;
     RC(launch_moments(ma, m->st, m->radial ? m->gate_kinds : 0));
     RC(launch_moment_reduce(m->d_partial.p, m->d_pair_start.p, P, T, W, D, m->d_moments.p, m->st, 1));
-    hipLaunchKernelGGL(k_loo_diag, dim3(C), dim3(256), 0, m->st, m->loo.G.p, Npad, m->d_chan_off.p, m->d_diagG.p);
+    hipLaunchKernelGGL(k_loo_diag, dim3(C), dim3(256), 0, m->st, m->loo.G.p, Npad, m->d_chan_off.p, m->diagG_dev());
     HIP_TRY(hipGetLastError());
     RC(mean_grad_enqueue(m, m->loo.vec.p + LOO_RHO * Npad, -1.0));
     return mark(m, 6);
diff --git a/mogptk_amd/csrc/mogp_api.hip b/mogptk_amd/csrc/mogp_api.hip
--- a/mogptk_amd/csrc/mogp_api.hip
+++ b/mogptk_amd/csrc/mogp_api.hip
@@ -605,6 +605,7 @@
         }
         HIP_TRY(dev_upload(m->d_pair_start.p, m->pair_start.data(), m->pair_start.size() * sizeof(int)));
     }
+    if (!m->h_up) HIP_TRY(hipHostMalloc(reinterpret_cast<void**>(&m->h_up), (size_t)m->C * sizeof(double), hipHostMallocDefault));
     if ((rc = m->d_partial.ensure(m->tiles.size() * (size_t)std::max(m->T, 1) * (size_t)std::max(m->Wt, 1)))) return rc;
     if (m->k.Npad == m->Npad) return (m->k.owned_rows && !m->sh_owned) ? spd_make_whole(m->k) : 0;
     return spd_alloc(m->k, m->Npad, m->sh_owned ? m->ctx->device : -1);
@@ -676,7 +677,6 @@
     TRY_RC(m->d_z.ensure(Npad));
     TRY_RC(m->d_alpha.ensure((size_t)(1 + nchunks) * Npad));
     TRY_RC(m->d_zz.ensure((Npad + 3) / 4));
-    TRY_RC(m->d_diagG.ensure(C));
     TRY_RC(m->d_info.ensure(2));
     TRY_RC(m->d_flag.ensure(1));
     TRY_RC(m->d_chan_off.ensure(C + 1));
@@ -709,15 +709,16 @@
     m->cv.release();
     m->d_x.release(); m->d_y.release(); m->d_table.release(); m->d_kind.release(); m->d_shape.release();
     m->d_noise.release(); m->d_dvar.release(); m->d_z.release(); m->d_alpha.release(); m->d_zz.release();
-    m->d_partial.release(); m->d_moments.release(); m->d_diagG.release(); m->d_tiles.release(); m->d_pair_start.release(); m->strip.release(); m->strip_own.release();
+    m->d_partial.release(); m->d_moments.release(); m->d_tiles.release(); m->d_pair_start.release(); m->strip.release(); m->strip_own.release();
     m->d_tiles_head.release(); m->d_tiles_tail.release(); m->strip_head.release(); m->strip_tail.release();
-    if (m->gram_ev) { hipError_t r = hipEventDestroy(m->gram_ev); (void)r; m->gram_ev = nullptr; }
     if (m->gram_tail_ev) { hipError_t r = hipEventDestroy(m->gram_tail_ev); (void)r; m->gram_tail_ev = nullptr; }
     m->d_chan_off.release(); m->d_flag.release(); m->d_info.release(); m->d_pivots.release(); m->acc_rhs.release();
     m->d_xs.release(); m->d_Ksf.release(); m->d_Vt.release(); m->d_mu.release(); m->d_var.release(); m->d_kdiag.release();
     m->d_Kss.release(); m->d_ptiles.release(); m->d_pred_tasks.release();
     m->ph_xx.release(); m->ph_sx.release(); m->ph_ss.release();
     if (m->h_pin) { hipError_t e = hipHostFree(m->h_pin); (void)e; m->h_pin = nullptr; }
+    if (m->h_up) { hipError_t e = hipHostFree(m->h_up); (void)e; m->h_up = nullptr; }
+    for (hipEvent_t* e : {&m->tail_ev[0], &m->tail_ev[1], &m->arm.ev, &m->arm.scal_ev}) if (*e) { hipError_t r = hipEventDestroy(*e); (void)r; *e = nullptr; }
     mean_release(m);
 
     delete m;
@@ -756,7 +757,7 @@
     if (m->tw) m->tw->pred_valid = false;
     m->table.assign(table, table + n);
     if ((rc = m->d_table.ensure(n))) return rc;
-    if ((rc = m->d_moments.ensure((size_t)(m->C * (m->C + 1) / 2) * T * W))) return rc;
+    if ((rc = m->d_moments.ensure((size_t)(m->C * (m->C + 1) / 2) * T * W + m->C))) return rc;
     HIP_TRY(hipMemcpyAsync(m->d_table.p, m->table.data(), n * sizeof(double), hipMemcpyHostToDevice, m->st));
     return MOGP_OK;
 }
diff --git a/mogptk_amd/csrc/mogp_internal.h b/mogptk_amd/csrc/mogp_internal.h
--- a/mogptk_amd/csrc/mogp_internal.h
+++ b/mogptk_amd/csrc/mogp_internal.h
@@ -71,10 +71,14 @@
 enum { GT_MIRROR = 1,
        GT_DIAG = 2 };
 
+enum { PH_CENTRES_EACH = 0,
+       PH_CENTRES_BOTH = 1,
+       PH_CENTRES_KEPT = 2 };
 struct PhaseRef {
     const int* offr = nullptr;
     const int* offc = nullptr;
     double* ws = nullptr;
+    int centres = PH_CENTRES_EACH;
 };
 size_t phase_ws_doubles(int C, int T, int64_t ldr, int64_t ldc);
 
diff --git a/mogptk_amd/csrc/mogp_model.h b/mogptk_amd/csrc/mogp_model.h
--- a/mogptk_amd/csrc/mogp_model.h
+++ b/mogptk_amd/csrc/mogp_model.h
@@ -1,6 +1,7 @@
 #pragma once
 #include "../../include/mogp_hip.h"
 #include "mogp_internal.h"
+#include <functional>
 
 #include <algorithm>
 #include <cmath>
@@ -96,6 +97,14 @@
     DevBuf<double> ws;
     DevBuf<int> offr, offc;
     std::vector<int> hr, hc;
+    const double* cen_ws = nullptr;
+    int cen_T = -1;
+    int prepare_fixed(const std::vector<int>& r, int C, int T, int64_t ld, hipStream_t s, PhaseRef& out) {
+        if (int rc = prepare(r, r, C, T, ld, ld, s, out)) return rc;
+        out.centres = (cen_ws == ws.p && cen_T == T) ? PH_CENTRES_KEPT : PH_CENTRES_BOTH;
+        cen_ws = ws.p; cen_T = T;
+        return 0;
+    }
     int prepare(const std::vector<int>& r, const std::vector<int>& c, int C, int T, int64_t ldr, int64_t ldc, hipStream_t s, PhaseRef& out) {
         int rc;
         if ((rc = ws.ensure(phase_ws_doubles(C, T, ldr, ldc)))) return rc;
@@ -112,7 +121,7 @@
         out.offr = offr.p; out.offc = offc.p; out.ws = ws.p;
         return 0;
     }
-    void release() { ws.release(); offr.release(); offc.release(); hr.clear(); hc.clear(); }
+    void release() { ws.release(); offr.release(); offc.release(); hr.clear(); hc.clear(); cen_ws = nullptr; cen_T = -1; }
 };
 
 struct SortedX {
@@ -201,6 +210,7 @@
     DevBuf<unsigned> flow_post;
     DevBuf<unsigned> flow_diag;
     DevBuf<unsigned long long> flow_trace;
+    std::function<int()> bulk_first;
     hipEvent_t tail_ready = nullptr;
     bool flow_used = false;
     bool want_vec = false, vec_done = false;
@@ -299,6 +309,15 @@
 };
 
 struct FlowRhs { double* T; double* X; int nt; hipEvent_t ready; };
+struct Armed {
+    bool enq = false;
+    bool valid = false;
+    bool want = false;
+    bool live = false;
+    hipEvent_t ev = nullptr, scal_ev = nullptr;
+    const void *chain_p = nullptr, *flow_p = nullptr, *zz_p = nullptr;
+    size_t chain_n = 0, nflags = 0, nzz = 0;
+};
 struct mogp_model {
     mogp_ctx* ctx = nullptr;
     int64_t N = 0, Npad = 0;
@@ -339,7 +358,7 @@
     std::vector<GTile> tiles_head, tiles_tail;
     DevBuf<GTile> d_tiles_head, d_tiles_tail;
     StripTiles strip_head, strip_tail;
-    hipEvent_t gram_ev = nullptr, gram_tail_ev = nullptr;
+    hipEvent_t gram_tail_ev = nullptr;
     DevBuf<int> d_pair_start_own;
     int own_rank = -1, own_n = 0;
     DevBuf<double> sh_send, sh_recv;
@@ -356,7 +375,9 @@
 
     std::vector<double> hy;
     DevBuf<double> d_symv;
-    DevBuf<double> d_x, d_y, d_table, d_noise, d_dvar, d_z, d_alpha, d_zz, d_partial, d_moments, d_diagG;
+    DevBuf<double> d_x, d_y, d_table, d_noise, d_dvar, d_z, d_alpha, d_zz, d_partial;
+    DevBuf<double> d_moments;
+    double* diagG_dev() const { return d_moments.p + (size_t)(C * (C + 1) / 2) * T * Wt; }
     DevBuf<GTile> d_tiles;
     std::vector<GemmTask> kinv_acc_tasks, kinv_lauum_tasks;
     std::vector<int> kinv_prefix;
@@ -378,6 +399,10 @@
 
     double* h_pin = nullptr;
     size_t h_pin_n = 0;
+    double* h_up = nullptr;
+    Armed arm;
+    hipStream_t tail_side = nullptr;
+    hipEvent_t tail_ev[2] = {nullptr, nullptr};
 
     bool profiling = false;
     std::vector<hipEvent_t> ev;
@@ -460,6 +485,7 @@
 #define MOGP_RETRY_NO_CHAIN 0x7e7e
 extern int g_outer;
 int begin_call(mogp_model* m, int64_t* info, bool one_gpu);
+int arm_drop(mogp_model* m);
 int exact_begin(mogp_model* m, const double* noise_var, const double* data_var, double jitter, GramArgs& ga, double& jabs);
 int report_not_pd(unsigned long long hinfo, int64_t* info);
 struct TestSide { SortedX ss; int64_t Spad = 0; int ntiles = 0; };
diff --git a/mogptk_amd/csrc/oa.hip b/mogptk_amd/csrc/oa.hip
--- a/mogptk_amd/csrc/oa.hip
+++ b/mogptk_amd/csrc/oa.hip
@@ -86,6 +86,7 @@
     double* lam = o.vec.p + V_LAM * Npad;
     RC(upload_sorted(m, q_nu, nu, 0.0));
     RC(upload_sorted(m, q_lambda, lam, 0.0));
+    RC(arm_drop(m));
     const unsigned long long big = std::numeric_limits<unsigned long long>::max();
     HIP_TRY(hipMemcpyAsync(m->d_info.p, &big, sizeof(big), hipMemcpyHostToDevice, m->st));
 
diff --git a/mogptk_amd/csrc/shard.hip b/mogptk_amd/csrc/shard.hip
--- a/mogptk_amd/csrc/shard.hip
+++ b/mogptk_amd/csrc/shard.hip
@@ -229,9 +229,9 @@
     if ((rc = mark(m, 5))) return rc;
     if ((rc = moment_pass_device(m, m->k.A.p, -1.0))) return rc;
     if ((rc = comm_allreduce(m->ctx, m->d_moments.p, (int64_t)P * T * W, m->st))) return rc;
-    if ((rc = comm_allreduce(m->ctx, m->d_diagG.p, C, m->st))) return rc;
+    if ((rc = comm_allreduce(m->ctx, m->diagG_dev(), C, m->st))) return rc;
     HIP_TRY(hipMemcpyAsync(moments, m->d_moments.p, (size_t)P * T * W * sizeof(double), hipMemcpyDeviceToHost, m->st));
-    HIP_TRY(hipMemcpyAsync(diagG, m->d_diagG.p, C * sizeof(double), hipMemcpyDeviceToHost, m->st));
+    HIP_TRY(hipMemcpyAsync(diagG, m->diagG_dev(), C * sizeof(double), hipMemcpyDeviceToHost, m->st));
     if ((rc = sweep_eval_scalars(m, lml, info))) return sharded_rc(m, rc);
     if (m->sh_prof_blocks > 0) {
         for (hipStream_t q : {m->st2, m->st2u}) if (q) HIP_TRY(hipStreamSynchronize(q));
diff --git a/mogptk_amd/csrc/sparse.hip b/mogptk_amd/csrc/sparse.hip
--- a/mogptk_amd/csrc/sparse.hip
+++ b/mogptk_amd/csrc/sparse.hip
@@ -203,6 +203,7 @@
     m->gemm_ev_used = 0; m->gemm_launches = 0; m->gemm_flops = 0.0;
     HIP_TRY(hipMemcpyAsync(t.zx.p, sz.xs.data(), (size_t)D * Mpad * sizeof(double), hipMemcpyHostToDevice, m->st));
     RC(sparse_tiles(m, t, sz, want_uf));
+    RC(arm_drop(m));
     const unsigned long long big = std::numeric_limits<unsigned long long>::max();
     HIP_TRY(hipMemcpyAsync(m->d_info.p, &big, sizeof(big), hipMemcpyHostToDevice, m->st));
 
```

Result: no change. 97.24, median of 6 (+0.4%).
